# apple/ml-4m

Measured on AMD Instinct MI355X. Metric: multimodal tokens/sec (4M-B train step, whole job), higher is better.
Workload: dtype bf16; 1 GPU; 4M-B mod7 (fm_base_12e_12d_swiglu_nobias, 360.8M params, 8 input / 7 target modalities) masked-modeling train step, 224^2 token grids, 128 input + 128 target tokens/sample, AdamW; model=fm_base_12e_12d_swiglu_nobias, per_gpu_batch=256, global_batch=256, seq_len=256, parallelism=dp1

## Files before the change

include/fourm_hip.h:

```cpp
#ifndef FOURM_HIP_H
#define FOURM_HIP_H
#include <stdint.h>

#ifdef __cplusplus
extern "C" {
#endif

#define FM_ABI_VERSION 11
int fm_abi_version(void);
const char* fm_last_error(void);

enum fm_epilogue {
    FM_EPI_BF16 = 0,
    FM_EPI_GELU = 1,
    FM_EPI_RESIDUAL = 2,
    FM_EPI_SWIGLU = 3,
    FM_EPI_F32 = 4,
    FM_EPI_TANH = 5,
    FM_EPI_SWIGLU_BWD = 6,
    FM_EPI_GELU_BWD = 7,
    FM_EPI_QUICK_GELU = 8,
    FM_EPI_RELU = 9,
    FM_EPI_RELU_BWD = 10
};

typedef struct fm_gemm_group {
    const void* W;
    void* out;
    int32_t N, K, ldw, pad_;
} fm_gemm_group;

typedef struct fm_gemm_nt_args {
    const void* W; const void* W2; const void* X;
    void* out; void* out2; const void* res; const void* bias; const void* bias2;
    int32_t M, N, K, ldw, ldx, ldo, ldo2, ldr, Hp, epilogue;
    const fm_gemm_group* groups; const int32_t* tile_group; int32_t max_N;
    int32_t fixed_tiling;
    const int32_t* m_dev; const int32_t* row0_dev;
    void* splitk_ws; int64_t splitk_ws_bytes;
    int32_t conv_C, conv_H, conv_W, conv_Ho, conv_Wo, conv_stride, conv_up, conv_pad_;
} fm_gemm_nt_args;
int fm_gemm_nt(const fm_gemm_nt_args* args, void* stream);
void fm_set_gemm_nt_config(int cfg);
int fm_get_gemm_nt_config(void);
void fm_set_reserved_cus(int n);
int fm_get_reserved_cus(void);

typedef struct fm_gemm_tn_args {
    const void* A; const void* B; void* out;
    int32_t R, N, K, lda, ldb, ldo, a_cols, b_cols, splits, force_tr;
    const fm_gemm_group* groups; const int32_t* seg_start; const int32_t* seg_count;
    int32_t n_groups, max_N, max_R, pad_;
} fm_gemm_tn_args;
int fm_gemm_tn(const fm_gemm_tn_args* args, void* stream);
#define FM_TN_MAX_JOBS 16
typedef struct fm_gemm_tn_job {
    const void* A; const void* B; void* out;
    int32_t R, N, K, lda, ldb, ldo, a_cols, b_cols;
} fm_gemm_tn_job;
int fm_gemm_tn_multi(const fm_gemm_tn_job* jobs, int n_jobs, void* stream);
void fm_set_gemm_tn_config(int cfg);
int fm_get_gemm_tn_config(void);
void fm_set_tn_transpose_read(int on);
int fm_get_tn_transpose_read(void);

int fm_layernorm_fwd(const void* x, int ldx, const void* w, const void* b, void* y, int ldy, int y_is_f32,
                     void* mean, void* rstd, const int32_t* row_map, int R, int D, float eps, void* stream);
int fm_layernorm_fwd_res(const void* x, int ldx, const void* delta, int ldd, void* x_out, int ldxo, const void* w, const void* b,
                         void* y, int ldy, int y_is_f32, void* mean, void* rstd, const int32_t* row_map, int R, int D, float eps,
                         void* stream);
int fm_layernorm_bwd(const void* dy, int lddy, const int32_t* dy_row_map, const void* x, int ldx, const void* w,
                     const void* mean, const void* rstd, const void* dres, void* dx, int lddx, void* dx_bf16,
                     int lddxbf, void* dw, void* db, int R, int D, void* stream);
int fm_layernorm_bwd_h(const void* dy, int lddy, const void* h, int ldh, const void* x, int ldx, const void* w,
                       const void* mean, const void* rstd, const void* dres, void* dx, int lddx, void* dx_bf16,
                       int lddxbf, void* dw, int R, int D, void* stream);

int fm_headnorm_fwd(const void* x, int ldx, const void* w, const void* b, void* y, int ldy, void* stats, int R, int H, float eps,
                    void* stream);
int fm_headnorm_bwd(const void* dy, int lddy, const void* x, int ldx, const void* w, const void* stats, void* dx, int lddx, void* dw,
                    void* db, int R, int H, void* stream);

enum fm_mask_kind {
    FM_MASK_NONE = 0,
    FM_MASK_KEYPAD = 1,
    FM_MASK_DECODER = 2,
    FM_MASK_DENSE = 3
};
typedef struct fm_attn_args {
    const void* Q; const void* K; const void* V; void* O;
    void* stat_m; void* stat_l;
    int32_t ldq, ldk, ldv, ldo;
    int32_t B, H, Nq, Nk, head_dim, mask_kind;
    float scale; int32_t causal;
    const void* kpad; const int32_t* cs; const int16_t* modq; const int16_t* modk; const void* dense;
    const void* dO; void* dQ; void* dK; void* dV;
    int32_t lddo, lddq, lddk, lddv;
    int32_t force_tr;
    int32_t kv_batch_rows;
    int32_t zero_attn;
} fm_attn_args;
int fm_attn_fwd(const fm_attn_args* args, void* stream);
int fm_attn_bwd(const fm_attn_args* args, void* stream);
void fm_set_attn_transpose_read(int on);
int fm_get_attn_transpose_read(void);

#define FM_ATTN_DECODE_MAX_NK 8192
typedef struct fm_attn_decode_args {
    const void* q; void* k; const void* v; void* o;
    const void* q_w; const void* q_b; const void* k_w; const void* k_b;
    const void* kpad;
    int32_t ldq, ldk, ldv, ldo;
    int32_t B, H, Nk, kv_batch_rows, k_new_row, is_f32, zero_attn, pad_;
    float scale, eps;
} fm_attn_decode_args;
int fm_attn_decode(const fm_attn_decode_args* args, void* stream);

#define FM_MAX_MODS 24
enum fm_mod_kind {
    FM_KIND_TOK = 0,
    FM_KIND_PATCH = 1,
    FM_KIND_SEQ = 2,
    FM_KIND_SEQ_EMB = 3
};
typedef struct fm_mod_desc {
    const void* ids;
    const void* mask;
    const void* dam;
    const void* table;
    const void* pos;
    const void* mod_emb;
    const void* proj_bias;
    int32_t L;
    int32_t kind, ids_are_i64, mod_id;
    int32_t max_len;
    int32_t shifted;
    int32_t mask_stride, id_stride;
    int32_t patch, channels, grid_w, orig_dim;
    int32_t head_index;
    int32_t pad_;
} fm_mod_desc;

typedef struct fm_select_desc {
    fm_mod_desc mods[FM_MAX_MODS];
    int32_t n_mods, batch, dim, n_keep, n_reg, total_len, is_decoder;
    int32_t raw;
    const void* reg_tokens;
    const void* mask_token;
    void* tokens;
    void* emb;
    void* x0;
    void* out_mask;
    void* out_mod;
    void* slot_mod;
    void* slot_src;
    void* slot_pos;
    void* target_ids;
    void* out_cs;
    void* out_mod_pre;
    void* out_mod_index;
    void* patch_rows;
    void* seqemb_rows;
    int32_t patch_ld, seqemb_ld;
    int32_t rows_f32;
    int32_t pad2_;
} fm_select_desc;
int fm_select_embed(const fm_select_desc* desc, void* stream);

typedef struct fm_embed_bwd_mod {
    void* d_table;
    void* d_pos;
    void* d_mod_emb;
    void* d_proj_bias;
    int32_t kind, has_padding_idx, padding_idx, pad_;
} fm_embed_bwd_mod;
typedef struct fm_embed_bwd_desc {
    fm_embed_bwd_mod mods[FM_MAX_MODS];
    const void* dx;
    const void* slot_mod; const void* slot_src; const void* slot_pos;
    void* d_mask_token;
    void* d_reg_tokens;
    int32_t n_mods, batch, dim, Nt, lddx, is_decoder;
} fm_embed_bwd_desc;
int fm_embed_bwd(const fm_embed_bwd_desc* desc, void* stream);

int fm_dense_decoder_mask(const int32_t* cs, const int16_t* mod, void* out, int B, int M, int causal, int use_cs,
                          int use_sep, void* stream);

enum fm_loss_type { FM_LOSS_MOD = 0, FM_LOSS_TOKEN = 1 };
#define FM_SEG_ROWS 256
int fm_segment_rows(const int32_t* head_of_row, int R, int n_heads, int32_t* seg_start, int32_t* seg_count,
                    int32_t* perm, int32_t* row_to_padded, int32_t* tile_group, int Rp, void* stream);
int fm_gather_rows(const void* src, int ld_src, const int32_t* perm, void* dst, int ld_dst, int Rp, int D, void* stream);
int fm_cross_entropy(void* logits, int ldl, const int32_t* perm, const int32_t* tile_group, const int64_t* target_ids,
                     const int32_t* vocab, const int32_t* seg_start, const int32_t* seg_count, const void* grad_scale,
                     int loss_type, int n_heads, int Rp, int max_vocab, void* row_loss, void* row_lse, void* head_loss,
                     void* total_loss, int write_grad, void* stream);

int fm_swiglu_bwd(const void* da, int ldda, const void* gu, int ldgu, void* dgu, int lddgu, int R, int H, int Hp, void* stream);
int fm_gelu_bwd(const void* dh, int lddh, const void* pre, int ldp, void* dpre, int lddp, int R, int H, int Hp, void* stream);
typedef struct fm_shadow_desc {
    const void* src; void* dst;
    int32_t ld_src, ld_dst, rows, cols, transpose, tile_start;
    const void* col_scale;
    int32_t dst_f32, reserved;
} fm_shadow_desc;
int fm_shadow_refresh(const fm_shadow_desc* descs, int n_descs, int total_tiles, void* stream);
#define FM_FOLD_MAX_JOBS 48
typedef struct fm_fold_grad_job {
    const void* dWp; const void* W; const void* gamma; void* gW; void* ggamma;
    int32_t rows, cols, ld_dwp, reserved;
} fm_fold_grad_job;
int fm_fold_colscale_grad(const fm_fold_grad_job* jobs, int n_jobs, void* stream);

int fm_cast_pad(const void* src, int ld_src, void* dst, int ld_dst, int rows, int cols, void* stream);
int fm_transpose_cast_pad(const void* src, int ld_src, void* dst, int ld_dst, int dst_cols, int rows, int cols, void* stream);
int fm_colsum(const void* dy, int ldy, void* db, int R, int N, void* stream);
int fm_f32_to_bf16(const void* src, void* dst, int64_t n, void* stream);
int fm_bf16_to_f32_scaled(const void* src, void* dst, int64_t n, float scale, void* stream);
int fm_add_bf16_f32(const void* x, const void* delta, void* out, int64_t n, void* stream);
int fm_scale_rows_bf16(void* x, int ld, const void* scale, int rows_per_sample, int R, int N, void* stream);

int fm_vit_patch_rows(const void* pixels, void* rows, int ld, int B, int C, int H, int W, int P, int rows_f32, void* stream);
int fm_vit_emb_rows(const void* pos, const void* mod_emb, void* x, int ldx, int B, int Np, int D, void* stream);
int fm_vit_colsum(const void* dy, int ldy, void* db, int R, int N, void* ws, int64_t ws_bytes, void* stream);

int fm_clip_embed_ln(const void* patches, int ldp, int patches_f32, const void* cls, const void* pos, const void* w, const void* b,
                     void* out, int ldo, int B, int G, int D, float eps, void* stream);

enum { FM_FEAT_COSINE = 0, FM_FEAT_L1 = 1 };
int fm_feat_distance(const void* pred, int ldp, const void* tgt, int ldt, int B, int T, int D, int mode, void* loss, void* dpred, int lddp,
                     void* stream);
int fm_quick_gelu_bwd(const void* da, int ldda, const void* pre, int ldp, void* dpre, int lddp, int R, int H, int Hp, void* stream);
int fm_quick_gelu_bwd_f32(const void* da, int ldda, const void* pre, int ldp, void* dpre, int lddp, int R, int H, void* stream);
int fm_clip_embed_ln_bwd(const void* dy, int lddy, const void* patches, int ldp, int patches_f32, const void* pos, const void* w,
                         void* d_patches, int lddp, int B, int G, int D, float eps, void* stream);
int fm_tap_add(void* g, int ldg, void* g_bf, int ldgb, const void* dtap, int ldt, const void* row_scale, int rows_per_sample, int R, int D,
               void* stream);

#define FM_LPIPS_CHUNK 64
int fm_lpips_stem(const void* img, const void* mul, const void* add, const void* w, const void* bias, void* out, int ldo, int is_f32, int B, int H,
                  int W, void* stream);
int fm_lpips_stem_bwd(const void* d, int ldd, int is_f32, const void* w, const void* mul, const void* row_scale, void* dimg, int B, int H, int W,
                      void* stream);
int fm_maxpool2x2_nhwc(const void* x, int ldx, void* y, int ldy, int is_f32, int B, int H, int W, int C, void* stream);
int fm_lpips_distance(const void* pred, int ldp, const void* tgt, int ldt, int is_f32, const void* w, int B, int P, int C, void* loss, void* dpred,
                      int lddp, void* scratch, void* stream);
int fm_lpips_tap_bwd(const void* act, int lda, const void* din, int ldi, const void* dtap, int ldt, const void* dpool, int ldp, void* d, int ldd,
                     int is_f32, int B, int H, int W, int C, void* stream);

int fm_lora_apply(const void* x, int ldx, const void* down, int64_t down_sr, int64_t down_sk, const void* up, int64_t up_sn, int64_t up_sr,
                  void* y, int ldy, float scale, void* p_out, int R, int K, int N, int r, int x_f32, int y_f32, void* stream);
int fm_lora_grad(const void* a, int lda, const void* b, void* out, int64_t out_sn, int64_t out_sr, float scale, int accumulate,
                 int R, int n, int r, int a_f32, void* stream);

int fm_adamw(void* p, const void* g, void* m, void* v, int64_t n, float lr, float beta1, float beta2, float eps,
             float weight_decay, int64_t step, const void* grad_mult, const void* hyper, void* sumsq, void* stream);
#define FM_ADAMW_CHUNK 8192
typedef struct fm_adamw_job {
    void* p; const void* g; void* m; void* v; void* dst_plain; void* dst_t;
    int32_t rows, cols, ld_plain, ld_t, tile_start, pad_;
} fm_adamw_job;
int fm_adamw_shadow(const fm_adamw_job* jobs, int n_jobs, int total_tiles, float lr, float beta1, float beta2, float eps,
                    float weight_decay, int64_t step, const void* grad_mult, const void* hyper, void* sumsq, void* stream);
int fm_sumsq(const void* x, int64_t n, void* out, void* stream);
int fm_clip_coef(const void* sumsq, float max_norm, void* norm_out, void* coef_out, void* stream);

int fm_sample_tokens(const void* logits, int ld, int logits_are_f32, int R, int V, float temperature, int top_k, float top_p,
                     const void* uniforms, void* out_ids, void* out_prob, void* stream);
int fm_guidance_combine(const void* uncond, int ldu, int uncond_is_f32, const void* cond, int ldc, int cond_is_f32, float weight,
                        void* out, int ldo, int R, int V, int accumulate, void* stream);
int fm_maskgit_commit(const void* prob, const void* samples, const int32_t* mod_pos, int B, int N, int num_select, void* tensor,
                      int tensor_is_i64, int L, void* input_mask, void* target_mask, int32_t* top_idx, void* stream);

typedef struct fm_gemm_f32_args {
    const void* X; const void* W; const void* W2; void* out; void* out2; const void* res; const void* bias; const void* bias2;
    int64_t sxm, sxk, swn, swk;
    int32_t M, N, K, ldo, ldo2, ldr, Hp, epilogue, accumulate, max_N, seg_rows, n_groups;
    const fm_gemm_group* groups; const int32_t* tile_group; const int32_t* seg_start; const int32_t* seg_count;
} fm_gemm_f32_args;
int fm_gemm_f32(const fm_gemm_f32_args* args, void* stream);
int fm_attn_f32_fwd(const fm_attn_args* args, void* stream);
int fm_attn_f32_bwd(const fm_attn_args* args, void* stream);
int fm_layernorm_bwd_f32(const void* dy, int lddy, const int32_t* dy_row_map, const void* x, int ldx, const void* w, const void* mean,
                         const void* rstd, const void* dres, void* dx, int lddx, void* dx2, int lddx2, void* dw, void* db, int R, int D,
                         void* stream);
int fm_headnorm_f32_fwd(const void* x, int ldx, const void* w, const void* b, void* y, int ldy, void* stats, int R, int H, float eps, void* stream);
int fm_headnorm_f32_bwd(const void* dy, int lddy, const void* x, int ldx, const void* w, const void* stats, void* dx, int lddx, void* dw, void* db,
                        int R, int H, void* stream);
int fm_swiglu_bwd_f32(const void* da, int ldda, const void* gu, int ldgu, void* dgu, int lddgu, int R, int H, int Hp, void* stream);
int fm_gelu_bwd_f32(const void* dh, int lddh, const void* pre, int ldp, void* dpre, int lddp, int R, int H, void* stream);
int fm_colsum_f32(const void* dy, int ldy, void* db, int R, int N, void* stream);
int fm_cross_entropy_f32(void* logits, int ldl, const int32_t* perm, const int32_t* tile_group, const int64_t* target_ids,
                         const int32_t* vocab, const int32_t* seg_start, const int32_t* seg_count, const void* grad_scale, int loss_type,
                         int n_heads, int padded_rows, int max_vocab, void* row_loss, void* row_lse, void* head_loss, void* total_loss,
                         int write_grad, void* stream);

int fm_unet_im2col_f32(const void* src1, int ld1, int C1, const void* src2, int ld2, int C2, int H2, int W2, void* out, int ldo, int kpad,
                       int B, int H, int W, int ksize, int stride, int up1, void* stream);
int fm_groupnorm_nhwc_f32(const void* x, int ldx, const void* add, int ld_add, const void* w, const void* b, void* y, int ldy, int B, int HW, int C,
                          int groups, float eps, int silu, void* stream);
int fm_unet_attention_f32(const void* qkv, int ld, void* out, int ldo, int B, int T, int heads, int ch, void* stream);
int fm_add_f32(const void* a, int lda, const void* b, int ldb, void* out, int ldo, int64_t rows, int C, void* stream);
int fm_silu_f32(const void* x, void* y, int64_t n, void* stream);
int fm_timestep_embedding_f32(const void* t, void* out, int ldo, int B, int dim, float max_period, void* stream);
int fm_unet_col2im_f32(const void* col, int ldc, void* dsrc, int ld, int C, int B, int H, int W, int ksize, int stride, int up1, int accumulate, void* stream);
int fm_groupnorm_nhwc_bwd_f32(const void* dy, int lddy, const void* x, int ldx, const void* add, int ld_add, const void* w, const void* b, void* dx, int lddx,
                              void* dw, void* db, void* dadd, int ld_dadd, void* scratch, int B, int HW, int C, int groups, float eps, int silu, void* stream);
int fm_unet_attention_bwd_f32(const void* qkv, int ld, const void* dout, int lddo, void* dqkv, int lddqkv, void* scratch, int B, int T, int heads, int ch,
                              void* stream);
int fm_silu_bwd_f32(const void* dy, const void* x, void* dx, int64_t n, void* stream);

int fm_vq_patchify(const void* img, void* out, int ld_out, int B, int C, int H, int W, int P, void* stream);
int fm_l2norm_rows(const void* x, int ldx, void* y, int ldy, int R, int D, void* stream);
int fm_vq_assign(const void* z, int ldz, const void* codes_normalized, const void* embed, int K, int D, int R,
                 int tokens_per_image, int normalize_latents, void* ws_val, void* ws_idx, int splits, int64_t* tokens,
                 void* quant, void* stream);
#define FM_VQ_WIDE_TILE 128
int fm_vq_assign_wide(const void* z, int ldz, const void* codes_normalized, const void* embed, int K, int D, int R,
                      int tokens_per_image, void* ws_val, void* ws_idx, int code_tiles, int64_t* tokens, void* quant, void* stream);
int fm_memcodes_assign(const void* z, int ldz, const void* keys, const void* values, int K, int d, int H, int R,
                       int tokens_per_image, void* ws_val, void* ws_idx, int code_tiles, int64_t* tokens, void* quant, void* stream);
int fm_vq_code_stats(const void* z, int ldz, const int64_t* tokens, int R, int D, int K, void* bins, void* sums, void* stream);
int fm_vq_ema_update(const void* bins, const void* sums, void* embed, void* cluster_size, int K, int D, float decay, void* stream);
int fm_vq_code_bias(const void* embed, int K, int D, void* bias, void* stream);
int fm_vq_assign_bias(const void* z, int ldz, const void* codes, const void* code_bias, const void* embed, int K, int D, int R,
                      int tokens_per_image, int normalize_latents, void* ws_val, void* ws_idx, int splits, int64_t* tokens,
                      void* quant, void* stream);
int fm_vq_code_stats_raw(const void* z, int ldz, const int64_t* tokens, int R, int D, int K, void* bins, void* sums, void* stream);
int fm_vq_ema_update_euclid(const void* bins, const void* sums, void* embed, void* embed_avg, void* cluster_size, void* total_scratch,
                            int K, int D, float decay, float eps, void* stream);

int fm_vq_unpatchify(const void* rows, int ld_rows, void* img, int B, int C, int H, int W, int P, void* stream);
#define FM_CONVNEXT_MAX_C 4
int fm_convnext_block(const void* x, void* y, const void* dw_weight, const void* dw_bias, const void* ln_weight, const void* ln_bias,
                      const void* pw1_weight, const void* pw1_bias, const void* pw2_weight, const void* pw2_bias, const void* gamma,
                      int B, int C, int H, int W, float eps, void* stream);
// ... 129 lines not shown
```

ml-4m_amd/csrc/layernorm.hip:

```cpp
#include <algorithm>
#include "common.h"
#include "fourm_hip.h"

namespace {

constexpr int MAXC_LIMIT = 8;

__device__ __forceinline__ float4 ld4(const float* p, bool nt) {
    if (nt) { const f32x4_t t = __builtin_nontemporal_load((const f32x4_t*)p); return make_float4(t[0], t[1], t[2], t[3]); }
    return *(const float4*)p;
}
__device__ __forceinline__ uint2 ld2u(const bf16_t* p, bool nt) {
    typedef __attribute__((ext_vector_type(2))) unsigned int u2_t;
    if (nt) { const u2_t t = __builtin_nontemporal_load((const u2_t*)p); return make_uint2(t[0], t[1]); }
    return *(const uint2*)p;
}
template <typename T> __device__ __forceinline__ void store4(T* p, float a, float b, float c, float d);
template <> __device__ __forceinline__ void store4<float>(float* p, float a, float b, float c, float d) {
    *(float4*)p = make_float4(a, b, c, d);
}
template <> __device__ __forceinline__ void store4<bf16_t>(bf16_t* p, float a, float b, float c, float d) {
    *(uint2*)p = make_uint2(pack2bf(a, b), pack2bf(c, d));
}

template <typename OutT, int MAXC, bool RES = false>
__global__ __launch_bounds__(256) void ln_fwd_kernel(const float* __restrict__ x, int ldx, const float* __restrict__ w,
                                                     const float* __restrict__ b, OutT* __restrict__ y, int ldy,
                                                     float* __restrict__ mean, float* __restrict__ rstd,
                                                     const int* __restrict__ row_map, int R, int D, float eps,
                                                     const bf16_t* __restrict__ delta = nullptr, int ldd = 0, float* __restrict__ xo = nullptr, int ldxo = 0,
                                                     int nt_res = 0) {
    const int lane = threadIdx.x & 63, wave = threadIdx.x >> 6;
    const int nch = D >> 2;
    float4 ww[MAXC], bb[MAXC];
#pragma unroll
    for (int c = 0; c < MAXC; ++c) {
        const int ch = lane + 64 * c;
        ww[c] = ch < nch ? *(const float4*)(w + ch * 4) : make_float4(0.f, 0.f, 0.f, 0.f);
        bb[c] = (b && ch < nch) ? *(const float4*)(b + ch * 4) : make_float4(0.f, 0.f, 0.f, 0.f);
    }
    constexpr int NR = 2;
    for (int r0 = blockIdx.x * 4 + wave; r0 < R; r0 += gridDim.x * 4 * NR) {
        float4 v[NR][MAXC];
#pragma unroll
        for (int q = 0; q < NR; ++q) {
            const int r = r0 + q * gridDim.x * 4;
#pragma unroll
            for (int c = 0; c < MAXC; ++c) {
                const int ch = lane + 64 * c;
                v[q][c] = (ch < nch && r < R) ? ld4(x + (size_t)r * ldx + ch * 4, nt_res & 2) : make_float4(0.f, 0.f, 0.f, 0.f);
            }
        }
        if constexpr (RES) {
            uint2 dl[NR][MAXC];
#pragma unroll
            for (int q = 0; q < NR; ++q) {
                const int r = r0 + q * gridDim.x * 4;
#pragma unroll
                for (int c = 0; c < MAXC; ++c) {
                    const int ch = lane + 64 * c;
                    dl[q][c] = (ch < nch && r < R) ? ld2u(delta + (size_t)r * ldd + ch * 4, nt_res & 2) : make_uint2(0u, 0u);
                }
            }
#pragma unroll
            for (int q = 0; q < NR; ++q) {
                const int r = r0 + q * gridDim.x * 4;
#pragma unroll
                for (int c = 0; c < MAXC; ++c) {
                    const int ch = lane + 64 * c;
                    float d4[4];
                    unpack_bf4(dl[q][c], d4);
                    v[q][c].x += d4[0]; v[q][c].y += d4[1]; v[q][c].z += d4[2]; v[q][c].w += d4[3];
                    if (ch < nch && r < R) {
                        if (nt_res & 1) __builtin_nontemporal_store(f32x4_t{v[q][c].x, v[q][c].y, v[q][c].z, v[q][c].w}, (f32x4_t*)(xo + (size_t)r * ldxo + ch * 4));
                        else *(float4*)(xo + (size_t)r * ldxo + ch * 4) = v[q][c];
                    }
                }
            }
        }
#pragma unroll
        for (int q = 0; q < NR; ++q) {
            const int r = r0 + q * gridDim.x * 4;
            if (r >= R) continue;
            float s = 0.f;
#pragma unroll
            for (int c = 0; c < MAXC; ++c) s += (v[q][c].x + v[q][c].y) + (v[q][c].z + v[q][c].w);
            const float mu = wave_sum(s) / (float)D;
            float sq = 0.f;
#pragma unroll
            for (int c = 0; c < MAXC; ++c) {
                const int ch = lane + 64 * c;
                if (ch < nch) {
                    const float a0 = v[q][c].x - mu, a1 = v[q][c].y - mu, a2 = v[q][c].z - mu, a3 = v[q][c].w - mu;
                    sq += (a0 * a0 + a1 * a1) + (a2 * a2 + a3 * a3);
                }
            }
            const float rs = rsqrtf(wave_sum(sq) / (float)D + eps);
            if (lane == 0) {
                if (mean) mean[r] = mu;
                if (rstd) rstd[r] = rs;
            }
            const int dst = row_map ? row_map[r] : r;
            if (dst < 0) continue;
            OutT* yr = y + (size_t)dst * ldy;
#pragma unroll
            for (int c = 0; c < MAXC; ++c) {
                const int ch = lane + 64 * c;
                if (ch < nch)
                    store4<OutT>(yr + ch * 4, (v[q][c].x - mu) * rs * ww[c].x + bb[c].x, (v[q][c].y - mu) * rs * ww[c].y + bb[c].y,
                                 (v[q][c].z - mu) * rs * ww[c].z + bb[c].z, (v[q][c].w - mu) * rs * ww[c].w + bb[c].w);
            }
        }
    }
}

static int ln_nt_flags() {
    static const int f = [] { const char* e = getenv("FOURM_LN_NT"); return e ? atoi(e) : 24; }();
    return f;
}
static int bwd_rows(int R) {
    static const int env = [] { const char* e = getenv("FOURM_LN_BWD_ROWS"); return e ? atoi(e) : 0; }();
    if (env >= 4) return env;
    return R >= 512 * 64 ? 64 : 32;
}

template <int MAXC, bool FROM_H = false, bool HAS_DB = true>
__global__ __launch_bounds__(256) void ln_bwd_kernel(const bf16_t* __restrict__ dy, int lddy, const int* __restrict__ dy_row_map,
                                                     const bf16_t* __restrict__ h, int ldh,
                                                     const float* __restrict__ x, int ldx, const float* __restrict__ w,
                                                     const float* __restrict__ mean, const float* __restrict__ rstd,
                                                     const float* dres, float* dx, int lddx, bf16_t* __restrict__ dx_bf, int lddxbf,
                                                     float* __restrict__ dw, float* __restrict__ db, int R, int D, int BWD_ROWS, int nt_dx) {
    extern __shared__ __attribute__((aligned(16))) char smem[];
    float* red = (float*)smem;
    const int lane = threadIdx.x & 63, wave = threadIdx.x >> 6;
    const int nch = D >> 2;
    float4 aw[MAXC], ab[MAXC], wv[MAXC], iw[FROM_H ? MAXC : 1];
    bool from_x[FROM_H ? MAXC : 1];
#pragma unroll
    for (int c = 0; c < MAXC; ++c) {
        aw[c] = ab[c] = make_float4(0.f, 0.f, 0.f, 0.f);
        const int ch = lane + 64 * c;
        wv[c] = ch < nch ? *(const float4*)(w + ch * 4) : make_float4(0.f, 0.f, 0.f, 0.f);
        if constexpr (FROM_H) {
            from_x[c] = fminf(fminf(fabsf(wv[c].x), fabsf(wv[c].y)), fminf(fabsf(wv[c].z), fabsf(wv[c].w))) < 1e-20f;
            iw[c] = from_x[c] ? make_float4(0.f, 0.f, 0.f, 0.f) : make_float4(1.f / wv[c].x, 1.f / wv[c].y, 1.f / wv[c].z, 1.f / wv[c].w);
        }
    }
    const int r_end = min(R, (int)(blockIdx.x + 1) * BWD_ROWS);
    constexpr int NR = 2;
    for (int r0 = blockIdx.x * BWD_ROWS + wave; r0 < r_end; r0 += 4 * NR) {
        uint2 dyp[NR][MAXC], hp[NR][FROM_H ? MAXC : 1];
        float4 xv[NR][MAXC], rv[NR][MAXC];
        float mu[NR], rs[NR];
        bool live[NR];
#pragma unroll
        for (int q = 0; q < NR; ++q) {
            const int r = r0 + 4 * q;
            live[q] = r < r_end;
            const int rr = live[q] ? r : r0;
            const int src = dy_row_map ? dy_row_map[rr] : rr;
            mu[q] = mean[rr]; rs[q] = rstd[rr];
#pragma unroll
            for (int c = 0; c < MAXC; ++c) {
                const int ch = lane + 64 * c;
                dyp[q][c] = make_uint2(0u, 0u);
                xv[q][c] = rv[q][c] = make_float4(0.f, 0.f, 0.f, 0.f);
                if (ch < nch && live[q]) {
                    if (src >= 0) dyp[q][c] = ld2u(dy + (size_t)src * lddy + ch * 4, nt_dx & 2);
                    if constexpr (FROM_H) {
                        hp[q][c] = ld2u(h + (size_t)rr * ldh + ch * 4, nt_dx & 4);
                        if (from_x[c]) xv[q][c] = *(const float4*)(x + (size_t)rr * ldx + ch * 4);
                    } else xv[q][c] = *(const float4*)(x + (size_t)rr * ldx + ch * 4);
                    if (dres) rv[q][c] = ld4(dres + (size_t)rr * lddx + ch * 4, nt_dx & 2);
                }
            }
        }
#pragma unroll
        for (int q = 0; q < NR; ++q) {
            if (!live[q]) continue;
            const int r = r0 + 4 * q;
            float4 g[MAXC], xh[MAXC];
            float s1 = 0.f, s2 = 0.f;
#pragma unroll
            for (int c = 0; c < MAXC; ++c) {
                const int ch = lane + 64 * c;
                g[c] = xh[c] = make_float4(0.f, 0.f, 0.f, 0.f);
                if (ch < nch) {
                    const uint2 p = dyp[q][c];
                    const float4 d = make_float4(bf2f((bf16_t)(p.x & 0xffff)), bf2f((bf16_t)(p.x >> 16)), bf2f((bf16_t)(p.y & 0xffff)), bf2f((bf16_t)(p.y >> 16)));
                    const float4 v = xv[q][c];
                    xh[c] = make_float4((v.x - mu[q]) * rs[q], (v.y - mu[q]) * rs[q], (v.z - mu[q]) * rs[q], (v.w - mu[q]) * rs[q]);
                    if constexpr (FROM_H) {
                        const uint2 hh = hp[q][c];
                        if (!from_x[c]) xh[c] = make_float4(bf2f((bf16_t)(hh.x & 0xffff)) * iw[c].x, bf2f((bf16_t)(hh.x >> 16)) * iw[c].y,
                                                            bf2f((bf16_t)(hh.y & 0xffff)) * iw[c].z, bf2f((bf16_t)(hh.y >> 16)) * iw[c].w);
                    }
                    aw[c].x += d.x * xh[c].x; aw[c].y += d.y * xh[c].y; aw[c].z += d.z * xh[c].z; aw[c].w += d.w * xh[c].w;
                    if constexpr (HAS_DB) { ab[c].x += d.x; ab[c].y += d.y; ab[c].z += d.z; ab[c].w += d.w; }
                    g[c] = make_float4(d.x * wv[c].x, d.y * wv[c].y, d.z * wv[c].z, d.w * wv[c].w);
                    s1 += (g[c].x + g[c].y) + (g[c].z + g[c].w);
                    s2 += (g[c].x * xh[c].x + g[c].y * xh[c].y) + (g[c].z * xh[c].z + g[c].w * xh[c].w);
                }
            }
            const float m1 = wave_sum(s1) / (float)D, m2 = wave_sum(s2) / (float)D;
#pragma unroll
            for (int c = 0; c < MAXC; ++c) {
                const int ch = lane + 64 * c;
                if (ch < nch) {
                    const float4 t = rv[q][c];
                    const float4 o = make_float4(rs[q] * (g[c].x - m1 - xh[c].x * m2) + t.x, rs[q] * (g[c].y - m1 - xh[c].y * m2) + t.y,
                                                 rs[q] * (g[c].z - m1 - xh[c].z * m2) + t.z, rs[q] * (g[c].w - m1 - xh[c].w * m2) + t.w);
                    if (nt_dx & 1) __builtin_nontemporal_store(f32x4_t{o.x, o.y, o.z, o.w}, (f32x4_t*)(dx + (size_t)r * lddx + ch * 4));
                    else *(float4*)(dx + (size_t)r * lddx + ch * 4) = o;
                    if (dx_bf) *(uint2*)(dx_bf + (size_t)r * lddxbf + ch * 4) = make_uint2(pack2bf(o.x, o.y), pack2bf(o.z, o.w));
                }
            }
        }
    }
    if (!dw && !db) return;
#pragma unroll
    for (int c = 0; c < MAXC; ++c) {
        const int ch = lane + 64 * c;
        if (ch < nch) {
            *(float4*)(red + (size_t)wave * D + ch * 4) = aw[c];
            if constexpr (HAS_DB) *(float4*)(red + (size_t)(4 + wave) * D + ch * 4) = ab[c];
        }
    }
    __syncthreads();
    for (int i = threadIdx.x; i < D; i += 256) {
        if (dw) unsafeAtomicAdd(dw + i, (red[i] + red[D + i]) + (red[2 * D + i] + red[3 * D + i]));
        if constexpr (HAS_DB) if (db) unsafeAtomicAdd(db + i, (red[4 * D + i] + red[5 * D + i]) + (red[6 * D + i] + red[7 * D + i]));
    }
}


__device__ __forceinline__ float group16_sum(float v) {
    v += __shfl_xor(v, 1, 64); v += __shfl_xor(v, 2, 64); v += __shfl_xor(v, 4, 64); v += __shfl_xor(v, 8, 64);
    return v;
}

__global__ __launch_bounds__(256) void headnorm_fwd_kernel(const bf16_t* __restrict__ x, int ldx, const float* __restrict__ w,
                                                           const float* __restrict__ b, bf16_t* __restrict__ y, int ldy,
                                                           float2* __restrict__ stats, int R, int H, float eps) {
    const int sub = threadIdx.x & 15;
    const float4 wv = *(const float4*)(w + sub * 4);
    const float4 bv = b ? *(const float4*)(b + sub * 4) : make_float4(0.f, 0.f, 0.f, 0.f);
    const size_t total = (size_t)R * H;
    for (size_t v = (size_t)blockIdx.x * 16 + (threadIdx.x >> 4); v < total; v += (size_t)gridDim.x * 16) {
        const int r = v / H, h = v % H;
        const uint2 p = *(const uint2*)(x + (size_t)r * ldx + h * 64 + sub * 4);
        const float e[4] = {bf2f((bf16_t)(p.x & 0xffff)), bf2f((bf16_t)(p.x >> 16)), bf2f((bf16_t)(p.y & 0xffff)), bf2f((bf16_t)(p.y >> 16))};
        const float mean = group16_sum(e[0] + e[1] + e[2] + e[3]) * (1.0f / 64.0f);
        float q = 0.f;
#pragma unroll
        for (int i = 0; i < 4; ++i) q += (e[i] - mean) * (e[i] - mean);
        const float rs = rsqrtf(group16_sum(q) * (1.0f / 64.0f) + eps);
        const float o0 = (e[0] - mean) * rs * wv.x + bv.x, o1 = (e[1] - mean) * rs * wv.y + bv.y;
        const float o2 = (e[2] - mean) * rs * wv.z + bv.z, o3 = (e[3] - mean) * rs * wv.w + bv.w;
        *(uint2*)(y + (size_t)r * ldy + h * 64 + sub * 4) = make_uint2(pack2bf(o0, o1), pack2bf(o2, o3));
        if (sub == 0 && stats) stats[v] = make_float2(mean, rs);
    }
}

__global__ __launch_bounds__(256) void headnorm_bwd_kernel(const bf16_t* __restrict__ dy, int lddy, const bf16_t* __restrict__ x, int ldx,
                                                           const float* __restrict__ w, const float2* __restrict__ stats,
                                                           bf16_t* __restrict__ dx, int lddx, float* __restrict__ dw, float* __restrict__ db,
                                                           int R, int H) {
    __shared__ float red[2][16][64];
    const int sub = threadIdx.x & 15, grp = threadIdx.x >> 4;
    const float4 wv = *(const float4*)(w + sub * 4);
    const float wj[4] = {wv.x, wv.y, wv.z, wv.w};
    float aw[4] = {0.f, 0.f, 0.f, 0.f}, ab[4] = {0.f, 0.f, 0.f, 0.f};
    const size_t total = (size_t)R * H;
    for (size_t v = (size_t)blockIdx.x * 16 + grp; v < total; v += (size_t)gridDim.x * 16) {
        const int r = v / H, h = v % H;
        const uint2 px = *(const uint2*)(x + (size_t)r * ldx + h * 64 + sub * 4);
        const uint2 pd = *(const uint2*)(dy + (size_t)r * lddy + h * 64 + sub * 4);
        const float2 st = stats[v];
        const float e[4] = {bf2f((bf16_t)(px.x & 0xffff)), bf2f((bf16_t)(px.x >> 16)), bf2f((bf16_t)(px.y & 0xffff)), bf2f((bf16_t)(px.y >> 16))};
        const float d[4] = {bf2f((bf16_t)(pd.x & 0xffff)), bf2f((bf16_t)(pd.x >> 16)), bf2f((bf16_t)(pd.y & 0xffff)), bf2f((bf16_t)(pd.y >> 16))};
        float xh[4], g[4], s1 = 0.f, s2 = 0.f;
#pragma unroll
        for (int i = 0; i < 4; ++i) {
            xh[i] = (e[i] - st.x) * st.y;
            g[i] = d[i] * wj[i];
            s1 += g[i]; s2 += g[i] * xh[i];
            aw[i] += d[i] * xh[i]; ab[i] += d[i];
        }
        s1 = group16_sum(s1) * (1.0f / 64.0f); s2 = group16_sum(s2) * (1.0f / 64.0f);
        float o[4];
#pragma unroll
        for (int i = 0; i < 4; ++i) o[i] = st.y * (g[i] - s1 - xh[i] * s2);
        *(uint2*)(dx + (size_t)r * lddx + h * 64 + sub * 4) = make_uint2(pack2bf(o[0], o[1]), pack2bf(o[2], o[3]));
    }
#pragma unroll
    for (int i = 0; i < 4; ++i) { red[0][grp][sub * 4 + i] = aw[i]; red[1][grp][sub * 4 + i] = ab[i]; }
    __syncthreads();
    if (threadIdx.x < 128) {
        const int which = threadIdx.x >> 6, c = threadIdx.x & 63;
        float s = 0.f;
#pragma unroll
        for (int gq = 0; gq < 16; ++gq) s += red[which][gq][c];
        float* dst = which ? db : dw;
        if (dst) unsafeAtomicAdd(dst + c, s);
    }
}

}

static int chunks_for(int D) { const int c = (D / 4 + 63) / 64; return c <= 2 ? 2 : c <= 3 ? 3 : c <= 4 ? 4 : 8; }

extern "C" int fm_layernorm_fwd(const void* x, int ldx, const void* w, const void* b, void* y, int ldy, int y_is_f32,
                                void* mean, void* rstd, const int32_t* row_map, int R, int D, float eps, void* stream) {
    FM_CHECK_ARG(x && w && y, "fm_layernorm_fwd: null pointer");
    FM_CHECK_ARG(R > 0 && D > 0 && D % 4 == 0 && D <= 64 * 4 * MAXC_LIMIT, "fm_layernorm_fwd: D=%d must be a multiple of 4 and <= %d", D, 64 * 4 * MAXC_LIMIT);
    FM_CHECK_ARG(ldx % 4 == 0 && ldy % 4 == 0, "fm_layernorm_fwd: leading dims must be multiples of 4");
    int grid = (R + 3) / 4;
    if (grid > 256 * 16) grid = 256 * 16;
#define LN_FWD(T, C)                                                                                                        \
    hipLaunchKernelGGL((ln_fwd_kernel<T, C>), dim3(grid), dim3(256), 0, (hipStream_t)stream, (const float*)x, ldx, (const float*)w, \
                       (const float*)b, (T*)y, ldy, (float*)mean, (float*)rstd, row_map, R, D, eps)
#define LN_FWD_C(T)                                    \
    switch (chunks_for(D)) {                           \
        case 2: LN_FWD(T, 2); break;                   \
        case 3: LN_FWD(T, 3); break;                   \
        case 4: LN_FWD(T, 4); break;                   \
        default: LN_FWD(T, 8); break;                  \
    }
    if (y_is_f32) { LN_FWD_C(float) } else { LN_FWD_C(bf16_t) }
#undef LN_FWD_C
#undef LN_FWD
    FM_CHECK_LAUNCH("fm_layernorm_fwd");
    return 0;
}

extern "C" int fm_layernorm_fwd_res(const void* x, int ldx, const void* delta, int ldd, void* x_out, int ldxo, const void* w, const void* b,
                                    void* y, int ldy, int y_is_f32, void* mean, void* rstd, const int32_t* row_map, int R, int D, float eps,
                                    void* stream) {
    FM_CHECK_ARG(x && delta && x_out && w && y, "fm_layernorm_fwd_res: null pointer");
    FM_CHECK_ARG(R > 0 && D > 0 && D % 4 == 0 && D <= 64 * 4 * MAXC_LIMIT, "fm_layernorm_fwd_res: D=%d must be a multiple of 4 and <= %d", D, 64 * 4 * MAXC_LIMIT);
    FM_CHECK_ARG(ldx % 4 == 0 && ldy % 4 == 0 && ldd % 4 == 0 && ldxo % 4 == 0, "fm_layernorm_fwd_res: leading dims must be multiples of 4");
    FM_CHECK_ARG((((uintptr_t)delta) & 7) == 0 && (((uintptr_t)x_out | (uintptr_t)x) & 15) == 0, "fm_layernorm_fwd_res: alignment (delta 8 B, x / x_out 16 B)");
    int grid = (R + 3) / 4;
    if (grid > 256 * 16) grid = 256 * 16;
#define LN_FWD(T, C)                                                                                                        \
    hipLaunchKernelGGL((ln_fwd_kernel<T, C, true>), dim3(grid), dim3(256), 0, (hipStream_t)stream, (const float*)x, ldx, (const float*)w, \
                       (const float*)b, (T*)y, ldy, (float*)mean, (float*)rstd, row_map, R, D, eps, (const bf16_t*)delta, ldd, (float*)x_out, ldxo, (ln_nt_flags() & 1) | ((ln_nt_flags() >> 1) & 2))
#define LN_FWD_C(T)                                    \
    switch (chunks_for(D)) {                           \
        case 2: LN_FWD(T, 2); break;                   \
        case 3: LN_FWD(T, 3); break;                   \
        case 4: LN_FWD(T, 4); break;                   \
        default: LN_FWD(T, 8); break;                  \
    }
    if (y_is_f32) { LN_FWD_C(float) } else { LN_FWD_C(bf16_t) }
#undef LN_FWD_C
#undef LN_FWD
    FM_CHECK_LAUNCH("fm_layernorm_fwd_res");
    return 0;
}

static int layernorm_bwd_launch(const void* dy, int lddy, const int32_t* dy_row_map, const void* h, int ldh, const void* x, int ldx, const void* w,
                                const void* mean, const void* rstd, const void* dres, void* dx, int lddx, void* dx_bf16,
                                int lddxbf, void* dw, void* db, int R, int D, void* stream) {
    FM_CHECK_ARG(dy && x && w && mean && rstd && dx, "fm_layernorm_bwd: null pointer");
    FM_CHECK_ARG(!h || ldh % 4 == 0, "fm_layernorm_bwd_h: ldh must be a multiple of 4");
    FM_CHECK_ARG(R > 0 && D > 0 && D % 4 == 0 && D <= 64 * 4 * MAXC_LIMIT, "fm_layernorm_bwd: D=%d unsupported", D);
    FM_CHECK_ARG(ldx % 4 == 0 && lddy % 4 == 0 && lddx % 4 == 0 && lddxbf % 4 == 0, "fm_layernorm_bwd: leading dims must be multiples of 4");
    const int BWD_ROWS = bwd_rows(R);
    const int grid = (R + BWD_ROWS - 1) / BWD_ROWS;
    const size_t lds = (size_t)8 * D * sizeof(float);
#define LN_BWD_(C, FH)                                                                                                      \
    {                                                                                                                       \
        auto k = ln_bwd_kernel<C, FH, !FH>;                                                                                     \
        static bool once = (hipFuncSetAttribute((const void*)k, hipFuncAttributeMaxDynamicSharedMemorySize, 8 * 2048 * 4) == hipSuccess); \
        (void)once;                                                                                                         \
        hipLaunchKernelGGL(k, dim3(grid), dim3(256), lds, (hipStream_t)stream, (const bf16_t*)dy, lddy, dy_row_map, (const bf16_t*)h, ldh, \
                           (const float*)x, ldx, (const float*)w, (const float*)mean, (const float*)rstd, (const float*)dres, (float*)dx, lddx, \
                           (bf16_t*)dx_bf16, lddxbf, (float*)dw, (float*)db, R, D, BWD_ROWS, ((ln_nt_flags() >> 1) & 1) | ((ln_nt_flags() >> 2) & 2) | ((ln_nt_flags() >> 2) & 4));                               \
    }
#define LN_BWD(C) { if (h) LN_BWD_(C, true) else LN_BWD_(C, false) }
    switch (chunks_for(D)) {
        case 2: LN_BWD(2) break;
        case 3: LN_BWD(3) break;
        case 4: LN_BWD(4) break;
        default: LN_BWD(8) break;
    }
#undef LN_BWD
#undef LN_BWD_
    FM_CHECK_LAUNCH("fm_layernorm_bwd");
    return 0;
}

extern "C" int fm_layernorm_bwd(const void* dy, int lddy, const int32_t* dy_row_map, const void* x, int ldx, const void* w,
                                const void* mean, const void* rstd, const void* dres, void* dx, int lddx, void* dx_bf16,
                                int lddxbf, void* dw, void* db, int R, int D, void* stream) {
    return layernorm_bwd_launch(dy, lddy, dy_row_map, nullptr, 0, x, ldx, w, mean, rstd, dres, dx, lddx, dx_bf16, lddxbf, dw, db, R, D, stream);
}

extern "C" int fm_layernorm_bwd_h(const void* dy, int lddy, const void* h, int ldh, const void* x, int ldx, const void* w,
                                  const void* mean, const void* rstd, const void* dres, void* dx, int lddx, void* dx_bf16,
                                  int lddxbf, void* dw, int R, int D, void* stream) {
    FM_CHECK_ARG(h, "fm_layernorm_bwd_h: null pointer");
    return layernorm_bwd_launch(dy, lddy, nullptr, h, ldh, x, ldx, w, mean, rstd, dres, dx, lddx, dx_bf16, lddxbf, dw, nullptr, R, D, stream);
}

extern "C" int fm_headnorm_fwd(const void* x, int ldx, const void* w, const void* b, void* y, int ldy, void* stats, int R, int H, float eps,
                               void* stream) {
    FM_CHECK_ARG(x && w && y && R > 0 && H > 0, "fm_headnorm_fwd: bad argument");
    FM_CHECK_ARG(ldx % 4 == 0 && ldy % 4 == 0 && ((((uintptr_t)x | (uintptr_t)y) & 7) == 0) && ((((uintptr_t)w | (uintptr_t)b) & 15) == 0),
                 "fm_headnorm_fwd: alignment (x/y 8 B, w/b 16 B, leading dims %% 4)");
    const size_t total = (size_t)R * H;
    const int grid = (int)std::min<size_t>((total + 15) / 16, 256 * 32);
    hipLaunchKernelGGL(headnorm_fwd_kernel, dim3(grid), dim3(256), 0, (hipStream_t)stream, (const bf16_t*)x, ldx, (const float*)w, (const float*)b,
                       (bf16_t*)y, ldy, (float2*)stats, R, H, eps);
    FM_CHECK_LAUNCH("fm_headnorm_fwd");
    return 0;
}

extern "C" int fm_headnorm_bwd(const void* dy, int lddy, const void* x, int ldx, const void* w, const void* stats, void* dx, int lddx, void* dw,
                               void* db, int R, int H, void* stream) {
    FM_CHECK_ARG(dy && x && w && stats && dx && R > 0 && H > 0, "fm_headnorm_bwd: bad argument");
    FM_CHECK_ARG(ldx % 4 == 0 && lddy % 4 == 0 && lddx % 4 == 0 && ((((uintptr_t)x | (uintptr_t)dy | (uintptr_t)dx) & 7) == 0) &&
                     ((((uintptr_t)w) & 15) == 0), "fm_headnorm_bwd: alignment (x/dy/dx 8 B, w 16 B, leading dims %% 4)");
    const size_t total = (size_t)R * H;
    const int grid = (int)std::min<size_t>((total + 15) / 16, 256 * 8);
    hipLaunchKernelGGL(headnorm_bwd_kernel, dim3(grid), dim3(256), 0, (hipStream_t)stream, (const bf16_t*)dy, lddy, (const bf16_t*)x, ldx,
                       (const float*)w, (const float2*)stats, (bf16_t*)dx, lddx, (float*)dw, (float*)db, R, H);
    FM_CHECK_LAUNCH("fm_headnorm_bwd");
    return 0;
}
```

ml-4m_amd/csrc/select_embed.hip:

```cpp
#include "common.h"
#include "fourm_hip.h"

namespace {

constexpr int MAXPOS = 8192;
constexpr int MAXKEEP = 1024;

struct SelArgs {
    fm_select_desc d;
};

__device__ __forceinline__ long long load_id(const void* ids, int is64, size_t i) {
    return is64 ? ((const long long*)ids)[i] : (long long)((const int*)ids)[i];
}

__device__ __forceinline__ int block_scan_excl(int v, int* wave_tot , int* total) {
    const int lane = threadIdx.x & 63, wave = threadIdx.x >> 6;
    const int inc = wave_scan_incl(v);
    if (lane == 63) wave_tot[wave] = inc;
    __syncthreads();
    int base = 0, tot = 0;
#pragma unroll
    for (int w = 0; w < 4; ++w) {
        const int t = wave_tot[w];
        if (w < wave) base += t;
        tot += t;
    }
    __syncthreads();
    *total = tot;
    return base + inc - v;
}

__global__ __launch_bounds__(256) void select_embed_kernel(SelArgs A) {
    const fm_select_desc& d = A.d;
    extern __shared__ __attribute__((aligned(16))) char smem[];
    const int P = d.total_len;
    int* rank_sel = (int*)smem;
    int* rank_pos = rank_sel + P;
    int* slot_p = rank_pos + P;
    uint8_t* flag = (uint8_t*)(slot_p + d.n_keep);
    __shared__ int wave_tot[4];
    __shared__ int mod_off[FM_MAX_MODS + 1];
    __shared__ int cs_scan[MAXKEEP];

    const int b = blockIdx.x;
    const int tid = threadIdx.x, lane = tid & 63, wave = tid >> 6;
    if (tid == 0) {
        int o = 0;
        for (int m = 0; m < d.n_mods; ++m) { mod_off[m] = o; o += d.mods[m].L; }
        mod_off[d.n_mods] = o;
    }
    __syncthreads();

    auto mod_of = [&](int p) {
        int m = 0;
        while (m + 1 < d.n_mods && p >= mod_off[m + 1]) ++m;
        return m;
    };

    int run_sel = 0, run_pos = 0;
    for (int base = 0; base < P; base += 256) {
        const int p = base + tid;
        int sel = 0, um = 0;
        if (p < P) {
            const int m = mod_of(p);
            const fm_mod_desc& md = d.mods[m];
            const int j = p - mod_off[m];
            const uint8_t* mk = (const uint8_t*)md.mask + (size_t)b * md.mask_stride;
            if (d.is_decoder && md.shifted) {
                um = mk[j] == 0;
                sel = (mk[j] == 0) && (mk[j + 1] == 0);
            } else {
                um = sel = mk[j] == 0;
            }
            flag[p] = (uint8_t)(sel | (um << 1));
        }
        int ts, tp;
        const int es = block_scan_excl(sel, wave_tot, &ts);
        const int ep = block_scan_excl(um, wave_tot, &tp);
        if (p < P) { rank_sel[p] = run_sel + es; rank_pos[p] = run_pos + ep; }
        run_sel += ts; run_pos += tp;
    }
    const int n_valid = run_sel;
    __syncthreads();
    for (int p = tid; p < P; p += 256) {
        const int s = d.raw ? p : (flag[p] & 1) ? rank_sel[p] : n_valid + (p - rank_sel[p]);
        if (s < d.n_keep) slot_p[s] = p;
    }
    __syncthreads();

    if (d.is_decoder && !d.raw) {
        if (wave == 0) {
            int run = 0;
            for (int base = 0; base < d.n_keep; base += 64) {
                const int s = base + lane;
                int v = 0;
                if (s < d.n_keep) {
                    const int p = slot_p[s];
                    const int m = mod_of(p);
                    const fm_mod_desc& md = d.mods[m];
                    v = ((const int*)md.dam)[(size_t)b * md.mask_stride + (p - mod_off[m])];
                }
                const int inc = wave_scan_incl(v);
                if (s < d.n_keep) cs_scan[s] = run + inc;
                run += __shfl(inc, 63, 64);
            }
        }
        __syncthreads();
    }

    const int D = d.dim, nch = D >> 2;
    const int Nt = d.n_reg + d.n_keep;
    for (int s = wave + 4 * blockIdx.y; s < Nt; s += 4 * gridDim.y) {
        const size_t orow = (size_t)b * Nt + s;
        float* tok_o = (float*)d.tokens + orow * D;
        float* emb_o = (float*)d.emb + orow * D;
        float* x0_o = d.x0 ? (float*)d.x0 + orow * D : nullptr;
        if (s < d.n_reg) {
            for (int c = lane; c < nch; c += 64) {
                const float4 t = *(const float4*)((const float*)d.reg_tokens + (size_t)s * D + c * 4);
                *(float4*)(tok_o + c * 4) = t;
                *(float4*)(emb_o + c * 4) = make_float4(0.f, 0.f, 0.f, 0.f);
                if (x0_o) *(float4*)(x0_o + c * 4) = t;
            }
            if (lane == 0) {
                ((uint8_t*)d.out_mask)[orow] = 0;
                ((int16_t*)d.out_mod)[orow] = -1;
                ((int32_t*)d.slot_mod)[orow] = -2;
                ((int32_t*)d.slot_src)[orow] = s;
                ((int32_t*)d.slot_pos)[orow] = 0;
            }
            const int esz = d.rows_f32 ? 2 : 1;
            if (d.patch_rows) {
                uint2* pr = (uint2*)((char*)d.patch_rows + orow * d.patch_ld * (size_t)(2 * esz));
                for (int f = lane; f < d.patch_ld / 4 * esz; f += 64) pr[f] = make_uint2(0u, 0u);
            }
            if (d.seqemb_rows) {
                uint2* sr = (uint2*)((char*)d.seqemb_rows + orow * d.seqemb_ld * (size_t)(2 * esz));
                for (int f = lane; f < d.seqemb_ld / 4 * esz; f += 64) sr[f] = make_uint2(0u, 0u);
            }
            continue;
        }
        const int sk = s - d.n_reg;
        const int p = slot_p[sk];
        const int m = mod_of(p);
        const fm_mod_desc& md = d.mods[m];
        const int j = p - mod_off[m];
        const bool masked = (flag[p] & 1) == 0;
        const bool own_unmasked = (flag[p] & 2) != 0;
        const bool raw = d.raw != 0;
        long long id = 0;
        int posrow = 0;
// ... 25 lines not shown
            else if (md.kind == FM_KIND_SEQ_EMB) trow = (const float*)md.proj_bias;
        }
        const float* prow = (const float*)md.pos + (size_t)posrow * D;
        const float* mrow = (const float*)md.mod_emb;
        const bool seq_kind = md.kind == FM_KIND_SEQ || md.kind == FM_KIND_SEQ_EMB;
        const bool with_emb = raw ? true : !masked;
        const bool with_pos = raw ? (!seq_kind || own_unmasked) : true;
        for (int c = lane; c < nch; c += 64) {
            float4 t = make_float4(0.f, 0.f, 0.f, 0.f), e = make_float4(0.f, 0.f, 0.f, 0.f);
            if (trow) t = *(const float4*)(trow + c * 4);
            if (with_emb) {
                const float4 mm = *(const float4*)(mrow + c * 4);
                float4 pp = make_float4(0.f, 0.f, 0.f, 0.f);
                if (with_pos) pp = *(const float4*)(prow + c * 4);
                e = make_float4(pp.x + mm.x, pp.y + mm.y, pp.z + mm.z, pp.w + mm.w);
            }
            *(float4*)(tok_o + c * 4) = t;
            *(float4*)(emb_o + c * 4) = e;
            if (x0_o) *(float4*)(x0_o + c * 4) = make_float4(t.x + e.x, t.y + e.y, t.z + e.z, t.w + e.w);
        }
        if (d.patch_rows && d.rows_f32) {
            float* pr = (float*)d.patch_rows + orow * d.patch_ld;
            const bool here = (!masked || raw) && md.kind == FM_KIND_PATCH;
            const int ps = md.patch, C = md.channels, gw = md.grid_w;
            const float* img = (const float*)md.ids + (size_t)b * md.id_stride;
            for (int f = lane; f < d.patch_ld; f += 64) {
                float v = 0.f;
                if (here && f < ps * ps * C) {
                    const int gy = j / gw, gx = j % gw, Wd = gw * ps, Hd = (md.L / gw) * ps;
                    const int c = f % C, px = (f / C) % ps, py = f / (C * ps);
                    v = img[((size_t)c * Hd + gy * ps + py) * Wd + gx * ps + px];
                }
                pr[f] = v;
            }
        } else if (d.patch_rows) {
            bf16_t* pr = (bf16_t*)d.patch_rows + orow * d.patch_ld;
            if ((!masked || raw) && md.kind == FM_KIND_PATCH) {
                const int ps = md.patch, C = md.channels, gw = md.grid_w;
                const int gy = j / gw, gx = j % gw;
                const float* img = (const float*)md.ids + (size_t)b * md.id_stride;
                const int Wd = gw * ps, Hd = (md.L / gw) * ps;
                for (int f = lane; f < d.patch_ld; f += 64) {
                    float v = 0.f;
                    if (f < ps * ps * C) {
                        const int c = f % C, px = (f / C) % ps, py = f / (C * ps);
                        v = img[((size_t)c * Hd + gy * ps + py) * Wd + gx * ps + px];
                    }
                    pr[f] = f2bf(v);
                }
            } else {
                for (int f = lane; f < d.patch_ld / 4; f += 64) *(uint2*)(pr + f * 4) = make_uint2(0u, 0u);
            }
        }
        if (d.seqemb_rows && d.rows_f32) {
            float* sr = (float*)d.seqemb_rows + orow * d.seqemb_ld;
            const bool here = (!masked || raw) && md.kind == FM_KIND_SEQ_EMB;
            const float* src = (const float*)md.ids + (size_t)b * md.id_stride + (size_t)j * md.orig_dim;
            for (int f = lane; f < d.seqemb_ld; f += 64) sr[f] = (here && f < md.orig_dim) ? src[f] : 0.f;
        } else if (d.seqemb_rows) {
            bf16_t* sr = (bf16_t*)d.seqemb_rows + orow * d.seqemb_ld;
            if ((!masked || raw) && md.kind == FM_KIND_SEQ_EMB) {
                const float* src = (const float*)md.ids + (size_t)b * md.id_stride + (size_t)j * md.orig_dim;
                for (int f = lane; f < d.seqemb_ld; f += 64) sr[f] = f2bf(f < md.orig_dim ? src[f] : 0.f);
            } else {
                for (int f = lane; f < d.seqemb_ld / 4; f += 64) *(uint2*)(sr + f * 4) = make_uint2(0u, 0u);
            }
        }
    }
}

__global__ __launch_bounds__(256) void embed_bwd_kernel(fm_embed_bwd_desc d) {
    extern __shared__ __attribute__((aligned(16))) char smem[];
    float* acc = (float*)smem;
    const int D = d.dim, nch = D >> 2;
    const int b = blockIdx.x, lane = threadIdx.x & 63, wave = threadIdx.x >> 6;
    const int rows = d.n_mods + 1;
    for (int i = threadIdx.x; i < rows * D; i += 256) acc[i] = 0.f;
    __shared__ int used[FM_MAX_MODS + 1];
    if (threadIdx.x <= FM_MAX_MODS) used[threadIdx.x] = 0;
    __syncthreads();
    constexpr int MAXQ = 8;
    const int parts = 4 * gridDim.y, part = wave + 4 * blockIdx.y;
    const int per = (d.Nt + parts - 1) / parts, s_lo = part * per, s_hi = min(d.Nt, s_lo + per);
    float4 racc[MAXQ];
    int cur = -1;
    bool cur_mask = false;
    auto flush = [&]() {
        if (cur < 0) return;
#pragma unroll
        for (int q = 0; q < MAXQ; ++q) {
            const int c = lane + 64 * q;
            if (c >= nch) break;
            float* a0 = acc + (size_t)cur * D + c * 4;
            atomicAdd(a0, racc[q].x); atomicAdd(a0 + 1, racc[q].y); atomicAdd(a0 + 2, racc[q].z); atomicAdd(a0 + 3, racc[q].w);
            if (cur_mask) {
                float* a1 = acc + (size_t)d.n_mods * D + c * 4;
                atomicAdd(a1, racc[q].x); atomicAdd(a1 + 1, racc[q].y); atomicAdd(a1 + 2, racc[q].z); atomicAdd(a1 + 3, racc[q].w);
            }
        }
    };
    for (int s = s_lo; s < s_hi; ++s) {
        const size_t row = (size_t)b * d.Nt + s;
        const int m = ((const int32_t*)d.slot_mod)[row];
        if (m == -1) continue;
        const float* g = (const float*)d.dx + row * d.lddx;
        if (m == -2) {
            if (d.d_reg_tokens)
                for (int c = lane; c < D; c += 64) unsafeAtomicAdd((float*)d.d_reg_tokens + (size_t)s * D + c, g[c]);
            continue;
        }
        const fm_embed_bwd_mod& md = d.mods[m];
        const int src = ((const int32_t*)d.slot_src)[row];
        const int posrow = ((const int32_t*)d.slot_pos)[row];
        const bool to_mask_token = d.is_decoder && md.kind == FM_KIND_TOK;
        if (m != cur) {
            flush();
            cur = m; cur_mask = to_mask_token;
#pragma unroll
            for (int q = 0; q < MAXQ; ++q) racc[q] = make_float4(0.f, 0.f, 0.f, 0.f);
            if (lane == 0) { used[m] = 1; if (to_mask_token) used[d.n_mods] = 1; }
        }
        float* trow = nullptr;
        if (to_mask_token) {}
        else if ((md.kind == FM_KIND_TOK || md.kind == FM_KIND_SEQ) && md.d_table && !(md.has_padding_idx && src == md.padding_idx))
            trow = (float*)md.d_table + (size_t)src * D;
        else if (md.kind == FM_KIND_SEQ_EMB && md.d_proj_bias) trow = (float*)md.d_proj_bias;
        float* prow = md.d_pos ? (float*)md.d_pos + (size_t)posrow * D : nullptr;
#pragma unroll
        for (int q = 0; q < MAXQ; ++q) {
            const int c = lane + 64 * q;
            if (c >= nch) break;
            const float4 v = *(const float4*)(g + c * 4);
            racc[q].x += v.x; racc[q].y += v.y; racc[q].z += v.z; racc[q].w += v.w;
            if (trow) {
                unsafeAtomicAdd(trow + c * 4, v.x); unsafeAtomicAdd(trow + c * 4 + 1, v.y);
                unsafeAtomicAdd(trow + c * 4 + 2, v.z); unsafeAtomicAdd(trow + c * 4 + 3, v.w);
            }
            if (prow) {
                unsafeAtomicAdd(prow + c * 4, v.x); unsafeAtomicAdd(prow + c * 4 + 1, v.y);
                unsafeAtomicAdd(prow + c * 4 + 2, v.z); unsafeAtomicAdd(prow + c * 4 + 3, v.w);
            }
        }
    }
    flush();
    __syncthreads();
    for (int m = 0; m < d.n_mods; ++m) {
        if (!used[m] || !d.mods[m].d_mod_emb) continue;
        for (int c = threadIdx.x; c < D; c += 256) unsafeAtomicAdd((float*)d.mods[m].d_mod_emb + c, acc[(size_t)m * D + c]);
    }
    if (used[d.n_mods] && d.d_mask_token)
        for (int c = threadIdx.x; c < D; c += 256) unsafeAtomicAdd((float*)d.d_mask_token + c, acc[(size_t)d.n_mods * D + c]);
}

__global__ void dense_decoder_mask_kernel(const int32_t* cs, const int16_t* mod, uint8_t* out, int B, int M, int causal, int use_cs, int use_sep) {
    const size_t i = (size_t)blockIdx.x * 256 + threadIdx.x;
    if (i >= (size_t)B * M * M) return;
    const int k = i % M, q = (i / M) % M, b = i / ((size_t)M * M);
    bool blk = false;
    if (causal) blk = k > q;
    else if (use_cs) blk = k >= cs[(size_t)b * M + q];
    if (use_sep) blk = blk || (mod[(size_t)b * M + q] != mod[(size_t)b * M + k]);
    out[i] = blk ? 1 : 0;
}

}

extern "C" int fm_select_embed(const fm_select_desc* d, void* stream) {
    FM_CHECK_ARG(d && d->tokens && d->emb && d->out_mask && d->out_mod && d->slot_mod && d->slot_src && d->slot_pos, "fm_select_embed: null output");
    FM_CHECK_ARG(d->n_mods > 0 && d->n_mods <= FM_MAX_MODS, "fm_select_embed: n_mods=%d out of range (max %d)", d->n_mods, FM_MAX_MODS);
    FM_CHECK_ARG(d->dim > 0 && d->dim % 4 == 0, "fm_select_embed: dim must be a multiple of 4");
    FM_CHECK_ARG(d->batch > 0 && d->n_keep > 0 && d->n_keep <= (d->raw ? MAXPOS : MAXKEEP), "fm_select_embed: n_keep=%d out of range (max %d)", d->n_keep,
                 d->raw ? MAXPOS : MAXKEEP);
    int total = 0;
    for (int m = 0; m < d->n_mods; ++m) {
        const fm_mod_desc& md = d->mods[m];
        FM_CHECK_ARG(md.L > 0 && md.mask && md.pos && md.mod_emb, "fm_select_embed: modality %d incomplete", m);
        FM_CHECK_ARG(md.kind != FM_KIND_PATCH || (d->patch_rows && md.ids), "fm_select_embed: pixel modality needs patch_rows and pixels");
        FM_CHECK_ARG(md.kind != FM_KIND_SEQ_EMB || (d->seqemb_rows && md.ids), "fm_select_embed: seq_emb modality needs seqemb_rows");
        FM_CHECK_ARG(!((md.kind == FM_KIND_TOK || md.kind == FM_KIND_SEQ) && !(d->is_decoder && md.kind == FM_KIND_TOK)) || md.table, "fm_select_embed: modality %d needs a table", m);
        FM_CHECK_ARG(!d->is_decoder || md.dam || d->raw, "fm_select_embed: decoder modality %d needs decoder_attention_mask", m);
        FM_CHECK_ARG(!(d->raw == 2 && md.kind == FM_KIND_TOK) || md.table, "fm_select_embed: modality %d needs a table", m);
        total += md.L;
    }
    FM_CHECK_ARG(total == d->total_len, "fm_select_embed: total_len=%d but the modalities sum to %d", d->total_len, total);
    FM_CHECK_ARG(total <= MAXPOS, "fm_select_embed: %d concatenated positions exceed %d", total, MAXPOS);
    FM_CHECK_ARG(d->n_keep <= total, "fm_select_embed: n_keep=%d exceeds the %d available positions", d->n_keep, total);
    FM_CHECK_ARG(d->raw >= 0 && d->raw <= 2 && (!d->raw || (d->n_keep == total && d->n_reg == 0)),
                 "fm_select_embed: raw views cover every position (n_keep == total_len) and carry no register tokens");
    FM_CHECK_ARG(!d->is_decoder || (d->target_ids && d->out_cs && d->out_mod_pre && d->out_mod_index && d->mask_token), "fm_select_embed: decoder outputs missing");
    FM_CHECK_ARG(d->n_reg == 0 || d->reg_tokens, "fm_select_embed: register tokens missing");
    FM_CHECK_ARG(d->patch_ld % 4 == 0 && d->seqemb_ld % 4 == 0, "fm_select_embed: side buffers need ld %% 4 == 0");
    const size_t lds = (size_t)total * 9 + (size_t)d->n_keep * 4 + 16;
    static bool once = (hipFuncSetAttribute((const void*)select_embed_kernel, hipFuncAttributeMaxDynamicSharedMemorySize, MAXPOS * 9 + MAXPOS * 4 + 16) == hipSuccess);
    (void)once;
    SelArgs A; A.d = *d;
    const int slices = d->batch >= 2048 ? 1 : d->batch >= 1024 ? 2 : 4;
    hipLaunchKernelGGL(select_embed_kernel, dim3(d->batch, slices), dim3(256), lds, (hipStream_t)stream, A);
    FM_CHECK_LAUNCH("fm_select_embed");
    return 0;
}

extern "C" int fm_embed_bwd(const fm_embed_bwd_desc* d, void* stream) {
    FM_CHECK_ARG(d && d->dx && d->slot_mod && d->slot_src && d->slot_pos, "fm_embed_bwd: null pointer");
    FM_CHECK_ARG(d->n_mods > 0 && d->n_mods <= FM_MAX_MODS && d->dim % 4 == 0 && d->dim <= 2048 && d->lddx % 4 == 0, "fm_embed_bwd: bad shape (dim <= 2048)");
    const size_t lds = (size_t)(d->n_mods + 1) * d->dim * sizeof(float);
    FM_CHECK_ARG(lds <= 150 * 1024, "fm_embed_bwd: %zu bytes of LDS needed", lds);
    static bool once = (hipFuncSetAttribute((const void*)embed_bwd_kernel, hipFuncAttributeMaxDynamicSharedMemorySize, 150 * 1024) == hipSuccess);
    (void)once;
    const int slices = d->batch >= 2048 ? 1 : d->batch >= 1024 ? 2 : 4;
    hipLaunchKernelGGL(embed_bwd_kernel, dim3(d->batch, slices), dim3(256), lds, (hipStream_t)stream, *d);
    FM_CHECK_LAUNCH("fm_embed_bwd");
    return 0;
}

extern "C" int fm_dense_decoder_mask(const int32_t* cs, const int16_t* mod, void* out, int B, int M, int causal, int use_cs, int use_sep, void* stream) {
    FM_CHECK_ARG(out && (causal || !use_cs || cs) && (!use_sep || mod), "fm_dense_decoder_mask: null pointer");
    const size_t n = (size_t)B * M * M;
    hipLaunchKernelGGL(dense_decoder_mask_kernel, dim3((n + 255) / 256), dim3(256), 0, (hipStream_t)stream, cs, mod, (uint8_t*)out, B, M, causal, use_cs, use_sep);
    FM_CHECK_LAUNCH("fm_dense_decoder_mask");
    return 0;
}
```

ml-4m_amd/fourm/hip/_lib.py:

```python
import ctypes as C
import os

FM_MAX_MODS = 24
_LIB_PATH = os.environ.get("FOURM_HIP_LIB") or os.path.join(os.path.dirname(os.path.dirname(os.path.abspath(__file__))), "_lib", "libfourm_hip.so")


class FourmHipUnavailable(ImportError):
    pass


def _load():
    if not os.path.exists(_LIB_PATH):
        raise FourmHipUnavailable(
            f"{_LIB_PATH} is missing - build the gfx950 kernels first: python ml-4m_amd/build_ext.py "
            "(the 4M hot path has no fallback implementation)")
    return C.CDLL(_LIB_PATH)


lib = _load()
lib.fm_last_error.restype = C.c_char_p
lib.fm_abi_version.restype = C.c_int
ABI_VERSION = 11
if lib.fm_abi_version() != ABI_VERSION:
    raise FourmHipUnavailable(f"libfourm_hip.so ABI {lib.fm_abi_version()} != expected {ABI_VERSION}; rebuild")

vp, i32, i64, f32 = C.c_void_p, C.c_int32, C.c_int64, C.c_float

EPI_BF16, EPI_GELU, EPI_RESIDUAL, EPI_SWIGLU, EPI_F32, EPI_TANH, EPI_SWIGLU_BWD, EPI_GELU_BWD, EPI_QUICK_GELU = 0, 1, 2, 3, 4, 5, 6, 7, 8
EPI_RELU, EPI_RELU_BWD = 9, 10
MASK_NONE, MASK_KEYPAD, MASK_DECODER, MASK_DENSE = 0, 1, 2, 3
KIND_TOK, KIND_PATCH, KIND_SEQ, KIND_SEQ_EMB = 0, 1, 2, 3
LOSS_MOD, LOSS_TOKEN = 0, 1


class GemmGroup(C.Structure):
    _fields_ = [("W", vp), ("out", vp), ("N", i32), ("K", i32), ("ldw", i32), ("pad_", i32)]


class GemmNTArgs(C.Structure):
    _fields_ = [("W", vp), ("W2", vp), ("X", vp), ("out", vp), ("out2", vp), ("res", vp), ("bias", vp), ("bias2", vp),
                ("M", i32), ("N", i32), ("K", i32), ("ldw", i32), ("ldx", i32), ("ldo", i32), ("ldo2", i32), ("ldr", i32),
                ("Hp", i32), ("epilogue", i32), ("groups", vp), ("tile_group", vp), ("max_N", i32), ("fixed_tiling", i32),
                ("m_dev", vp), ("row0_dev", vp), ("splitk_ws", vp), ("splitk_ws_bytes", i64),
                ("conv_C", i32), ("conv_H", i32), ("conv_W", i32), ("conv_Ho", i32), ("conv_Wo", i32), ("conv_stride", i32), ("conv_up", i32), ("conv_pad_", i32)]


class GemmTNArgs(C.Structure):
    _fields_ = [("A", vp), ("B", vp), ("out", vp), ("R", i32), ("N", i32), ("K", i32), ("lda", i32), ("ldb", i32),
                ("ldo", i32), ("a_cols", i32), ("b_cols", i32), ("splits", i32), ("force_tr", i32), ("groups", vp),
                ("seg_start", vp), ("seg_count", vp), ("n_groups", i32), ("max_N", i32), ("max_R", i32), ("pad_", i32)]


class GemmTNJob(C.Structure):
    _fields_ = [("A", vp), ("B", vp), ("out", vp), ("R", i32), ("N", i32), ("K", i32), ("lda", i32), ("ldb", i32),
                ("ldo", i32), ("a_cols", i32), ("b_cols", i32)]


TN_MAX_JOBS = 16


class AttnArgs(C.Structure):
    _fields_ = [("Q", vp), ("K", vp), ("V", vp), ("O", vp), ("stat_m", vp), ("stat_l", vp),
                ("ldq", i32), ("ldk", i32), ("ldv", i32), ("ldo", i32),
                ("B", i32), ("H", i32), ("Nq", i32), ("Nk", i32), ("head_dim", i32), ("mask_kind", i32),
                ("scale", f32), ("causal", i32),
                ("kpad", vp), ("cs", vp), ("modq", vp), ("modk", vp), ("dense", vp),
                ("dO", vp), ("dQ", vp), ("dK", vp), ("dV", vp),
                ("lddo", i32), ("lddq", i32), ("lddk", i32), ("lddv", i32), ("force_tr", i32), ("kv_batch_rows", i32), ("zero_attn", i32)]


class AttnDecodeArgs(C.Structure):
    _fields_ = [("q", vp), ("k", vp), ("v", vp), ("o", vp), ("q_w", vp), ("q_b", vp), ("k_w", vp), ("k_b", vp), ("kpad", vp),
                ("ldq", i32), ("ldk", i32), ("ldv", i32), ("ldo", i32),
                ("B", i32), ("H", i32), ("Nk", i32), ("kv_batch_rows", i32), ("k_new_row", i32), ("is_f32", i32), ("zero_attn", i32), ("pad_", i32),
                ("scale", f32), ("eps", f32)]


class ModDesc(C.Structure):
    _fields_ = [("ids", vp), ("mask", vp), ("dam", vp), ("table", vp), ("pos", vp), ("mod_emb", vp), ("proj_bias", vp),
                ("L", i32), ("kind", i32), ("ids_are_i64", i32), ("mod_id", i32), ("max_len", i32), ("shifted", i32),
                ("mask_stride", i32), ("id_stride", i32), ("patch", i32), ("channels", i32), ("grid_w", i32),
                ("orig_dim", i32), ("head_index", i32), ("pad_", i32)]


class ShadowDesc(C.Structure):
    _fields_ = [("src", vp), ("dst", vp), ("ld_src", i32), ("ld_dst", i32), ("rows", i32), ("cols", i32),
                ("transpose", i32), ("tile_start", i32), ("col_scale", vp), ("dst_f32", i32), ("reserved", i32)]


FOLD_MAX_JOBS = 48


class FoldGradJob(C.Structure):
    _fields_ = [("dWp", vp), ("W", vp), ("gamma", vp), ("gW", vp), ("ggamma", vp), ("rows", i32), ("cols", i32), ("ld_dwp", i32), ("reserved", i32)]


class GemmF32Args(C.Structure):
    _fields_ = [("X", vp), ("W", vp), ("W2", vp), ("out", vp), ("out2", vp), ("res", vp), ("bias", vp), ("bias2", vp),
                ("sxm", i64), ("sxk", i64), ("swn", i64), ("swk", i64),
                ("M", i32), ("N", i32), ("K", i32), ("ldo", i32), ("ldo2", i32), ("ldr", i32), ("Hp", i32), ("epilogue", i32),
                ("accumulate", i32), ("max_N", i32), ("seg_rows", i32), ("n_groups", i32),
                ("groups", vp), ("tile_group", vp), ("seg_start", vp), ("seg_count", vp)]


class SpanMaskArgs(C.Structure):
    _fields_ = [("ids", vp), ("len", vp), ("unit", vp), ("noise", vp), ("keep_prob", vp), ("r_choice", vp), ("input_budget", vp), ("target_budget", vp),
                ("sentinel_ids", vp), ("emb", vp), ("emb_out", vp), ("src", vp), ("tensor", vp), ("input_mask", vp), ("target_mask", vp),
                ("decoder_attention_mask", vp), ("tries", vp),
                ("B", i32), ("ld_ids", i32), ("T", i32), ("ld_noise", i32), ("n_sentinels", i32), ("max_tokens", i32), ("vocab_offset", i32), ("pad_id", i32),
                ("emb_rows", i32), ("emb_dim", i32)]


class AdamWJob(C.Structure):
    _fields_ = [("p", vp), ("g", vp), ("m", vp), ("v", vp), ("dst_plain", vp), ("dst_t", vp),
                ("rows", i32), ("cols", i32), ("ld_plain", i32), ("ld_t", i32), ("tile_start", i32), ("pad_", i32)]


class SelectDesc(C.Structure):
    _fields_ = [("mods", ModDesc * FM_MAX_MODS),
                ("n_mods", i32), ("batch", i32), ("dim", i32), ("n_keep", i32), ("n_reg", i32), ("total_len", i32),
                ("is_decoder", i32), ("raw", i32),
                ("reg_tokens", vp), ("mask_token", vp),
                ("tokens", vp), ("emb", vp), ("x0", vp), ("out_mask", vp), ("out_mod", vp), ("slot_mod", vp),
                ("slot_src", vp), ("slot_pos", vp), ("target_ids", vp), ("out_cs", vp), ("out_mod_pre", vp),
                ("out_mod_index", vp), ("patch_rows", vp), ("seqemb_rows", vp), ("patch_ld", i32), ("seqemb_ld", i32),
                ("rows_f32", i32), ("pad2_", i32)]


class EmbedBwdMod(C.Structure):
    _fields_ = [("d_table", vp), ("d_pos", vp), ("d_mod_emb", vp), ("d_proj_bias", vp),
                ("kind", i32), ("has_padding_idx", i32), ("padding_idx", i32), ("pad_", i32)]


class EmbedBwdDesc(C.Structure):
    _fields_ = [("mods", EmbedBwdMod * FM_MAX_MODS), ("dx", vp), ("slot_mod", vp), ("slot_src", vp), ("slot_pos", vp),
                ("d_mask_token", vp), ("d_reg_tokens", vp),
                ("n_mods", i32), ("batch", i32), ("dim", i32), ("Nt", i32), ("lddx", i32), ("is_decoder", i32)]


class EmaJob(C.Structure):
    _fields_ = [("ema", vp), ("model", vp), ("n", i64), ("first_chunk", i64)]


class PilCropJob(C.Structure):
    _fields_ = [("src_off", i64), ("mid_off", i64), ("out_slot", i64), ("blk_rows", i64), ("blk_cols", i64), ("H", i32), ("W", i32), ("top", i32), ("left", i32),
                ("h", i32), ("w", i32), ("flip", i32), ("tab_w", i32), ("tab_h", i32), ("taps_w", i32), ("taps_h", i32), ("pad_", i32)]


def _sig(name, *argtypes):
    fn = getattr(lib, name)
    fn.argtypes = list(argtypes)
    fn.restype = C.c_int
    return fn


P = C.POINTER
gemm_nt = _sig("fm_gemm_nt", P(GemmNTArgs), vp)
gemm_tn = _sig("fm_gemm_tn", P(GemmTNArgs), vp)
gemm_tn_multi = _sig("fm_gemm_tn_multi", P(GemmTNJob), C.c_int, vp)
layernorm_fwd = _sig("fm_layernorm_fwd", vp, i32, vp, vp, vp, i32, i32, vp, vp, vp, i32, i32, f32, vp)
layernorm_fwd_res = _sig("fm_layernorm_fwd_res", vp, i32, vp, i32, vp, i32, vp, vp, vp, i32, i32, vp, vp, vp, i32, i32, f32, vp)
layernorm_bwd = _sig("fm_layernorm_bwd", vp, i32, vp, vp, i32, vp, vp, vp, vp, vp, i32, vp, i32, vp, vp, i32, i32, vp)
layernorm_bwd_h = _sig("fm_layernorm_bwd_h", vp, i32, vp, i32, vp, i32, vp, vp, vp, vp, vp, i32, vp, i32, vp, i32, i32, vp)
attn_fwd = _sig("fm_attn_fwd", P(AttnArgs), vp)
attn_bwd = _sig("fm_attn_bwd", P(AttnArgs), vp)
attn_decode = _sig("fm_attn_decode", P(AttnDecodeArgs), vp)
ATTN_DECODE_MAX_NK = 8192
select_embed = _sig("fm_select_embed", P(SelectDesc), vp)
embed_bwd = _sig("fm_embed_bwd", P(EmbedBwdDesc), vp)
dense_decoder_mask = _sig("fm_dense_decoder_mask", vp, vp, vp, i32, i32, i32, i32, i32, vp)
segment_rows = _sig("fm_segment_rows", vp, i32, i32, vp, vp, vp, vp, vp, i32, vp)
gather_rows = _sig("fm_gather_rows", vp, i32, vp, vp, i32, i32, i32, vp)
cross_entropy = _sig("fm_cross_entropy", vp, i32, vp, vp, vp, vp, vp, vp, vp, i32, i32, i32, i32, vp, vp, vp, vp, i32, vp)
swiglu_bwd = _sig("fm_swiglu_bwd", vp, i32, vp, i32, vp, i32, i32, i32, i32, vp)
gelu_bwd = _sig("fm_gelu_bwd", vp, i32, vp, i32, vp, i32, i32, i32, i32, vp)
cast_pad = _sig("fm_cast_pad", vp, i32, vp, i32, i32, i32, vp)
transpose_cast_pad = _sig("fm_transpose_cast_pad", vp, i32, vp, i32, i32, i32, i32, vp)
colsum = _sig("fm_colsum", vp, i32, vp, i32, i32, vp)
shadow_refresh = _sig("fm_shadow_refresh", vp, i32, i32, vp)
fold_colscale_grad = _sig("fm_fold_colscale_grad", vp, i32, vp)
headnorm_fwd = _sig("fm_headnorm_fwd", vp, i32, vp, vp, vp, i32, vp, i32, i32, C.c_float, vp)
headnorm_bwd = _sig("fm_headnorm_bwd", vp, i32, vp, i32, vp, vp, vp, i32, vp, vp, i32, i32, vp)
f32_to_bf16 = _sig("fm_f32_to_bf16", vp, vp, i64, vp)
bf16_to_f32_scaled = _sig("fm_bf16_to_f32_scaled", vp, vp, i64, f32, vp)
add_bf16_f32 = _sig("fm_add_bf16_f32", vp, vp, vp, i64, vp)
lib.fm_set_reserved_cus.argtypes = [C.c_int]
lib.fm_get_reserved_cus.restype = C.c_int
lib.fm_get_reserved_cus.argtypes = []
adamw = _sig("fm_adamw", vp, vp, vp, vp, i64, f32, f32, f32, f32, f32, i64, vp, vp, vp, vp)
adamw_shadow = _sig("fm_adamw_shadow", vp, i32, i32, f32, f32, f32, f32, f32, i64, vp, vp, vp, vp)
sumsq = _sig("fm_sumsq", vp, i64, vp, vp)
clip_coef = _sig("fm_clip_coef", vp, f32, vp, vp, vp)
sample_tokens = _sig("fm_sample_tokens", vp, i32, i32, i32, i32, f32, i32, f32, vp, vp, vp, vp)
maskgit_commit = _sig("fm_maskgit_commit", vp, vp, vp, i32, i32, i32, vp, i32, i32, vp, vp, vp, vp)
gemm_f32 = _sig("fm_gemm_f32", P(GemmF32Args), vp)
attn_f32_fwd = _sig("fm_attn_f32_fwd", P(AttnArgs), vp)
attn_f32_bwd = _sig("fm_attn_f32_bwd", P(AttnArgs), vp)
layernorm_bwd_f32 = _sig("fm_layernorm_bwd_f32", vp, i32, vp, vp, i32, vp, vp, vp, vp, vp, i32, vp, i32, vp, vp, i32, i32, vp)
headnorm_f32_fwd = _sig("fm_headnorm_f32_fwd", vp, i32, vp, vp, vp, i32, vp, i32, i32, C.c_float, vp)
headnorm_f32_bwd = _sig("fm_headnorm_f32_bwd", vp, i32, vp, i32, vp, vp, vp, i32, vp, vp, i32, i32, vp)
swiglu_bwd_f32 = _sig("fm_swiglu_bwd_f32", vp, i32, vp, i32, vp, i32, i32, i32, i32, vp)
gelu_bwd_f32 = _sig("fm_gelu_bwd_f32", vp, i32, vp, i32, vp, i32, i32, i32, vp)
colsum_f32 = _sig("fm_colsum_f32", vp, i32, vp, i32, i32, vp)
cross_entropy_f32 = _sig("fm_cross_entropy_f32", vp, i32, vp, vp, vp, vp, vp, vp, vp, i32, i32, i32, i32, vp, vp, vp, vp, i32, vp)
vq_patchify = _sig("fm_vq_patchify", vp, vp, i32, i32, i32, i32, i32, i32, vp)
l2norm_rows = _sig("fm_l2norm_rows", vp, i32, vp, i32, i32, i32, vp)
vq_assign = _sig("fm_vq_assign", vp, i32, vp, vp, i32, i32, i32, i32, i32, vp, vp, i32, vp, vp, vp)
lib.fm_set_tn_transpose_read.argtypes = [C.c_int]
lib.fm_set_gemm_tn_config.argtypes = [C.c_int]
lib.fm_set_attn_transpose_read.argtypes = [C.c_int]

lib.fm_set_gemm_nt_config.argtypes = [C.c_int]
lib.fm_lab_set.argtypes = [C.c_int, C.c_int]
lib.fm_lab_set.restype = None
vq_code_stats = _sig("fm_vq_code_stats", vp, i32, vp, i32, i32, i32, vp, vp, vp)
vq_ema_update = _sig("fm_vq_ema_update", vp, vp, vp, vp, i32, i32, f32, vp)
vq_code_bias = _sig("fm_vq_code_bias", vp, i32, i32, vp, vp)
vq_assign_bias = _sig("fm_vq_assign_bias", vp, i32, vp, vp, vp, i32, i32, i32, i32, i32, vp, vp, i32, vp, vp, vp)
vq_code_stats_raw = _sig("fm_vq_code_stats_raw", vp, i32, vp, i32, i32, i32, vp, vp, vp)
vq_ema_update_euclid = _sig("fm_vq_ema_update_euclid", vp, vp, vp, vp, vp, vp, i32, i32, f32, f32, vp)
vq_unpatchify = _sig("fm_vq_unpatchify", vp, i32, vp, i32, i32, i32, i32, i32, vp)
VQ_WIDE_TILE, CONVNEXT_MAX_C = 128, 4
vq_assign_wide = _sig("fm_vq_assign_wide", vp, i32, vp, vp, i32, i32, i32, i32, vp, vp, i32, vp, vp, vp)
memcodes_assign = _sig("fm_memcodes_assign", vp, i32, vp, vp, i32, i32, i32, i32, i32, vp, vp, i32, vp, vp, vp)
convnext_block = _sig("fm_convnext_block", vp, vp, vp, vp, vp, vp, vp, vp, vp, vp, vp, i32, i32, i32, i32, f32, vp)
vq_latent_grad = _sig("fm_vq_latent_grad", vp, i32, vp, vp, vp, i32, vp, f32, vp, i32, vp, i32, i32, vp)
tanh_bwd_f32 = _sig("fm_tanh_bwd_f32", vp, vp, vp, i32, i32, i32, vp)
embed_rows_f32 = _sig("fm_embed_rows_f32", vp, vp, vp, i32, i32, i32, vp)
vq_patchify_ex = _sig("fm_vq_patchify_ex", vp, vp, vp, vp, vp, vp, i32, i32, i32, i32, i32, i32, vp)
vq_cls_emb_bwd = _sig("fm_vq_cls_emb_bwd", vp, i32, vp, vp, i32, i32, i32, i32, i32, vp)
vq_latent_grad_normalized = _sig("fm_vq_latent_grad_normalized", vp, i32, vp, vp, vp, i32, vp, f32, vp, i32, vp, i32, i32, vp)
scale_rows_bf16 = _sig("fm_scale_rows_bf16", vp, i32, vp, i32, i32, i32, vp)
image_mask = _sig("fm_image_mask", vp, vp, vp, i32, i32, vp, vp, vp, vp)
token_budgets = _sig("fm_token_budgets", vp, vp, vp, vp, vp, vp, vp, i32, i32, i32, i32, vp, vp, vp)
span_mask = _sig("fm_span_mask", P(SpanMaskArgs), vp)
guidance_combine = _sig("fm_guidance_combine", vp, i32, i32, vp, i32, i32, f32, vp, i32, i32, i32, i32, vp)
unpack_image_u8 = _sig("fm_unpack_image_u8", vp, vp, i32, i32, i32, i32, P(C.c_float), P(C.c_float), vp)
unpack_ids_u16 = _sig("fm_unpack_ids_u16", vp, vp, i64, vp)
unpack_mask_bits = _sig("fm_unpack_mask_bits", vp, vp, i32, i32, vp)
decoder_attention_from_target = _sig("fm_decoder_attention_from_target", vp, vp, i32, i32, vp)
split3_bf16 = _sig("fm_split3_bf16", vp, i32, vp, i32, i32, i32, i32, i32, vp)
unet_im2col = _sig("fm_unet_im2col", vp, i32, i32, vp, i32, i32, i32, i32, vp, i32, i32, i32, i32, i32, i32, i32, i32, vp)
groupnorm_nhwc = _sig("fm_groupnorm_nhwc", vp, i32, vp, i32, vp, vp, vp, i32, vp, i32, i32, i32, i32, f32, i32, vp)
add_bf16 = _sig("fm_add_bf16", vp, i32, vp, i32, vp, i32, i64, i32, vp)
silu_f32_to_bf16 = _sig("fm_silu_f32_to_bf16", vp, vp, i64, vp)
timestep_embedding = _sig("fm_timestep_embedding", vp, vp, i32, i32, i32, f32, vp)
unet_attention = _sig("fm_unet_attention", vp, i32, vp, i32, i32, i32, i32, i32, vp)
unet_im2col_f32 = _sig("fm_unet_im2col_f32", vp, i32, i32, vp, i32, i32, i32, i32, vp, i32, i32, i32, i32, i32, i32, i32, i32, vp)
groupnorm_nhwc_f32 = _sig("fm_groupnorm_nhwc_f32", vp, i32, vp, i32, vp, vp, vp, i32, i32, i32, i32, i32, f32, i32, vp)
unet_attention_f32 = _sig("fm_unet_attention_f32", vp, i32, vp, i32, i32, i32, i32, i32, vp)
add_f32 = _sig("fm_add_f32", vp, i32, vp, i32, vp, i32, i64, i32, vp)
silu_f32 = _sig("fm_silu_f32", vp, vp, i64, vp)
timestep_embedding_f32 = _sig("fm_timestep_embedding_f32", vp, vp, i32, i32, i32, f32, vp)
unet_col2im_f32 = _sig("fm_unet_col2im_f32", vp, i32, vp, i32, i32, i32, i32, i32, i32, i32, i32, i32, vp)
groupnorm_nhwc_bwd_f32 = _sig("fm_groupnorm_nhwc_bwd_f32", vp, i32, vp, i32, vp, i32, vp, vp, vp, i32, vp, vp, vp, i32, vp, i32, i32, i32, i32, f32, i32, vp)
unet_attention_bwd_f32 = _sig("fm_unet_attention_bwd_f32", vp, i32, vp, i32, vp, i32, vp, i32, i32, i32, i32, vp)
silu_bwd_f32 = _sig("fm_silu_bwd_f32", vp, vp, vp, i64, vp)
diffusion_x0 = _sig("fm_diffusion_x0", vp, vp, f32, f32, vp, i64, vp)
quantile_abs = _sig("fm_quantile_abs", vp, i32, i64, f32, vp, vp)
diffusion_step = _sig("fm_diffusion_step", vp, vp, f32, f32, vp, vp, vp, f32, f32, f32, f32, vp, vp, i32, i64, vp)
lora_apply = _sig("fm_lora_apply", vp, i32, vp, i64, i64, vp, i64, i64, vp, i32, f32, vp, i32, i32, i32, i32, i32, i32, vp)
lora_grad = _sig("fm_lora_grad", vp, i32, vp, vp, i64, i64, f32, i32, i32, i32, i32, i32, vp)
vit_patch_rows = _sig("fm_vit_patch_rows", vp, vp, i32, i32, i32, i32, i32, i32, i32, vp)
vit_emb_rows = _sig("fm_vit_emb_rows", vp, vp, vp, i32, i32, i32, i32, vp)
vit_colsum = _sig("fm_vit_colsum", vp, i32, vp, i32, i32, vp, i64, vp)
clip_embed_ln = _sig("fm_clip_embed_ln", vp, i32, i32, vp, vp, vp, vp, vp, i32, i32, i32, i32, f32, vp)
FEAT_COSINE, FEAT_L1 = 0, 1
feat_distance = _sig("fm_feat_distance", vp, i32, vp, i32, i32, i32, i32, i32, vp, vp, i32, vp)
quick_gelu_bwd = _sig("fm_quick_gelu_bwd", vp, i32, vp, i32, vp, i32, i32, i32, i32, vp)
quick_gelu_bwd_f32 = _sig("fm_quick_gelu_bwd_f32", vp, i32, vp, i32, vp, i32, i32, i32, vp)
clip_embed_ln_bwd = _sig("fm_clip_embed_ln_bwd", vp, i32, vp, i32, i32, vp, vp, vp, i32, i32, i32, i32, f32, vp)
tap_add = _sig("fm_tap_add", vp, i32, vp, i32, vp, i32, vp, i32, i32, i32, vp)
LPIPS_CHUNK = 64
lpips_stem = _sig("fm_lpips_stem", vp, vp, vp, vp, vp, vp, i32, i32, i32, i32, i32, vp)
lpips_stem_bwd = _sig("fm_lpips_stem_bwd", vp, i32, i32, vp, vp, vp, vp, i32, i32, i32, vp)
maxpool2x2_nhwc = _sig("fm_maxpool2x2_nhwc", vp, i32, vp, i32, i32, i32, i32, i32, i32, vp)
lpips_distance = _sig("fm_lpips_distance", vp, i32, vp, i32, i32, vp, i32, i32, i32, vp, vp, i32, vp, vp)
lpips_tap_bwd = _sig("fm_lpips_tap_bwd", vp, i32, vp, i32, vp, i32, vp, i32, vp, i32, i32, i32, i32, i32, i32, vp)
LOSS_MSE, LOSS_L1, LOSS_SMOOTH_L1, LOSS_CE_INDEX, LOSS_BCE, LOSS_COSINE, LOSS_COSINE_1D = 0, 1, 2, 3, 4, 5, 6
RECONST_CHUNK, EMA_CHUNK, TOKEN_USAGE_MAX_K = 4096, 4096, 1 << 20
reconst_loss_scratch = _sig("fm_reconst_loss_scratch", i32, i32, i32, i64)
reconst_loss = _sig("fm_reconst_loss", vp, vp, i32, i32, i32, i64, vp, vp, vp, vp)
scale_f32 = _sig("fm_scale_f32", vp, vp, i64, vp)
mask_out_samples = _sig("fm_mask_out_samples", vp, vp, f32, vp, i32, i32, i64, vp)
ema_update = _sig("fm_ema_update", vp, i32, i64, f32, f32, vp)
diffusion_pair = _sig("fm_diffusion_pair", vp, vp, vp, vp, vp, i32, vp, vp, i32, i64, vp)
token_usage = _sig("fm_token_usage", vp, i32, i64, i64, i32, vp, vp, vp)
METRIC_RAW, METRIC_DENORM, METRIC_SIGMOID_PRED = 0, 1, 2
METRIC_CHUNK, SSIM_TILE, SSIM_MAX_KERNEL = 4096, 32, 11
metric_sums_scratch = _sig("fm_metric_sums_scratch", i32, i32, i64)
metric_sums = _sig("fm_metric_sums", vp, vp, i32, i32, i32, i32, i64, i32, i32, f32, vp, vp, vp, vp)
ssim_scale_scratch = _sig("fm_ssim_scale_scratch", i32, i32, i32, i32, i32)
ssim_scale = _sig("fm_ssim_scale", vp, vp, i32, i32, i32, i32, i32, i32, i32, vp, i32, f32, f32, vp, vp, vp, vp)
avgpool2x2_pair = _sig("fm_avgpool2x2_pair", vp, vp, i32, i32, i32, i32, i32, i32, i32, vp, vp, vp)
token_histogram = _sig("fm_token_histogram", vp, i32, i64, i32, vp, vp, vp)
RESIZE_BILINEAR, RESIZE_BILINEAR_AA, RESIZE_NEAREST = 0, 1, 2
RESIZE_MAX_TAPS = 64
resize_axis_table = _sig("fm_resize_axis_table", i32, i32, i32, P(i32), P(i32), P(f32), P(C.c_double), P(i32), P(i32))
resize_bilinear_fwd = _sig("fm_resize_bilinear_fwd", vp, vp, i32, i32, i32, i32, i32, vp, vp, vp, i32, vp, vp, vp, i32, vp, vp, i32, vp)
resize_bilinear_bwd = _sig("fm_resize_bilinear_bwd", vp, vp, i32, i32, i32, i32, i32, vp, vp, vp, i32, vp, vp, vp, vp, vp, i32, vp, vp, vp, i32, vp)
resize_nearest = _sig("fm_resize_nearest", vp, vp, i32, i32, i32, i32, i32, i32, vp, vp, vp)
PIL_NEAREST, PIL_BILINEAR, PIL_BICUBIC = 0, 1, 2
PIL_MAX_TAPS = 1024
pil_axis_table = _sig("fm_pil_axis_table", i32, i32, i32, P(i32), P(i32), P(i32))
pil_crop_resize = _sig("fm_pil_crop_resize", P(PilCropJob), vp, i32, vp, i64, vp, i64, vp, i64, i32, i32, i32, vp, vp, vp, vp, i64, vp)
pil_axis_table_f64 = _sig("fm_pil_axis_table_f64", i32, i32, i32, P(i32), P(i32), P(C.c_double))
pil_crop_resize16 = _sig("fm_pil_crop_resize16", P(PilCropJob), vp, i32, vp, i64, vp, i64, vp, i64, i32, vp, vp, i64, vp)
depth_standardize = _sig("fm_depth_standardize", vp, i32, i64, i64, i64, vp, vp, vp)
EXPORTS = ["fm_pil_axis_table_f64", "fm_pil_crop_resize16", "fm_depth_standardize", "fm_pil_axis_table", "fm_pil_crop_resize", "fm_resize_axis_table", "fm_resize_bilinear_fwd", "fm_resize_bilinear_bwd", "fm_resize_nearest","fm_metric_sums_scratch", "fm_metric_sums", "fm_ssim_scale_scratch", "fm_ssim_scale", "fm_avgpool2x2_pair", "fm_token_histogram",
           "fm_reconst_loss_scratch", "fm_reconst_loss", "fm_scale_f32", "fm_mask_out_samples", "fm_ema_update", "fm_diffusion_pair", "fm_token_usage", "fm_lpips_stem", "fm_lpips_stem_bwd", "fm_maxpool2x2_nhwc", "fm_lpips_distance", "fm_lpips_tap_bwd", "fm_feat_distance", "fm_quick_gelu_bwd", "fm_quick_gelu_bwd_f32", "fm_clip_embed_ln_bwd", "fm_tap_add", "fm_clip_embed_ln", "fm_attn_decode", "fm_vit_patch_rows", "fm_vit_emb_rows", "fm_vit_colsum", "fm_lora_apply", "fm_lora_grad", "fm_vq_assign_wide", "fm_memcodes_assign", "fm_convnext_block", "fm_split3_bf16", "fm_unet_im2col", "fm_groupnorm_nhwc", "fm_add_bf16", "fm_silu_f32_to_bf16", "fm_timestep_embedding", "fm_unet_attention", "fm_diffusion_x0", "fm_quantile_abs",
           "fm_diffusion_step", "fm_unpack_image_u8", "fm_unpack_ids_u16", "fm_unpack_mask_bits", "fm_decoder_attention_from_target", "fm_guidance_combine", "fm_image_mask", "fm_token_budgets", "fm_span_mask", "fm_vq_code_stats", "fm_vq_ema_update", "fm_vq_code_bias", "fm_vq_assign_bias", "fm_vq_code_stats_raw", "fm_vq_ema_update_euclid", "fm_vq_unpatchify", "fm_vq_latent_grad", "fm_tanh_bwd_f32", "fm_embed_rows_f32", "fm_vq_patchify_ex", "fm_vq_cls_emb_bwd", "fm_vq_latent_grad_normalized", "fm_abi_version", "fm_last_error", "fm_gemm_nt", "fm_set_gemm_nt_config", "fm_get_gemm_nt_config", "fm_set_reserved_cus", "fm_get_reserved_cus", "fm_bf16_to_f32_scaled", "fm_add_bf16_f32", "fm_scale_rows_bf16", "fm_gemm_tn", "fm_gemm_tn_multi", "fm_set_gemm_tn_config", "fm_get_gemm_tn_config", "fm_set_tn_transpose_read",
           "fm_get_tn_transpose_read", "fm_layernorm_fwd", "fm_layernorm_fwd_res", "fm_layernorm_bwd", "fm_layernorm_bwd_h", "fm_headnorm_fwd", "fm_headnorm_bwd", "fm_attn_fwd", "fm_attn_bwd",
           "fm_set_attn_transpose_read", "fm_get_attn_transpose_read", "fm_select_embed", "fm_embed_bwd",
           "fm_dense_decoder_mask", "fm_segment_rows", "fm_gather_rows", "fm_cross_entropy", "fm_swiglu_bwd",
           "fm_gelu_bwd", "fm_cast_pad", "fm_transpose_cast_pad", "fm_shadow_refresh", "fm_fold_colscale_grad", "fm_colsum", "fm_f32_to_bf16", "fm_adamw", "fm_adamw_shadow",
           "fm_sumsq", "fm_clip_coef", "fm_vq_patchify", "fm_l2norm_rows", "fm_vq_assign",
           "fm_sample_tokens", "fm_maskgit_commit", "fm_gemm_f32", "fm_attn_f32_fwd", "fm_attn_f32_bwd", "fm_layernorm_bwd_f32", "fm_headnorm_f32_fwd", "fm_headnorm_f32_bwd",
           "fm_swiglu_bwd_f32", "fm_gelu_bwd_f32", "fm_colsum_f32", "fm_cross_entropy_f32", "fm_lab_set",
           "fm_unet_im2col_f32", "fm_groupnorm_nhwc_f32", "fm_unet_attention_f32", "fm_add_f32", "fm_silu_f32", "fm_timestep_embedding_f32",
           "fm_unet_col2im_f32", "fm_groupnorm_nhwc_bwd_f32", "fm_unet_attention_bwd_f32", "fm_silu_bwd_f32"]


def check(rc: int):
    if rc != 0:
        raise RuntimeError(f"libfourm_hip: {lib.fm_last_error().decode()} (rc={rc})")
```

ml-4m_amd/fourm/hip/engine.py:

```python
import math
import os
import random
import weakref
from typing import Dict, List, Optional

import torch
import torch.nn as nn

from . import _lib as L
from . import ops

_WEIGHT_EPOCH = 0
FUSE_ACT_BWD = os.environ.get("FOURM_FUSE_ACT_BWD", "0") == "1"
HEADS_DENSE = os.environ.get("FOURM_HEADS_DENSE", "1") == "1"
HEADS_DENSE_MAX = int(os.environ.get("FOURM_HEADS_DENSE_MAX", "8"))
DEFER_RESIDUAL = os.environ.get("FOURM_DEFER_RESIDUAL", "1") == "1"
HOIST_CTX = os.environ.get("FOURM_HOIST_CTX", "1") == "1"
LN_BWD_FROM_H = os.environ.get("FOURM_LN_BWD_FROM_H", "1") == "1"
DP_RESERVE_ALWAYS = os.environ.get("FOURM_DP_RESERVE_ALWAYS", "0") == "1"


def bump_weight_epoch():
    global _WEIGHT_EPOCH
    _WEIGHT_EPOCH += 1


def ru(x, m):
    return (x + m - 1) // m * m


def is_lora(lin) -> bool:
    return hasattr(lin, "lora_down")


def check_lora_targets(model):
    from fourm.models.lora_utils import MAX_LORA_WIDTH, LoRAWrapper
    ok = set()
    for blk in model.encoder:
        ok |= {id(blk.attn.qkv), id(blk.attn.proj)}
    for blk in getattr(model, "decoder", ()):
        ok |= {id(blk.self_attn.qkv), id(blk.self_attn.proj), id(blk.cross_attn.q), id(blk.cross_attn.kv), id(blk.cross_attn.proj)}
    for name, mod in model.named_modules():
        if not isinstance(mod, LoRAWrapper):
            continue
        if id(mod) not in ok:
            raise NotImplementedError(f"LoRA wrapper at '{name}': the HIP engine adapts the attention Linears of the encoder / decoder blocks only "
                                      "(the MLP's fc1 / fc3 run as one launch whose SwiGLU epilogue consumes the pre-activation; embeddings and "
                                      "heads have no low-rank path)")
        width = mod.lora_down.weight.shape[0]
        if width > MAX_LORA_WIDTH:
            raise NotImplementedError(f"LoRA wrapper at '{name}': rank x packed Linears = {width} exceeds {MAX_LORA_WIDTH}")


class Shadow:
    __slots__ = ("buf", "params", "jobs", "stamp")

    def __init__(self, buf, params, jobs):
        self.buf, self.params, self.jobs, self.stamp = buf, params, jobs, None


class Workspace:

    def __init__(self, device, per_stream: bool = False):
        self.device = device
        self.per_stream = per_stream
        self.bufs: Dict[tuple, torch.Tensor] = {}

    def get(self, name, shape, dtype):
        key = (name, tuple(shape), dtype, torch.cuda.current_stream(self.device).cuda_stream) if self.per_stream else (name, tuple(shape), dtype)
        t = self.bufs.get(key)
        if t is None:
            t = self.bufs[key] = torch.zeros(shape, dtype=dtype, device=self.device)
        return t

    def nbytes(self):
        return sum(t.numel() * t.element_size() for t in self.bufs.values())


def fill_mod_desc(md, d, emb, is_dec: bool, mod_id: int, head_index: int = 0, raw: int = 0, name: str = "modality"):
    kind = emb.kind
    t = d["tensor"]
    B = t.shape[0]
    mask = d["target_mask" if is_dec else "input_mask"]
    mask = mask.reshape(B, -1)
    if mask.dtype != torch.bool:
        mask = mask.bool()
    mask = mask.contiguous()
    keep = [mask]
    md.mask, md.mask_stride = mask.data_ptr(), mask.shape[1]
    md.kind, md.mod_id, md.head_index = kind, mod_id, head_index
    md.pos = emb.pos_emb.data_ptr()
    md.mod_emb = emb.mod_emb.data_ptr()
    md.shifted = 1 if (is_dec and kind == L.KIND_SEQ and raw != 2) else 0
    md.max_len = getattr(emb, "max_length", 0) or 0
    if kind in (L.KIND_TOK, L.KIND_SEQ):
        ids = t.reshape(B, -1)
        if ids.dtype not in (torch.int32, torch.int64):
            ids = ids.long()
        ids = ids.contiguous()
        keep.append(ids)
        md.ids, md.ids_are_i64, md.id_stride = ids.data_ptr(), 1 if ids.dtype == torch.int64 else 0, ids.shape[1]
        md.table = emb.token_emb.weight.data_ptr()
        md.L = ids.shape[1] - (1 if md.shifted else 0)
        if ids.shape[1] != mask.shape[1]:
            raise ValueError(f"{name}: tensor has {ids.shape[1]} positions but the mask has {mask.shape[1]}")
    elif kind == L.KIND_PATCH:
        px = t.float().contiguous()
        keep.append(px)
        _, C, Hh, Ww = px.shape
        ps = emb.patch_size[0]
        md.ids, md.id_stride = px.data_ptr(), C * Hh * Ww
        md.patch, md.channels, md.grid_w = ps, C, Ww // ps
        md.L = (Hh // ps) * (Ww // ps)
    else:
        e = t.float().contiguous()
        keep.append(e)
        md.ids, md.id_stride, md.orig_dim = e.data_ptr(), e.shape[1] * e.shape[2], e.shape[2]
        md.proj_bias = emb.emb_proj.bias.data_ptr()
        md.L = e.shape[1]
    if is_dec and (raw != 2 or "decoder_attention_mask" in d):
        dam = d["decoder_attention_mask"].reshape(B, -1)
        if dam.dtype != torch.int32:
            dam = dam.int()
        dam = dam.contiguous()
        keep.append(dam)
        md.dam = dam.data_ptr()
    return keep


class FourMEngine:
    _pending = None
    _drop_now = None
    drop_uniforms = None

    def __init__(self, model):
        from fourm.models.fm_utils import GatedMlp, NormAttention, act_name
        self.model = model
        check_lora_targets(model)
        self.D = model.dim
        blk = model.encoder[0] if len(model.encoder) else model.decoder[0]
        attn0 = blk.attn if hasattr(blk, "attn") else blk.self_attn
        self.H = attn0.num_heads
        if self.D // self.H != 64:
            raise NotImplementedError(f"head_dim {self.D // self.H}: the HIP attention kernels are built for head_dim 64")
        self.qk_norm = isinstance(attn0, NormAttention)
        self.gated = isinstance(blk.mlp, GatedMlp)
        self.act = act_name(blk.mlp.act)
        if self.gated and self.act != "silu":
            raise NotImplementedError("gated MLP is implemented for SiLU (SwiGLU) only")
        if not self.gated and self.act != "gelu":
            raise NotImplementedError("plain MLP is implemented for exact GELU only")
        self.Hd = blk.mlp.hidden_features
        self.Hp = ru(self.Hd, 64)
        self.scale = 64 ** -0.5
        self.eps = blk.norm1.eps
        prec = getattr(model, "compute_precision", None) or os.environ.get("FOURM_PRECISION", "bf16")
        if prec not in ("bf16", "fp32"):
            raise ValueError(f"compute_precision {prec!r}: 'bf16' or 'fp32'")
        self.fp32 = prec == "fp32"
        self.adt = torch.float32 if self.fp32 else torch.bfloat16
        self.ws: Optional[Workspace] = None
        self.shadows: Dict[tuple, Shadow] = {}
        self._shadow_table = None
        self.flat_params = self.flat_grads = None
        self._slices = {}
        self._ctx = None
        self._dw_jobs = None
        self._pending = None
        self.reducer = None

    @property
    def checkpointing(self):
        return bool(getattr(self.model, "use_act_checkpoint", False))

    @property
    def device(self):
        t = getattr(self.model, "mask_token", None)
        return (t if t is not None else next(self.model.parameters())).device

    def _unique_params(self):
        seen, out = set(), []
        for n, p in getattr(self.model, "engine_parameters", self.model.named_parameters)():
            if id(p) not in seen:
                seen.add(id(p))
                out.append((n, p))
        return out

    def flatten(self):
        named = self._unique_params()
        dev = self.device

        def nodecay(n):
            return "norm." in n or ".norm" in n or n.endswith(".bias")
        late = {id(b.cross_attn.kv.weight) for b in self.model.decoder} if self.hoist_ctx else set()
        named.sort(key=lambda np_: (nodecay(np_[0]), id(np_[1]) in late))
        off, slices = 0, {}
        for n, p in named:
            slices[id(p)] = (off, p.numel())
            off += ru(p.numel(), 16)
        flat = torch.zeros(off, dtype=torch.float32, device=dev)
        for n, p in named:
            o, k = slices[id(p)]
            flat[o:o + k].copy_(p.data.reshape(-1))
            p.data = flat[o:o + k].view(p.shape)
        self.flat_params, self._slices = flat, slices
        self.flat_grads = torch.zeros_like(flat)
        self._named = named
        bump_weight_epoch()

    def _ensure_flat(self):
        if self.flat_params is None or self.flat_params.device != self.device:
            self.flatten()
            return
        for n, p in self._named[:4] + self._named[-4:]:
            o, k = self._slices[id(p)]
            if p.data_ptr() != self.flat_params.data_ptr() + 4 * o:
                self.flatten()
                return

    def grad_stages(self):
        m = self.model
        owner = {}

        def claim(stage, module_or_params):
            ps = module_or_params.parameters() if isinstance(module_or_params, nn.Module) else module_or_params
            for p in ps:
                owner[id(p)] = stage
        for i, blk in enumerate(m.decoder):
            claim(f"dec{i}", blk)
        if self.hoist_ctx:
            claim("dec_emb", [b.cross_attn.kv.weight for b in m.decoder] + [b.context_norm.weight for b in m.decoder])
        claim("heads", [m.decoder_norm.weight] + ([m.decoder_norm.bias] if isinstance(m.decoder_norm.bias, nn.Parameter) else []))
        claim("dec_emb", m.decoder_embeddings)
        claim("dec_emb", [m.mask_token])
        claim("ctx", m.decoder_proj_context)
        claim("ctx", m.encoder_norm)
        for i, blk in enumerate(m.encoder):
            claim(f"enc{i}", blk)
        claim("enc_emb", m.encoder_embeddings)
        if m.register_tokens is not None:
            claim("enc_emb", [m.register_tokens])
        stages = {}
        for n, p in self._named:
            o, k = self._slices[id(p)]
            stage = owner.get(id(p), "enc_emb") if k >= 65536 else "tail"
            stages.setdefault(stage, []).append((o, ru(k, 16)))
        return stages

    def _stage(self, name):
        if self.reducer is not None:
            self.reducer.stage_done(name)

    def grad_view(self, p):
        o, k = self._slices[id(p)]
        return self.flat_grads[o:o + k].view(p.shape)

    def grads_were_cleared(self) -> bool:
        live = getattr(self, "_attached", None)
        if not live:
            return True
        for p in live[:4] + live[-4:]:
            if p.grad is None or p.grad.data_ptr() != self.grad_view(p).data_ptr():
                return True
        return False

    def untouched_params(self):
        c = self._ctx
        if c is None or self.reducer is not None:
            return []
        m, touched, cand = self.model, set(), []
        for names, embs in ((c["enc"]["names"], m.encoder_embeddings), (c["dec"]["names"], m.decoder_embeddings)):
            for n, e in embs.items():
                if n in names:
                    touched.update(id(p) for p in e.parameters())
                else:
                    cand.extend(e.parameters())
        return [p for p in cand if id(p) not in touched]

    def attach_grads(self, zero: bool, untouched=()):
        if zero:
            with ops._prof("fills"):
                self.flat_grads.zero_()
            self._window_touched = set()
        skip = {id(p) for p in untouched} - getattr(self, "_window_touched", set())
        self._attached = []
        for n, p in self._named:
            if not p.requires_grad:
                continue
            if id(p) in skip:
                p.grad = None
                continue
            self._window_touched.add(id(p))
            p.grad = self.grad_view(p)
            self._attached.append(p)

    def _stamp(self, params):
        return tuple((p._version, _WEIGHT_EPOCH, p.data_ptr()) for p in params)

    def _get_shadow(self, key, make) -> torch.Tensor:
        s = self.shadows.get(key)
        if s is None:
            s = self.shadows[key] = make()
            for p in s.params:
                regs = getattr(p, "_fourm_shadows", None)
                if regs is None:
                    regs = p._fourm_shadows = []
                regs.append((weakref.ref(self), key))
        if s.stamp != self._stamp(s.params):
            self._refresh_shadows()
        return s.buf

    def _refresh_shadows(self):
        stale = [s for s in self.shadows.values() if s.stamp != self._stamp(s.params)]
        jobs = []
        for s in stale:
            jobs += [(j[0].detach().reshape(j[0].shape[0], -1), j[1], j[2], j[3].detach() if len(j) > 3 and j[3] is not None else None) for j in s.jobs]
        sig = tuple((a.data_ptr(), b.data_ptr(), tr, sc.data_ptr() if sc is not None else 0) for (a, b, tr, sc) in jobs)
        if self._shadow_table is None or self._shadow_table[0] != sig:
            table, tiles = ops.shadow_jobs_table(jobs, self.device)
            self._shadow_table = (sig, table, len(jobs), tiles)
        _, table, n, tiles = self._shadow_table
        ops.shadow_refresh(table, n, tiles)
        for s in stale:
            s.stamp = self._stamp(s.params)

    def mark_shadows_fresh(self, keys, written):
        for key in keys:
            s = self.shadows.get(key)
            if s is not None and all(len(j) == 3 and (id(j[0]), j[1].data_ptr()) in written for j in s.jobs):
                s.stamp = self._stamp(s.params)

    def w(self, p, pad_rows=False):
        if self.fp32:
            return p.detach().reshape(p.shape[0], -1)
        def make():
            out_f, in_f = p.shape[0], p[0].numel()
            buf = torch.zeros(ru(out_f, 64) if pad_rows else out_f, ru(in_f, 64), dtype=torch.bfloat16, device=p.device)
            return Shadow(buf, (p,), [(p, buf, False)])
        s = self._get_shadow(("w", id(p)), make)
        assert not pad_rows or s.shape[0] >= ru(p.shape[0], 64), "w(): the cached image was created without pad_rows"
        return s

    def wt(self, p, pad_rows=False):
        if self.fp32:
            return p.detach().reshape(p.shape[0], -1).t()
        def make():
            out_f, in_f = p.shape[0], p[0].numel()
            buf = torch.zeros(ru(in_f, 64) if pad_rows else in_f, ru(out_f, 64), dtype=torch.bfloat16, device=p.device)
            return Shadow(buf, (p,), [(p, buf, True)])
        s = self._get_shadow(("wt", id(p)), make)
        assert not pad_rows or s.shape[0] >= ru(p[0].numel(), 64), "wt(): the cached image was created without pad_rows"
        return s

    def w_fold(self, lin, norm):
        p, g = lin.weight, norm.weight
        def make():
            out_f, in_f = p.shape
            buf = torch.zeros(out_f, in_f if self.fp32 else ru(in_f, 64), dtype=self.adt, device=p.device)
            return Shadow(buf, (p, g), [(p, buf, False, g)])
        return self._get_shadow(("wfold", id(p)), make)

    def wt_fold_stack(self):
        m, D = self.model, self.D
        def make():
            Ld = len(m.decoder)
            buf = torch.zeros(D, Ld * 2 * D, dtype=self.adt, device=self.device)
            ps, jobs = [], []
            for i, blk in enumerate(m.decoder):
                p, g = blk.cross_attn.kv.weight, blk.context_norm.weight
                ps += [p, g]
                jobs.append((p, buf[:, i * 2 * D:(i + 1) * 2 * D], True, g))
            return Shadow(buf, tuple(ps), jobs)
        return self._get_shadow(("wtfold", 0), make)

    @property
    def hoist_ctx(self):
        h = getattr(self, "_hoist_ctx", None)
        if h is None:
            dec = getattr(self.model, "decoder", ())
            h = HOIST_CTX and len(dec) > 0 and all(
                not isinstance(b.context_norm.bias, nn.Parameter) and b.cross_attn.kv.bias is None and not is_lora(b.cross_attn.kv)
                for b in dec)
            self._hoist_ctx = h
        return h

    def w13t(self, mlp):
        def make():
            buf = torch.zeros(self.D, 2 * self.Hp, dtype=torch.bfloat16, device=self.device)
            p1, p3 = mlp.fc1.weight, mlp.fc3.weight
            return Shadow(buf, (p1, p3), [(p1, buf[:, :self.Hp], True), (p3, buf[:, self.Hp:], True)])
        return self._get_shadow(("w13t", id(mlp)), make)

    def _mod_desc(self, md: L.ModDesc, name, d, emb, is_dec, head_index=0, raw=0):
        return fill_mod_desc(md, d, emb, is_dec, int(self.model.modality_info[name]["id"]), head_index, raw, name)

    def select(self, mod_dict, n_keep: int, is_dec: bool, order: List[str], prefix: str, want_x0=True, heads=None, raw=0):
        m = self.model
        embs = m.decoder_embeddings if is_dec else m.encoder_embeddings
        names = [n for n in order if n in embs]
        if not names:
            raise ValueError("no modality of mod_dict is known to the model")
        if len(names) > L.FM_MAX_MODS:
# ... 267 lines not shown
    def decoder_mask(self, cs, mod_pre):
        m = self.model
        return dict(mask_kind=L.MASK_DECODER, cs=None if m.decoder_causal_mask else cs, causal=m.decoder_causal_mask,
                    modq=mod_pre if m.decoder_sep_mask else None, modk=mod_pre if m.decoder_sep_mask else None)

    def encode_context(self, enc, st=None):
        m = self.model
        save = st is not None
        B, N = enc["B"], enc["Nt"]
        emask = self.keypad(enc["mask"])
        x = enc["x0"]
        ckpt = save and self.checkpointing
        for i, blk in enumerate(m.encoder):
            if ckpt:
                st["enc_layers"].append(dict(ckpt_in=x))
                x = self.encoder_block_fwd(blk, x, B, N, emask, None, f"enc{i % 2}", defer_out=True, out_name=f"enc{i}.x_out")
                st["enc_layers"][-1]["dp"] = self._last_dp
                continue
            sv = {} if save else None
            x = self.encoder_block_fwd(blk, x, B, N, emask, sv, f"enc{i}" if save else f"enc{i % 2}", defer_out=True)
            if save:
                st["enc_layers"].append(sv)
        R, Rp, D = B * N, x.shape[0], self.D
        sv_top = {} if save else None
        xn = self._ln(m.encoder_norm, x, self._buf(sv_top, "top", "xn", (Rp, D), self.adt), R, sv_top, "en", "top")
        ctx = self._buf(sv_top, "top", "ctx", (Rp, D), torch.float32)
        pc = m.decoder_proj_context
        ops.gemm_nt(xn, self.w(pc.weight), ctx, epilogue=L.EPI_RESIDUAL, res=enc["emb"], bias=pc.bias, M=R, N=D, K=D)
        return x, ctx, emask, sv_top

    def trunk_forward(self, enc, dec, save: bool):
        m = self.model
        B, N, Mt = enc["B"], enc["Nt"], dec["Nt"]
        st = dict(enc_layers=[], dec_layers=[]) if save else None
        x, ctx, emask, sv_top = self.encode_context(enc, st)
        y = dec["x0"]
        smask = self.decoder_mask(dec["cs"], dec["mod_pre"]) if "cs" in dec else dec["sa_mask"]
        ctx_hat, sv_hat = None, None
        if self.hoist_ctx:
            sv_hat = {} if save else None
            ctx_hat = self._ln(self._unit_norm(), ctx, self._buf(sv_hat, "top", "ctx_hat", (ctx.shape[0], self.D), self.adt), B * N, sv_hat, "ch", "top")
        for i, blk in enumerate(m.decoder):
            if save and self.checkpointing:
                st["dec_layers"].append(dict(ckpt_in=y))
                y = self.decoder_block_fwd(blk, y, ctx, B, Mt, N, smask, emask, None, f"dec{i % 2}", defer_out=i + 1 < len(m.decoder),
                                           out_name=f"dec{i}.y_out", ctx_hat=ctx_hat)
                st["dec_layers"][-1]["dp"] = self._last_dp
                continue
            sv = {} if save else None
            y = self.decoder_block_fwd(blk, y, ctx, B, Mt, N, smask, emask, sv, f"dec{i}" if save else f"dec{i % 2}",
                                       defer_out=i + 1 < len(m.decoder), ctx_hat=ctx_hat)
            if save:
                st["dec_layers"].append(sv)
        if save:
            st.update(top=sv_top, x_final=x, y_final=y, ctx=ctx, emask=emask, smask=smask, ctx_hat=ctx_hat, sv_hat=sv_hat)
        return y, st

    def heads_setup(self, dec, y_final, save):
        m = self.model
        heads = dec["heads"]
        nH = len(heads)
        B, Mt, D = dec["B"], dec["Nt"], self.D
        R = B * Mt
        Rp = ops.padded_rows(R, nH)
        ws, dev, i32 = self.ws, self.device, torch.int32
        hs = dict(n=nH, Rp=Rp, heads=heads)
        hs["seg_start"], hs["seg_count"] = ws.get("heads.seg_start", (nH,), i32), ws.get("heads.seg_count", (nH,), i32)
        hs["perm"], hs["r2p"] = ws.get("heads.perm", (Rp,), i32), ws.get("heads.r2p", (R,), i32)
        hs["tile_group"] = ws.get("heads.tile_group", (Rp // ops.SEG,), i32)
        ops.segment_rows(dec["head_of_row"].view(-1), nH, hs["seg_start"], hs["seg_count"], hs["perm"], hs["r2p"], hs["tile_group"])
        sv = {} if save else None
        yp = ws.get("heads.yp", (Rp, D), self.adt)
        with ops._prof("fills"):
            yp.zero_()
        self._ln(m.decoder_norm, y_final, yp, R, sv, "dn", "heads", row_map=hs["r2p"])
        vocabs = [m.decoder_embeddings[h].vocab_size for h in heads]
        hs["vocabs"], hs["maxV"] = vocabs, max(vocabs)
        ldl = ru(hs["maxV"], 64)
        w_fwd = [self.w(m.decoder_embeddings[h].to_logits.weight) for h in heads]
        w_bwd = [self.wt(m.decoder_embeddings[h].to_logits.weight) for h in heads] if save else None
        key = tuple(t.data_ptr() for t in w_fwd) + (tuple(t.data_ptr() for t in w_bwd) if save else ())
        cache = getattr(self, "_head_groups", None)
        if cache is None or cache[0] != key:
            fwd = ops.make_groups([dict(W=t, N=v, K=D, ldw=D) for t, v in zip(w_fwd, vocabs)], dev)
            if self.fp32:
                bwd = ops.make_groups([dict(W=m.decoder_embeddings[h].to_logits.weight, N=D, K=v, ldw=D, transposed=1)
                                       for h, v in zip(heads, vocabs)], dev) if save else None
            else:
                bwd = ops.make_groups([dict(W=t, N=D, K=ru(v, 64), ldw=ru(v, 64)) for t, v in zip(w_bwd, vocabs)], dev) if save else None
            vt = torch.tensor(vocabs, dtype=i32, device=dev)
            self._head_groups = cache = (key, fwd, bwd, vt)
        hs["g_fwd"], hs["g_bwd"], hs["vocab_t"] = cache[1], cache[2], cache[3]
        logits = ws.get("heads.logits", (Rp, ldl), self.adt)
        if HEADS_DENSE and not self.fp32 and nH <= HEADS_DENSE_MAX and ops.heads_dense_ok(w_fwd, vocabs, logits):
            ops.gemm_nt_heads(yp, w_fwd, vocabs, hs["seg_start"], hs["seg_count"], logits, D)
        else:
            ops.gemm_nt_grouped(yp, hs["g_fwd"], hs["tile_group"], logits, hs["maxV"], max_K=D)
        hs.update(yp=yp, logits=logits, sv=sv)
        hs["row_loss"] = ws.get("heads.row_loss", (Rp,), torch.float32)
        hs["row_lse"] = ws.get("heads.row_lse", (Rp,), torch.float32)
        hs["head_loss"] = ws.get("heads.head_loss", (nH,), torch.float32)
        hs["total"] = ws.get("heads.total", (1,), torch.float32)
        return hs

    def loss_forward(self, dec, hs, loss_type):
        lt = L.LOSS_MOD if loss_type in ("mod", "modality") else L.LOSS_TOKEN
        hs["loss_type"] = lt
        ops.cross_entropy(hs["logits"], hs["perm"], hs["tile_group"], dec["target_ids"].view(-1), hs["vocab_t"], hs["seg_start"],
                          hs["seg_count"], hs["n"], hs["maxV"], hs["row_loss"], hs["row_lse"], hs["head_loss"], hs["total"], loss_type=lt)
        return hs["total"], hs["head_loss"]

    def dec_order(self, mod_dict):
        names = [n for n in mod_dict if n in self.model.decoder_embeddings]
        return random.sample(names, len(names))

    def train_forward(self, mod_dict, n_enc, n_dec, loss_type, save=True):
        if loss_type not in ("mod", "modality", "token"):
            raise ValueError("Invalid loss type")
        self.prepare()
        if save:
            self._ensure_flat()
        enc_names = [n for n in mod_dict if n in self.model.encoder_embeddings]
        enc = self.select(mod_dict, n_enc, False, enc_names, "enc.")
        dec = self.select(mod_dict, n_dec, True, self.dec_order(mod_dict), "dec.")
        y, st = self.trunk_forward(enc, dec, save)
        hs = self.heads_setup(dec, y, save)
        total, head_loss = self.loss_forward(dec, hs, loss_type)
        if save:
            self._ctx = dict(enc=enc, dec=dec, st=st, hs=hs)
        return total, head_loss, hs["heads"], hs["seg_count"]

    def _g(self, p):
        return self.grad_view(p) if p.requires_grad else None

    def _dW(self, dy, x, lin, R64, n_cols=None, dy_cols=None):
        g = self._g(lin.weight)
        N = lin.weight.shape[0] if n_cols is None else n_cols
        if g is not None:
            if self._dw_jobs is not None:
                self._dw_jobs.append((dy, x, g.view(g.shape[0], -1), N, lin.weight[0].numel(), R64))
            else:
                ops.gemm_tn(dy, x, g.view(g.shape[0], -1), N=N, K=lin.weight[0].numel(), R=R64)
        if lin.bias is not None and lin.bias.requires_grad:
            ops.colsum(dy, self.grad_view(lin.bias), N, R=R64)

    def _flush_dW(self):
        jobs, self._dw_jobs = self._dw_jobs, None
        if jobs:
            ops.gemm_tn_multi(jobs)

    def _ln_bwd(self, norm, dy, x, sv, key, g, g_bf, R, dres, dy_row_map=None):
        dw = self._g(norm.weight)
        db = self._g(norm.bias) if isinstance(norm.bias, nn.Parameter) else None
        ops.layernorm_bwd(dy, x, norm.weight, sv[key + ".mu"], sv[key + ".rs"], g, dres=dres, dx_bf16=g_bf, dw=dw, db=db,
                          dy_row_map=dy_row_map, R=R, h=sv.get(key + ".h"))

    def _mlp_bwd(self, mlp, sv, g_bf, R, Rp):
        bf, D, Hp, Hd = self.adt, self.D, self.Hp, self.Hd
        R64 = R
        ws = self.ws
        self._dW(g_bf, sv["act"], mlp.fc2, R64)
        dh = ws.get("bwd.dh", (Rp, D), bf)
        fuse = FUSE_ACT_BWD and self.act != "quick_gelu"
        if not fuse:
            da = ws.get("bwd.da", (Rp, Hp), bf)
            padN = not self.fp32 and Hp != Hd
            ops.gemm_nt(g_bf, self.wt(mlp.fc2.weight, padN), da, M=R, N=Hp if padN else Hd, K=D)
        if self.gated:
            dgu = ws.get("bwd.dgu", (Rp, 2 * Hp), bf)
            if fuse:
                ops.gemm_nt(g_bf, self.wt(mlp.fc2.weight), dgu, M=R, N=Hd, K=D, epilogue=L.EPI_SWIGLU_BWD, res=sv["gu"], Hp=Hp)
            else:
                ops.swiglu_bwd(da, sv["gu"], dgu, Hd, Hp, R=R)
            self._dW(dgu[:, :Hp], sv["h2"], mlp.fc1, R64, n_cols=Hd)
            self._dW(dgu[:, Hp:], sv["h2"], mlp.fc3, R64, n_cols=Hd)
            if self.fp32:
                ops.gemm_nt(dgu[:, :Hp], self.wt(mlp.fc1.weight), dh, M=R, N=D, K=Hd)
                ops.gemm_nt(dgu[:, Hp:], self.wt(mlp.fc3.weight), dh, M=R, N=D, K=Hd, epilogue=L.EPI_F32, res=dh)
            else:
                ops.gemm_nt(dgu, self.w13t(mlp), dh, M=R, N=D, K=2 * Hp)
        else:
            dpre = ws.get("bwd.dpre", (Rp, Hp), bf)
            if fuse:
                ops.gemm_nt(g_bf, self.wt(mlp.fc2.weight), dpre, M=R, N=Hd, K=D, epilogue=L.EPI_GELU_BWD, res=sv["pre"])
            elif self.act == "quick_gelu":
                ops.quick_gelu_bwd(da, sv["pre"], dpre, Hd, Hp, R=R)
            else:
                ops.gelu_bwd(da, sv["pre"], dpre, Hd, Hp, R=R)
            self._dW(dpre, sv["h2"], mlp.fc1, R64, n_cols=Hd)
            ops.gemm_nt(dpre, self.wt(mlp.fc1.weight), dh, M=R, N=D, K=Hp)
        return dh

    def _self_attn_bwd(self, attn, sv, g_bf, B, N, R, Rp, mask):
        bf, D = self.adt, self.D
        R64, ws = R, self.ws
        self._dW(g_bf, sv["o"], attn.proj, R64)
        do = ws.get("bwd.do", (Rp, D), bf)
        ops.gemm_nt(g_bf, self.wt(attn.proj.weight), do, M=R, N=D, K=D)
        self._lora_bwd(attn.proj, g_bf, sv["o"], do, sv.get("lora.proj"), R)
        dqkv = ws.get("bwd.dqkv", (Rp, 3 * D), bf)
        qkv = sv["qkv"]
        if self.qk_norm:
            dqkn = ws.get("bwd.dqkn", (Rp, 2 * D), bf)
            ops.attn_bwd(sv["qkn.q"], sv["qkn.k"], qkv[:, 2 * D:], sv["o"], do, dqkn[:, :D], dqkn[:, D:], dqkv[:, 2 * D:],
                         B, self.H, N, N, self.scale, sv["sm"], sv["sl"], zero_attn=getattr(attn, "allow_zero_attn", False), **mask)
            self._qk_norm_bwd(attn, sv, "qkn", dqkn[:, :D], dqkn[:, D:], qkv[:, :D], qkv[:, D:2 * D], dqkv[:, :D], dqkv[:, D:2 * D], R, R)
        else:
            ops.attn_bwd(qkv[:, :D], qkv[:, D:2 * D], qkv[:, 2 * D:], sv["o"], do, dqkv[:, :D], dqkv[:, D:2 * D], dqkv[:, 2 * D:],
                         B, self.H, N, N, self.scale, sv["sm"], sv["sl"], zero_attn=getattr(attn, "allow_zero_attn", False), **mask)
        self._dW(dqkv, sv["h1"], attn.qkv, R64)
        dh = ws.get("bwd.dh", (Rp, D), bf)
        ops.gemm_nt(dqkv, self.wt(attn.qkv.weight), dh, M=R, N=D, K=3 * D)
        self._lora_bwd(attn.qkv, dqkv, sv["h1"], dh, sv.get("lora.qkv"), R)
        return dh

    def encoder_block_bwd(self, blk, sv, g, g_bf, B, N, mask):
        R, Rp = B * N, g.shape[0]
        self._dw_jobs = []
        dp = sv.get("dp")
        if dp:
            ops.scale_rows_bf16(g_bf, dp[1], N, R)
        dh = self._mlp_bwd(blk.mlp, sv, g_bf, R, Rp)
        g1 = self.ws.get("bwd.enc.gbf1", tuple(g_bf.shape), g_bf.dtype)
        self._ln_bwd(blk.norm2, dh, sv["x_mid"], sv, "n2", g, g1, R, dres=g)
        if dp:
            ops.scale_rows_bf16(g1, dp[0], N, R)
        dh = self._self_attn_bwd(blk.attn, sv, g1, B, N, R, Rp, mask)
        self._flush_dW()
        self._ln_bwd(blk.norm1, dh, sv["x_in"], sv, "n1", g, g_bf, R, dres=g)

    def decoder_block_bwd(self, blk, sv, g, g_bf, dctx, dctx_bf, ctx, B, M, N, sa_mask, xa_mask, hoist=None):
        bf, D = self.adt, self.D
        Rq, Rqp, Rc, Rcp = B * M, g.shape[0], B * N, ctx.shape[0]
        ws = self.ws
        self._dw_jobs = []
        g_in = g_bf
        dp = sv.get("dp")
        if dp:
            ops.scale_rows_bf16(g_in, dp[2], M, Rq)
        dh = self._mlp_bwd(blk.mlp, sv, g_in, Rq, Rqp)
        g_bf = ws.get("bwd.dec.gbf1", tuple(g_in.shape), g_in.dtype)
        self._ln_bwd(blk.norm2, dh, sv["y2"], sv, "n2", g, g_bf, Rq, dres=g)
        if dp:
            ops.scale_rows_bf16(g_bf, dp[1], M, Rq)
        xa = blk.cross_attn
        self._dW(g_bf, sv["o2"], xa.proj, Rq)
        do = ws.get("bwd.do", (Rqp, D), bf)
        ops.gemm_nt(g_bf, self.wt(xa.proj.weight), do, M=Rq, N=D, K=D)
        self._lora_bwd(xa.proj, g_bf, sv["o2"], do, sv.get("lora.proj2"), Rq)
        dq = ws.get("bwd.dq", (Rqp, D), bf)
        dkv = ws.get("bwd.dkv", (Rcp, 2 * D), bf) if hoist is None else hoist[0]
        kv = sv["kv"]
        if self.qk_norm:
            dqn = ws.get("bwd.dqn", (Rqp, D), bf)
            dkn = ws.get("bwd.dkn", (Rcp, D), bf)
            ops.attn_bwd(sv["xqkn.q"], sv["xqkn.k"], kv[:, D:], sv["o2"], do, dqn, dkn, dkv[:, D:], B, self.H, M, N, self.scale,
                         sv["sm2"], sv["sl2"], zero_attn=getattr(xa, "allow_zero_attn", False), **xa_mask)
            self._qk_norm_bwd(xa, sv, "xqkn", dqn, dkn, sv["q"], kv[:, :D], dq, dkv[:, :D], Rq, Rc)
        else:
            ops.attn_bwd(sv["q"], kv[:, :D], kv[:, D:], sv["o2"], do, dq, dkv[:, :D], dkv[:, D:], B, self.H, M, N, self.scale,
                         sv["sm2"], sv["sl2"], zero_attn=getattr(xa, "allow_zero_attn", False), **xa_mask)
        self._dW(dq, sv["hq"], xa.q, Rq)
        dhq = ws.get("bwd.dh", (Rqp, D), bf)
        ops.gemm_nt(dq, self.wt(xa.q.weight), dhq, M=Rq, N=D, K=D)
        self._lora_bwd(xa.q, dq, sv["hq"], dhq, sv.get("lora.q"), Rq)
        g_bf = ws.get("bwd.dec.gbf2", tuple(g_in.shape), g_in.dtype)
        self._ln_bwd(blk.query_norm, dhq, sv["y1"], sv, "nq", g, g_bf, Rq, dres=g)
        if dp:
            ops.scale_rows_bf16(g_bf, dp[0], M, Rq)
        if hoist is None:
            self._dW(dkv, sv["hc"], xa.kv, Rc)
            dhc = ws.get("bwd.dhc", (Rcp, D), bf)
            ops.gemm_nt(dkv, self.wt(xa.kv.weight), dhc, M=Rc, N=D, K=2 * D)
            self._lora_bwd(xa.kv, dkv, sv["hc"], dhc, sv.get("lora.kv"), Rc)
            self._ln_bwd(blk.context_norm, dhc, ctx, sv, "nc", dctx, dctx_bf, Rc, dres=dctx)
        elif xa.kv.weight.requires_grad or blk.context_norm.weight.requires_grad:
            self._dw_jobs.append((dkv, hoist[1], hoist[2], 2 * D, D, Rc))
        dh = self._self_attn_bwd(blk.self_attn, sv, g_bf, B, M, Rq, Rqp, sa_mask)
        self._flush_dW()
        self._ln_bwd(blk.norm1, dh, sv["y_in"], sv, "n1", g, g_in, Rq, dres=g)

    def _embed_bwd(self, sel, dx, dx_extra, is_dec):
        m = self.model
        embs = m.decoder_embeddings if is_dec else m.encoder_embeddings
        d = L.EmbedBwdDesc()
        for i, n in enumerate(sel["names"]):
            e, md = embs[n], d.mods[i]
            md.kind = e.kind
            if e.kind in (L.KIND_TOK, L.KIND_SEQ) and not (is_dec and e.kind == L.KIND_TOK):
                w = e.token_emb.weight
                md.d_table = self.grad_view(w).data_ptr() if w.requires_grad else None
                pad = e.token_emb.padding_idx
                md.has_padding_idx, md.padding_idx = (1, pad) if pad is not None else (0, 0)
            if isinstance(e.pos_emb, nn.Parameter) and e.pos_emb.requires_grad:
                md.d_pos = self.grad_view(e.pos_emb).data_ptr()
            if e.mod_emb.requires_grad:
                md.d_mod_emb = self.grad_view(e.mod_emb).data_ptr()
            if e.kind == L.KIND_SEQ_EMB and e.emb_proj.bias.requires_grad:
                md.d_proj_bias = self.grad_view(e.emb_proj.bias).data_ptr()
        d.dx, d.lddx = dx.data_ptr(), dx.stride(0)
        d.slot_mod, d.slot_src, d.slot_pos = sel["slot_mod"].data_ptr(), sel["slot_src"].data_ptr(), sel["slot_pos"].data_ptr()
        if is_dec and m.mask_token.requires_grad:
            d.d_mask_token = self.grad_view(m.mask_token).data_ptr()
        if not is_dec and m.num_register_tokens and m.register_tokens.requires_grad:
            d.d_reg_tokens = self.grad_view(m.register_tokens).data_ptr()
        d.n_mods, d.batch, d.dim, d.Nt, d.is_decoder = len(sel["names"]), sel["B"], self.D, sel["Nt"], 1 if is_dec else 0
        with ops._prof("embed_bwd"):
            L.check(L.embed_bwd(ops.C.byref(d), ops._stream()))
        if dx_extra is not None:
            d2 = L.EmbedBwdDesc()
            ops.C.memmove(ops.C.byref(d2), ops.C.byref(d), ops.C.sizeof(d))
            for i in range(d.n_mods):
                d2.mods[i].d_table = None
                d2.mods[i].d_proj_bias = None
            d2.d_reg_tokens = None
            d2.dx, d2.lddx = dx_extra.data_ptr(), dx_extra.stride(0)
            with ops._prof("embed_bwd"):
                L.check(L.embed_bwd(ops.C.byref(d2), ops._stream()))

    def train_backward(self, grad_scale: torch.Tensor):
        c = self._ctx
        if c is None:
            raise RuntimeError("train_backward without a preceding training forward")
        self._ctx, self._dw_jobs = None, None
        if self.reducer is not None:
            self.reducer.begin()
            if getattr(self.reducer, "reserved_cus", 0):
                L.lib.fm_set_reserved_cus(int(self.reducer.reserved_cus))
        m, ws = self.model, self.ws
        enc, dec, st, hs = c["enc"], c["dec"], c["st"], c["hs"]
        B, N, Mt, D = enc["B"], enc["Nt"], dec["Nt"], self.D
        bf, f32 = self.adt, torch.float32
        Rq, Rc = B * Mt, B * N
        Rqp, Rcp = st["y_final"].shape[0], st["x_final"].shape[0]
        ops.cross_entropy(hs["logits"], hs["perm"], hs["tile_group"], dec["target_ids"].view(-1), hs["vocab_t"], hs["seg_start"],
                          hs["seg_count"], hs["n"], hs["maxV"], hs["row_loss"], hs["row_lse"], hs["head_loss"], hs["total"],
                          loss_type=hs["loss_type"], grad_scale=grad_scale, write_grad=True)
        dyp = ws.get("bwd.dyp", (hs["Rp"], D), bf)
        ops.gemm_nt_grouped(hs["logits"], hs["g_bwd"], hs["tile_group"], dyp, D, max_K=ru(hs["maxV"], 64))
        heads = [m.decoder_embeddings[h] for h in hs["heads"]]
        if any(h.to_logits.weight.requires_grad for h in heads):
            outs = [self.grad_view(h.to_logits.weight) if h.to_logits.weight.requires_grad else None for h in heads]
            key = tuple(o.data_ptr() if o is not None else 0 for o in outs)
            cache = getattr(self, "_head_tn_groups", None)
            if cache is None or cache[0] != key:
                cache = self._head_tn_groups = (key, ops.make_groups(
                    [dict(out=o, N=(v if o is not None else 0)) for o, v in zip(outs, hs["vocabs"])], self.device))
            tn = cache[1]
            ops.gemm_tn_grouped(hs["logits"], hs["yp"], tn, hs["seg_start"], hs["seg_count"], hs["n"], hs["maxV"], hs["Rp"], D)
        g = ws.get("bwd.g_dec", (Rqp, D), f32)
        g_bf = ws.get("bwd.g_dec_bf", (Rqp, D), bf)
        self._ln_bwd(m.decoder_norm, dyp, st["y_final"], hs["sv"], "dn", g, g_bf, Rq, dres=None, dy_row_map=hs["r2p"])
        self._stage("heads")
        dctx = ws.get("bwd.dctx", (Rcp, D), f32)
        dctx_bf = ws.get("bwd.dctx_bf", (Rcp, D), bf)
        Ld = len(m.decoder)
        ctx_hat = st.get("ctx_hat")
        if ctx_hat is None:
            with ops._prof("fills"):
                dctx.zero_()
        else:
            dkv_all = ws.get("bwd.dkv_all", (Rcp, Ld * 2 * D), bf)
            dwp = ws.get("bwd.dwp", (Ld, 2 * D, D), f32)
            with ops._prof("fills"):
                dwp.zero_()
        for i in reversed(range(Ld)):
            sv = st["dec_layers"][i]
            if "ckpt_in" in sv:
                y_in, dp, sv = sv["ckpt_in"], sv["dp"], {}
                self.decoder_block_fwd(m.decoder[i], y_in, st["ctx"], B, Mt, N, st["smask"], st["emask"], sv, "ckpt", out_name="ckpt.out", dp=dp,
                                       ctx_hat=ctx_hat)
            hoist = None if ctx_hat is None else (dkv_all[:, i * 2 * D:(i + 1) * 2 * D], ctx_hat, dwp[i])
            self.decoder_block_bwd(m.decoder[i], sv, g, g_bf, dctx, dctx_bf, st["ctx"], B, Mt, N, st["smask"], st["emask"], hoist=hoist)
            self._stage(f"dec{i}")
        if ctx_hat is not None and Ld:
            dxh = ws.get("bwd.dhc", (Rcp, D), bf)
            ops.gemm_nt(dkv_all, self.wt_fold_stack(), dxh, M=Rc, N=D, K=Ld * 2 * D)
            self._ln_bwd(self._unit_norm(), dxh, st["ctx"], st["sv_hat"], "ch", dctx, dctx_bf, Rc, dres=None)
            jobs = [(dwp[i], b.cross_attn.kv.weight.detach(), b.context_norm.weight.detach(), self._g(b.cross_attn.kv.weight), self._g(b.context_norm.weight))
                    for i, b in enumerate(m.decoder) if b.cross_attn.kv.weight.requires_grad or b.context_norm.weight.requires_grad]
            if jobs:
                ops.fold_colscale_grad(jobs)
        self._embed_bwd(dec, g, None, True)
        self._stage("dec_emb")
        top = st["top"]
        if len(m.decoder) == 0:
            ops.f32_to_bf16(dctx, dctx_bf)
        self._dW(dctx_bf, top["xn"], m.decoder_proj_context, Rc)
        dxn = ws.get("bwd.dh", (Rcp, D), bf)
        ops.gemm_nt(dctx_bf, self.wt(m.decoder_proj_context.weight), dxn, M=Rc, N=D, K=D)
        ge = ws.get("bwd.g_enc", (Rcp, D), f32)
        ge_bf = ws.get("bwd.g_enc_bf", (Rcp, D), bf)
        self._ln_bwd(m.encoder_norm, dxn, st["x_final"], top, "en", ge, ge_bf, Rc, dres=None)
        self._stage("ctx")
        for i in reversed(range(len(m.encoder))):
            sv = st["enc_layers"][i]
            if "ckpt_in" in sv:
                x_in, dp, sv = sv["ckpt_in"], sv["dp"], {}
                self.encoder_block_fwd(m.encoder[i], x_in, B, N, st["emask"], sv, "ckpt", out_name="ckpt.out", dp=dp)
            self.encoder_block_bwd(m.encoder[i], sv, ge, ge_bf, B, N, st["emask"])
            self._stage(f"enc{i}")
        for n in enc["names"]:
            e = m.encoder_embeddings[n]
            if e.kind == L.KIND_PATCH and e.proj.weight.requires_grad:
                ops.gemm_tn(ge_bf, enc["patch_rows"], self.grad_view(e.proj.weight), N=D, K=e.proj.weight.shape[1], R=Rc)
            elif e.kind == L.KIND_SEQ_EMB and e.emb_proj.weight.requires_grad:
                ops.gemm_tn(ge_bf, enc["seqemb_rows"], self.grad_view(e.emb_proj.weight), N=D, K=e.emb_proj.weight.shape[1], R=Rc)
        self._embed_bwd(enc, ge, dctx, False)
        if self.reducer is not None:
            self.reducer.finish()
            if getattr(self.reducer, "reserved_cus", 0) and not DP_RESERVE_ALWAYS:
                L.lib.fm_set_reserved_cus(0)
```

ml-4m_amd/fourm/hip/ops.py:

```python
import contextlib
import ctypes as C
import threading
from typing import Optional

import torch

from . import _lib as L

_PROFILER = None


def set_profiler(p):
    global _PROFILER
    _PROFILER = p


class _Null:
    def __enter__(self):
        return self

    def __exit__(self, *a):
        return False


# ... 101 lines not shown


def _gemm_f32(x, w, out, *, epilogue=L.EPI_BF16, bias=None, res=None, w2=None, bias2=None, out2=None, Hp=0, N=None, K=None, M=None,
              accumulate=False):
    assert w.dtype == torch.float32 and out.dtype == torch.float32 and x.stride(1) == 1 and out.stride(1) == 1
    a = L.GemmF32Args()
    a.X, a.W, a.W2, a.out, a.out2, a.res, a.bias, a.bias2 = _p(x), _p(w), _p(w2), _p(out), _p(out2), _p(res), _p(bias), _p(bias2)
    a.M = x.shape[0] if M is None else M
    a.N = w.shape[0] if N is None else N
    a.K = min(w.shape[1] if K is None else K, w.shape[1])
    a.sxm, a.sxk, a.swn, a.swk = x.stride(0), 1, w.stride(0), w.stride(1)
    if w2 is not None:
        assert w2.stride() == w.stride()
    a.ldo, a.ldo2, a.ldr = out.stride(0), out2.stride(0) if out2 is not None else 0, res.stride(0) if res is not None else 0
    a.Hp, a.epilogue, a.accumulate = Hp, epilogue, 1 if accumulate else 0
    with _prof("gemm_f32", 2.0 * a.M * a.N * a.K * (2 if epilogue == L.EPI_SWIGLU else 1), 4.0 * (a.K * (a.M + a.N) + a.M * a.N), tag=f"M{a.M} N{a.N} K{a.K}"):
        L.check(L.gemm_f32(C.byref(a), _stream()))
    return out


@_timed("heads_gemm_nt (logits, dY)")
def gemm_nt_grouped(x, groups, tile_group, out, max_N, M=None, max_K=0):
    if x.dtype == torch.float32:
        a = L.GemmF32Args()
        a.X, a.out, a.groups, a.tile_group = _p(x), _p(out), _p(groups), _p(tile_group)
        a.M, a.N, a.max_N, a.seg_rows = (x.shape[0] if M is None else M), max_N, max_N, SEG
        a.sxm, a.sxk, a.ldo, a.epilogue = x.stride(0), 1, out.stride(0), L.EPI_BF16
        L.check(L.gemm_f32(C.byref(a), _stream()))
        return out
    a = L.GemmNTArgs()
    a.X, a.out = _p(x), _p(out)
    a.M = x.shape[0] if M is None else M
    a.K = max_K
    a.ldx, a.ldo = _ld(x), _ld(out)
    a.epilogue = L.EPI_BF16
    a.groups, a.tile_group, a.max_N = _p(groups), _p(tile_group), max_N
    L.check(L.gemm_nt(C.byref(a), _stream()))
    return out


def heads_dense_ok(ws, vocabs, out):
    return (out.dtype == torch.bfloat16 and all(v % 8 == 0 for v in vocabs) and all(w.dtype == torch.bfloat16 and w.shape[1] % 64 == 0 for w in ws)
            and _ld(out) % 64 == 0 and out.data_ptr() % 128 == 0)


@_timed("heads_gemm_nt (logits, dY)")
def gemm_nt_heads(x, ws, vocabs, seg_start, seg_count, out, K):
    for h, (w, v) in enumerate(zip(ws, vocabs)):
        a = L.GemmNTArgs()
        a.W, a.X, a.out = _p(w), _p(x), _p(out)
        a.M, a.N, a.K = x.shape[0], v, K
        a.ldw, a.ldx, a.ldo = _ld(w), _ld(x), _ld(out)
        a.epilogue = L.EPI_BF16
        a.m_dev, a.row0_dev = seg_count.data_ptr() + 4 * h, seg_start.data_ptr() + 4 * h
        L.check(L.gemm_nt(C.byref(a), _stream()))
    return out


def gemm_tn(a_mat, b_mat, out, *, N=None, K=None, R=None, splits=0, force_tr=-1, a_cols=0, b_cols=0):
    if a_mat.dtype == torch.float32:
        g = L.GemmF32Args()
        g.X, g.W, g.out = _p(a_mat), _p(b_mat), _p(out)
        g.M = a_mat.shape[1] if N is None else N
        g.N = b_mat.shape[1] if K is None else K
        g.K = a_mat.shape[0] if R is None else R
        g.sxm, g.sxk, g.swn, g.swk = 1, a_mat.stride(0), 1, b_mat.stride(0)
        g.ldo, g.epilogue, g.accumulate = _ld(out), L.EPI_BF16, 1
        L.check(L.gemm_f32(C.byref(g), _stream()))
        return out
    a = L.GemmTNArgs()
    a.A, a.B, a.out = _p(a_mat), _p(b_mat), _p(out)
    a.R = a_mat.shape[0] if R is None else R
    a.N = a_mat.shape[1] if N is None else N
    a.K = b_mat.shape[1] if K is None else K
    a.lda, a.ldb, a.ldo = _ld(a_mat), _ld(b_mat), _ld(out)
    a.a_cols = a_cols or a_mat.shape[1]
    a.b_cols = b_cols or b_mat.shape[1]
    a.splits, a.force_tr = splits, force_tr
    with _prof("gemm_tn", 2.0 * a.R * a.N * a.K, 2.0 * a.R * (a.N + a.K) + 4.0 * a.N * a.K, tag=f"R{a.R} N{a.N} K{a.K}"):
        L.check(L.gemm_tn(C.byref(a), _stream()))
    return out


def gemm_tn_multi(jobs):
    if not jobs:
        return
    if jobs[0][0].dtype == torch.float32:
        for a_mat, b_mat, out, N, K, R in jobs:
            gemm_tn(a_mat, b_mat, out, N=N, K=K, R=R)
        return
    for lo in range(0, len(jobs), L.TN_MAX_JOBS):
        part = jobs[lo:lo + L.TN_MAX_JOBS]
        arr = (L.GemmTNJob * len(part))()
        flops = 0.0
        for j, (a_mat, b_mat, out, N, K, R) in zip(arr, part):
            j.A, j.B, j.out = _p(a_mat), _p(b_mat), _p(out)
            j.R, j.N, j.K = R, N, K
            j.lda, j.ldb, j.ldo = _ld(a_mat), _ld(b_mat), _ld(out)
            j.a_cols, j.b_cols = a_mat.shape[1], b_mat.shape[1]
            flops += 2.0 * R * N * K
        with _prof("gemm_tn_multi", flops, 0.0, tag=f"jobs{len(part)} R{part[0][5]}"):
            L.check(L.gemm_tn_multi(arr, len(part), _stream()))


@_timed("heads_gemm_tn (dW)")
def gemm_tn_grouped(a_mat, b_mat, groups, seg_start, seg_count, n_groups, max_N, max_R, K, *, splits=0, force_tr=-1):
    if a_mat.dtype == torch.float32:
        g = L.GemmF32Args()
        g.X, g.W, g.groups, g.seg_start, g.seg_count = _p(a_mat), _p(b_mat), _p(groups), _p(seg_start), _p(seg_count)
        g.N, g.max_N, g.n_groups = K, max_N, n_groups
        g.sxm, g.sxk, g.swn, g.swk = 1, a_mat.stride(0), 1, b_mat.stride(0)
        g.ldo, g.epilogue, g.accumulate = K, L.EPI_BF16, 1
        L.check(L.gemm_f32(C.byref(g), _stream()))
        return
    a = L.GemmTNArgs()
    a.A, a.B = _p(a_mat), _p(b_mat)
    a.K = K
    a.lda, a.ldb, a.ldo = _ld(a_mat), _ld(b_mat), K
    a.a_cols, a.b_cols = a_mat.shape[1], b_mat.shape[1]
    a.splits, a.force_tr = splits, force_tr
    a.groups, a.seg_start, a.seg_count = _p(groups), _p(seg_start), _p(seg_count)
    a.n_groups, a.max_N, a.max_R = n_groups, max_N, max_R
    L.check(L.gemm_tn(C.byref(a), _stream()))


def make_groups(entries, device):
    arr = (L.GemmGroup * len(entries))()
    for i, e in enumerate(entries):
        arr[i].W = e["W"].data_ptr() if e.get("W") is not None else None
        arr[i].out = e["out"].data_ptr() if e.get("out") is not None else None
        arr[i].N, arr[i].K, arr[i].ldw = e["N"], e.get("K", 0), e.get("ldw", 0)
        arr[i].pad_ = e.get("transposed", 0)
    host = torch.frombuffer(bytearray(bytes(arr)), dtype=torch.uint8)
    return host.to(device)


def layernorm_fwd(x, w, b, y, mean=None, rstd=None, row_map=None, eps=1e-6, R=None, delta=None, x_out=None):
    R = x.shape[0] if R is None else R
    if delta is not None:
        with _prof("layernorm_fwd", 0.0, R * w.numel() * (10 + y.element_size())):
            L.check(L.layernorm_fwd_res(_p(x), _ld(x), _p(delta), _ld(delta), _p(x_out), _ld(x_out), _p(w), _p(b), _p(y), _ld(y),
                                        1 if y.dtype == torch.float32 else 0, _p(mean), _p(rstd), _p(row_map), R, w.numel(), eps, _stream()))
        return y
    with _prof("layernorm_fwd", 0.0, R * w.numel() * (4 + y.element_size())):
        return _ln_fwd(x, w, b, y, mean, rstd, row_map, eps, R)


def _ln_fwd(x, w, b, y, mean, rstd, row_map, eps, R):
    L.check(L.layernorm_fwd(_p(x), _ld(x), _p(w), _p(b), _p(y), _ld(y), 1 if y.dtype == torch.float32 else 0,
                            _p(mean), _p(rstd), _p(row_map), R, w.numel(), eps, _stream()))
    return y


def layernorm_bwd(dy, x, w, mean, rstd, dx, *, dres=None, dx_bf16=None, dw=None, db=None, dy_row_map=None, R=None, h=None):
    R = x.shape[0] if R is None else R
    if h is not None and dy.dtype != torch.float32 and db is None and dy_row_map is None:
        with _prof("layernorm_bwd", 0.0, R * w.numel() * (2 + 2 + 4 + 4 + (2 if dx_bf16 is not None else 0))):
            L.check(L.layernorm_bwd_h(_p(dy), _ld(dy), _p(h), _ld(h), _p(x), _ld(x), _p(w), _p(mean), _p(rstd), _p(dres), _p(dx), _ld(dx),
                                      _p(dx_bf16), _ld(dx_bf16) if dx_bf16 is not None else 0, _p(dw), R, w.numel(), _stream()))
        return dx
    with _prof("layernorm_bwd", 0.0, R * w.numel() * (2 + 4 + 4 + 4 + (2 if dx_bf16 is not None else 0))):
        return _ln_bwd(dy, x, w, mean, rstd, dx, dres, dx_bf16, dw, db, dy_row_map, R)


def _ln_bwd(dy, x, w, mean, rstd, dx, dres, dx_bf16, dw, db, dy_row_map, R):
    if dy.dtype == torch.float32:
        L.check(L.layernorm_bwd_f32(_p(dy), _ld(dy), _p(dy_row_map), _p(x), _ld(x), _p(w), _p(mean), _p(rstd), _p(dres), _p(dx), _ld(dx),
                                    _p(dx_bf16), _ld(dx_bf16) if dx_bf16 is not None else 0, _p(dw), _p(db), R, w.numel(), _stream()))
        return dx
    L.check(L.layernorm_bwd(_p(dy), _ld(dy), _p(dy_row_map), _p(x), _ld(x), _p(w), _p(mean), _p(rstd), _p(dres), _p(dx), _ld(dx),
                            _p(dx_bf16), _ld(dx_bf16) if dx_bf16 is not None else 0, _p(dw), _p(db), R, w.numel(), _stream()))
    return dx


@_timed("headnorm")
def headnorm_fwd(x, w, b, y, stats, R, H, eps):
    if x.dtype == torch.float32:
        return L.check(L.headnorm_f32_fwd(_p(x), _ld(x), _p(w), _p(b), _p(y), _ld(y), _p(stats), R, H, eps, _stream()))
    L.check(L.headnorm_fwd(_p(x), _ld(x), _p(w), _p(b), _p(y), _ld(y), _p(stats), R, H, eps, _stream()))


@_timed("headnorm")
def headnorm_bwd(dy, x, w, stats, dx, dw, db, R, H):
    if x.dtype == torch.float32:
        return L.check(L.headnorm_f32_bwd(_p(dy), _ld(dy), _p(x), _ld(x), _p(w), _p(stats), _p(dx), _ld(dx), _p(dw), _p(db), R, H, _stream()))
    L.check(L.headnorm_bwd(_p(dy), _ld(dy), _p(x), _ld(x), _p(w), _p(stats), _p(dx), _ld(dx), _p(dw), _p(db), R, H, _stream()))


def _attn_args(q, k, v, o, B, H, Nq, Nk, scale, mask_kind, kpad, cs, modq, modk, dense, causal, stat_m, stat_l, force_tr, zero_attn=False):
    a = L.AttnArgs()
    a.Q, a.K, a.V, a.O = _p(q), _p(k), _p(v), _p(o)
    a.ldq, a.ldk, a.ldv, a.ldo = q.stride(0), k.stride(0), v.stride(0), o.stride(0)
    a.B, a.H, a.Nq, a.Nk, a.head_dim, a.mask_kind = B, H, Nq, Nk, 64, mask_kind
    a.scale, a.causal = scale, 1 if causal else 0
    a.kpad, a.cs, a.modq, a.modk, a.dense = _p(kpad), _p(cs), _p(modq), _p(modk), _p(dense)
    a.stat_m, a.stat_l = _p(stat_m), _p(stat_l)
    a.force_tr, a.zero_attn = force_tr, 1 if zero_attn else 0
    return a


def attn_fwd(q, k, v, o, B, H, Nq, Nk, scale, *, mask_kind=L.MASK_NONE, kpad=None, cs=None, modq=None, modk=None, dense=None,
             causal=False, stat_m=None, stat_l=None, force_tr=-1, kv_batch_rows=0, zero_attn=False):
    a = _attn_args(q, k, v, o, B, H, Nq, Nk, scale, mask_kind, kpad, cs, modq, modk, dense, causal, stat_m, stat_l, force_tr, zero_attn)
    a.kv_batch_rows = kv_batch_rows
    if q.dtype == torch.float32:
        L.check(L.attn_f32_fwd(C.byref(a), _stream()))
        return o
    with _prof("attn_fwd", 4.0 * B * H * Nq * Nk * 64):
        L.check(L.attn_fwd(C.byref(a), _stream()))
    return o


@_timed("attn_decode")
def attn_decode(q, k, v, o, B, H, Nk, scale, *, kv_batch_rows=0, k_new_row=-1, q_norm=None, k_norm=None, eps=1e-6, kpad=None, zero_attn=False):
    a = L.AttnDecodeArgs()
    a.q, a.k, a.v, a.o = _p(q), _p(k), _p(v), _p(o)
    if not (q.dtype == k.dtype == v.dtype == o.dtype) or q.dtype not in (torch.bfloat16, torch.float32):
        raise TypeError("attn_decode: q, k, v, o must share one of bf16 / fp32")
    for w in (q_norm or ()) + (k_norm or ()):
        if w is not None and (w.dtype != torch.float32 or w.numel() != 64 or not w.is_contiguous()):
            raise TypeError("attn_decode: norm vectors are contiguous fp32 (64)")
    a.q_w, a.q_b = (_p(q_norm[0]), _p(q_norm[1])) if q_norm is not None else (None, None)
    a.k_w, a.k_b = (_p(k_norm[0]), _p(k_norm[1])) if k_norm is not None else (None, None)
    if kpad is not None and (kpad.dtype not in (torch.bool, torch.uint8) or kpad.shape != (B, Nk) or not kpad.is_contiguous()):
        raise TypeError("attn_decode: kpad is a contiguous (B, Nk) bool / uint8 tensor")
    a.kpad = _p(kpad)
    a.ldq, a.ldk, a.ldv, a.ldo = _ld(q), _ld(k), _ld(v), _ld(o)
    a.B, a.H, a.Nk, a.kv_batch_rows, a.k_new_row = B, H, Nk, kv_batch_rows, k_new_row
    a.is_f32, a.zero_attn, a.scale, a.eps = int(q.dtype == torch.float32), 1 if zero_attn else 0, scale, eps
    L.check(L.attn_decode(C.byref(a), _stream()))
    return o


def attn_bwd(q, k, v, o, do, dq, dk, dv, B, H, Nq, Nk, scale, stat_m, stat_l, *, mask_kind=L.MASK_NONE, kpad=None, cs=None,
             modq=None, modk=None, dense=None, causal=False, force_tr=-1, zero_attn=False):
    a = _attn_args(q, k, v, o, B, H, Nq, Nk, scale, mask_kind, kpad, cs, modq, modk, dense, causal, stat_m, stat_l, force_tr, zero_attn)
    a.dO, a.dQ, a.dK, a.dV = _p(do), _p(dq), _p(dk), _p(dv)
    a.lddo, a.lddq, a.lddk, a.lddv = do.stride(0), dq.stride(0), dk.stride(0), dv.stride(0)
    if q.dtype == torch.float32:
        dk.zero_(); dv.zero_()
        L.check(L.attn_f32_bwd(C.byref(a), _stream()))
        return
    with _prof("attn_bwd", 10.0 * B * H * Nq * Nk * 64):
        L.check(L.attn_bwd(C.byref(a), _stream()))


def padded_rows(R: int, n_heads: int) -> int:
    return ru(R, SEG) + SEG * (n_heads - 1)


@_timed("heads_misc")
def segment_rows(head_of_row, n_heads, seg_start, seg_count, perm, row_to_padded, tile_group):
    L.check(L.segment_rows(_p(head_of_row), head_of_row.numel(), n_heads, _p(seg_start), _p(seg_count), _p(perm),
                           _p(row_to_padded), _p(tile_group), perm.numel(), _stream()))


@_timed("heads_misc")
def gather_rows(src, perm, dst, D):
    L.check(L.gather_rows(_p(src), _ld(src), _p(perm), _p(dst), _ld(dst), perm.numel(), D, _stream()))


@_timed("cross_entropy")
def cross_entropy(logits, perm, tile_group, target_ids, vocab, seg_start, seg_count, n_heads, max_vocab, row_loss, row_lse, head_loss,
                  total_loss, *, loss_type=L.LOSS_MOD, grad_scale=None, write_grad=False):
    fn = L.cross_entropy_f32 if logits.dtype == torch.float32 else L.cross_entropy
    L.check(fn(_p(logits), _ld(logits), _p(perm), _p(tile_group), _p(target_ids), _p(vocab), _p(seg_start),
                            _p(seg_count), _p(grad_scale), loss_type, n_heads, perm.numel(), max_vocab, _p(row_loss), _p(row_lse),
                            _p(head_loss), _p(total_loss), 1 if write_grad else 0, _stream()))


@_timed("swiglu_bwd")
def swiglu_bwd(da, gu, dgu, H, Hp, R=None):
    if da.dtype == torch.float32:
        return L.check(L.swiglu_bwd_f32(_p(da), _ld(da), _p(gu), _ld(gu), _p(dgu), _ld(dgu), da.shape[0] if R is None else R, H, Hp, _stream()))
    L.check(L.swiglu_bwd(_p(da), _ld(da), _p(gu), _ld(gu), _p(dgu), _ld(dgu), da.shape[0] if R is None else R, H, Hp, _stream()))


@_timed("gelu_bwd")
def gelu_bwd(dh, pre, dpre, H, Hp, R=None):
    if dh.dtype == torch.float32:
        return L.check(L.gelu_bwd_f32(_p(dh), _ld(dh), _p(pre), _ld(pre), _p(dpre), _ld(dpre), dh.shape[0] if R is None else R, H, _stream()))
    L.check(L.gelu_bwd(_p(dh), _ld(dh), _p(pre), _ld(pre), _p(dpre), _ld(dpre), dh.shape[0] if R is None else R, H, Hp, _stream()))


@_timed("gelu_bwd")
def quick_gelu_bwd(da, pre, dpre, H, Hp, R=None):
    R = da.shape[0] if R is None else R
    if da.dtype == torch.float32:
        return L.check(L.quick_gelu_bwd_f32(_p(da), _ld(da), _p(pre), _ld(pre), _p(dpre), _ld(dpre), R, H, _stream()))
    L.check(L.quick_gelu_bwd(_p(da), _ld(da), _p(pre), _ld(pre), _p(dpre), _ld(dpre), R, H, Hp, _stream()))


def tap_add(g, dtap, g_bf=None, row_scale=None, rows_per_sample=0, R=None):
    R = g.shape[0] if R is None else R
    L.check(L.tap_add(_p(g), _ld(g), _p(g_bf), _ld(g_bf) if g_bf is not None else 0, _p(dtap), _ld(dtap), _p(row_scale), rows_per_sample, R, g.shape[1],
                      _stream()))
    return g


def feat_distance(pred, tgt, B, T, mode, loss, dpred):
    L.check(L.feat_distance(_p(pred), _ld(pred), _p(tgt), _ld(tgt), B, T, pred.shape[1], mode, _p(loss), _p(dpred), _ld(dpred), _stream()))
    return loss


def _is_f32(t):
    if t.dtype not in (torch.float32, torch.bfloat16):
        raise TypeError(f"feature rows are bf16 or f32, got {t.dtype}")
    return 1 if t.dtype == torch.float32 else 0


def lpips_stem(img, mul, add, w, bias, out, B, H, W):
    esz = out.element_size()
    with _prof("lpips_stem", 2.0 * B * H * W * 64 * 27, B * H * W * (12.0 + 64 * esz), tag=f"B{B} {H}x{W}"):
        L.check(L.lpips_stem(_p(img), _p(mul), _p(add), _p(w), _p(bias), _p(out), _ld(out), _is_f32(out), B, H, W, _stream()))
    return out


def lpips_stem_bwd(d, w, mul, row_scale, dimg, B, H, W):
    with _prof("lpips_stem_bwd", 2.0 * B * H * W * 64 * 27, B * H * W * (12.0 + 64 * d.element_size()), tag=f"B{B} {H}x{W}"):
        L.check(L.lpips_stem_bwd(_p(d), _ld(d), _is_f32(d), _p(w), _p(mul), _p(row_scale), _p(dimg), B, H, W, _stream()))
    return dimg


def maxpool2x2_nhwc(x, y, B, H, W, C):
    with _prof("maxpool2x2_nhwc", 0.0, 1.25 * B * H * W * C * x.element_size(), tag=f"B{B} {H}x{W} C{C}"):
# ... 391 lines not shown
```

Before: 1.156 million tokens/s.

## Replace atomic LayerNorm/embedding grad accumulation with per-workgroup partials and batched folds

Result: no change. 1.166 million tokens/s, median of 6 (+0.9%).

```diff
diff --git a/include/fourm_hip.h b/include/fourm_hip.h
--- a/include/fourm_hip.h
+++ b/include/fourm_hip.h
@@ -75,6 +75,19 @@
 int fm_layernorm_bwd_h(const void* dy, int lddy, const void* h, int ldh, const void* x, int ldx, const void* w,
                        const void* mean, const void* rstd, const void* dres, void* dx, int lddx, void* dx_bf16,
                        int lddxbf, void* dw, int R, int D, void* stream);
+int fm_layernorm_bwd_workgroups(int R);
+int fm_layernorm_bwd_parts(const void* dy, int lddy, const int32_t* dy_row_map, const void* x, int ldx, const void* w,
+                           const void* mean, const void* rstd, const void* dres, void* dx, int lddx, void* dx_bf16,
+                           int lddxbf, void* part_dw, void* part_db, int R, int D, void* stream);
+int fm_layernorm_bwd_h_parts(const void* dy, int lddy, const void* h, int ldh, const void* x, int ldx, const void* w,
+                             const void* mean, const void* rstd, const void* dres, void* dx, int lddx, void* dx_bf16,
+                             int lddxbf, void* part_dw, int R, int D, void* stream);
+#define FM_FOLD_PARTS_MAX_JOBS 16
+typedef struct fm_fold_parts_job {
+    const void* part; void* dst;
+    int32_t n_parts, D, ld, reserved;
+} fm_fold_parts_job;
+int fm_fold_partials(const fm_fold_parts_job* jobs, int n_jobs, void* stream);
 
 int fm_headnorm_fwd(const void* x, int ldx, const void* w, const void* b, void* y, int ldy, void* stats, int R, int H, float eps,
                     void* stream);
@@ -183,6 +196,8 @@
     int32_t n_mods, batch, dim, Nt, lddx, is_decoder;
 } fm_embed_bwd_desc;
 int fm_embed_bwd(const fm_embed_bwd_desc* desc, void* stream);
+int fm_embed_bwd_ws_scratch(const fm_embed_bwd_desc* desc);
+int fm_embed_bwd_ws(const fm_embed_bwd_desc* desc, const void* dx_extra, int lddx_extra, void* scratch, int64_t scratch_bytes, void* stream);
 
 int fm_dense_decoder_mask(const int32_t* cs, const int16_t* mod, void* out, int B, int M, int causal, int use_cs,
                           int use_sep, void* stream);
diff --git a/ml-4m_amd/csrc/layernorm.hip b/ml-4m_amd/csrc/layernorm.hip
--- a/ml-4m_amd/csrc/layernorm.hip
+++ b/ml-4m_amd/csrc/layernorm.hip
@@ -130,7 +130,8 @@
                                                      const float* __restrict__ x, int ldx, const float* __restrict__ w,
                                                      const float* __restrict__ mean, const float* __restrict__ rstd,
                                                      const float* dres, float* dx, int lddx, bf16_t* __restrict__ dx_bf, int lddxbf,
-                                                     float* __restrict__ dw, float* __restrict__ db, int R, int D, int BWD_ROWS, int nt_dx) {
+                                                     float* __restrict__ dw, float* __restrict__ db, int R, int D, int BWD_ROWS, int nt_dx,
+                                                     float* __restrict__ part_dw, float* __restrict__ part_db) {
     extern __shared__ __attribute__((aligned(16))) char smem[];
     float* red = (float*)smem;
     const int lane = threadIdx.x & 63, wave = threadIdx.x >> 6;
@@ -218,7 +219,7 @@
             }
         }
     }
-    if (!dw && !db) return;
+    if (!dw && !db && !part_dw && !part_db) return;
 #pragma unroll
     for (int c = 0; c < MAXC; ++c) {
         const int ch = lane + 64 * c;
@@ -229,8 +230,47 @@
     }
     __syncthreads();
     for (int i = threadIdx.x; i < D; i += 256) {
-        if (dw) unsafeAtomicAdd(dw + i, (red[i] + red[D + i]) + (red[2 * D + i] + red[3 * D + i]));
-        if constexpr (HAS_DB) if (db) unsafeAtomicAdd(db + i, (red[4 * D + i] + red[5 * D + i]) + (red[6 * D + i] + red[7 * D + i]));
+        const float sw = (red[i] + red[D + i]) + (red[2 * D + i] + red[3 * D + i]);
+        if (part_dw) part_dw[(size_t)blockIdx.x * D + i] = sw;
+        else if (dw) unsafeAtomicAdd(dw + i, sw);
+        if constexpr (HAS_DB) {
+            const float sb = (red[4 * D + i] + red[5 * D + i]) + (red[6 * D + i] + red[7 * D + i]);
+            if (part_db) part_db[(size_t)blockIdx.x * D + i] = sb;
+            else if (db) unsafeAtomicAdd(db + i, sb);
+        }
+    }
+}
+
+constexpr int FOLD_WAVES = 16;
+struct FoldPartsArgs { fm_fold_parts_job job[FM_FOLD_PARTS_MAX_JOBS]; };
+__global__ __launch_bounds__(64 * FOLD_WAVES) void fold_partials_kernel(FoldPartsArgs a) {
+    __shared__ float red[FOLD_WAVES][64];
+    const fm_fold_parts_job j = a.job[blockIdx.y];
+    const int lane = threadIdx.x & 63, wave = threadIdx.x >> 6;
+    const int c = blockIdx.x * 64 + lane;
+    if (blockIdx.x * 64 >= j.D) return;
+    const int per = (j.n_parts + FOLD_WAVES - 1) / FOLD_WAVES;
+    const int lo = min(j.n_parts, wave * per), hi = min(j.n_parts, lo + per);
+    float s = 0.f;
+    if (c < j.D) {
+        const float* p = (const float*)j.part + (size_t)lo * j.ld + c;
+        int i = lo;
+        for (; i + 8 <= hi; i += 8, p += (size_t)8 * j.ld) {
+            float v[8];
+#pragma unroll
+            for (int q = 0; q < 8; ++q) v[q] = p[(size_t)q * j.ld];
+#pragma unroll
+            for (int q = 0; q < 8; ++q) s += v[q];
+        }
+        for (; i < hi; ++i, p += j.ld) s += *p;
+    }
+    red[wave][lane] = s;
+    __syncthreads();
+    if (wave == 0 && c < j.D) {
+        float t = red[0][lane];
+#pragma unroll
+        for (int w = 1; w < FOLD_WAVES; ++w) t += red[w][lane];
+        ((float*)j.dst)[c] += t;
     }
 }
 
@@ -363,7 +403,7 @@
 
 static int layernorm_bwd_launch(const void* dy, int lddy, const int32_t* dy_row_map, const void* h, int ldh, const void* x, int ldx, const void* w,
                                 const void* mean, const void* rstd, const void* dres, void* dx, int lddx, void* dx_bf16,
-                                int lddxbf, void* dw, void* db, int R, int D, void* stream) {
+                                int lddxbf, void* dw, void* db, int R, int D, void* stream, void* part_dw = nullptr, void* part_db = nullptr) {
     FM_CHECK_ARG(dy && x && w && mean && rstd && dx, "fm_layernorm_bwd: null pointer");
     FM_CHECK_ARG(!h || ldh % 4 == 0, "fm_layernorm_bwd_h: ldh must be a multiple of 4");
     FM_CHECK_ARG(R > 0 && D > 0 && D % 4 == 0 && D <= 64 * 4 * MAXC_LIMIT, "fm_layernorm_bwd: D=%d unsupported", D);
@@ -378,7 +418,8 @@
         (void)once;                                                                                                         \
         hipLaunchKernelGGL(k, dim3(grid), dim3(256), lds, (hipStream_t)stream, (const bf16_t*)dy, lddy, dy_row_map, (const bf16_t*)h, ldh, \
                            (const float*)x, ldx, (const float*)w, (const float*)mean, (const float*)rstd, (const float*)dres, (float*)dx, lddx, \
-                           (bf16_t*)dx_bf16, lddxbf, (float*)dw, (float*)db, R, D, BWD_ROWS, ((ln_nt_flags() >> 1) & 1) | ((ln_nt_flags() >> 2) & 2) | ((ln_nt_flags() >> 2) & 4));                               \
+                           (bf16_t*)dx_bf16, lddxbf, (float*)dw, (float*)db, R, D, BWD_ROWS, ((ln_nt_flags() >> 1) & 1) | ((ln_nt_flags() >> 2) & 2) | ((ln_nt_flags() >> 2) & 4), \
+                           (float*)part_dw, (float*)part_db);                                                               \
     }
 #define LN_BWD(C) { if (h) LN_BWD_(C, true) else LN_BWD_(C, false) }
     switch (chunks_for(D)) {
@@ -404,6 +445,44 @@
                                   int lddxbf, void* dw, int R, int D, void* stream) {
     FM_CHECK_ARG(h, "fm_layernorm_bwd_h: null pointer");
     return layernorm_bwd_launch(dy, lddy, nullptr, h, ldh, x, ldx, w, mean, rstd, dres, dx, lddx, dx_bf16, lddxbf, dw, nullptr, R, D, stream);
+}
+
+extern "C" int fm_layernorm_bwd_workgroups(int R) {
+    if (R <= 0) return 0;
+    const int rows = bwd_rows(R);
+    return (R + rows - 1) / rows;
+}
+
+extern "C" int fm_layernorm_bwd_parts(const void* dy, int lddy, const int32_t* dy_row_map, const void* x, int ldx, const void* w,
+                                      const void* mean, const void* rstd, const void* dres, void* dx, int lddx, void* dx_bf16,
+                                      int lddxbf, void* part_dw, void* part_db, int R, int D, void* stream) {
+    FM_CHECK_ARG((((uintptr_t)part_dw | (uintptr_t)part_db) & 3) == 0, "fm_layernorm_bwd_parts: partial buffers must be 4-byte aligned");
+    return layernorm_bwd_launch(dy, lddy, dy_row_map, nullptr, 0, x, ldx, w, mean, rstd, dres, dx, lddx, dx_bf16, lddxbf, nullptr, nullptr, R, D, stream,
+                                part_dw, part_db);
+}
+
+extern "C" int fm_layernorm_bwd_h_parts(const void* dy, int lddy, const void* h, int ldh, const void* x, int ldx, const void* w,
+                                        const void* mean, const void* rstd, const void* dres, void* dx, int lddx, void* dx_bf16,
+                                        int lddxbf, void* part_dw, int R, int D, void* stream) {
+    FM_CHECK_ARG(h, "fm_layernorm_bwd_h_parts: null pointer");
+    FM_CHECK_ARG((((uintptr_t)part_dw) & 3) == 0, "fm_layernorm_bwd_h_parts: partial buffer must be 4-byte aligned");
+    return layernorm_bwd_launch(dy, lddy, nullptr, h, ldh, x, ldx, w, mean, rstd, dres, dx, lddx, dx_bf16, lddxbf, nullptr, nullptr, R, D, stream,
+                                part_dw, nullptr);
+}
+
+extern "C" int fm_fold_partials(const fm_fold_parts_job* jobs, int n_jobs, void* stream) {
+    FM_CHECK_ARG(jobs && n_jobs > 0 && n_jobs <= FM_FOLD_PARTS_MAX_JOBS, "fm_fold_partials: 1..FM_FOLD_PARTS_MAX_JOBS jobs");
+    FoldPartsArgs a;
+    int max_d = 0;
+    for (int i = 0; i < n_jobs; ++i) {
+        FM_CHECK_ARG(jobs[i].part && jobs[i].dst && jobs[i].n_parts > 0 && jobs[i].D > 0 && jobs[i].ld >= jobs[i].D, "fm_fold_partials: bad job %d", i);
+        FM_CHECK_ARG((((uintptr_t)jobs[i].part | (uintptr_t)jobs[i].dst) & 3) == 0, "fm_fold_partials: job %d is not 4-byte aligned", i);
+        a.job[i] = jobs[i];
+        max_d = std::max(max_d, jobs[i].D);
+    }
+    hipLaunchKernelGGL(fold_partials_kernel, dim3((max_d + 63) / 64, n_jobs), dim3(64 * FOLD_WAVES), 0, (hipStream_t)stream, a);
+    FM_CHECK_LAUNCH("fm_fold_partials");
+    return 0;
 }
 
 extern "C" int fm_headnorm_fwd(const void* x, int ldx, const void* w, const void* b, void* y, int ldy, void* stats, int R, int H, float eps,
diff --git a/ml-4m_amd/csrc/select_embed.hip b/ml-4m_amd/csrc/select_embed.hip
--- a/ml-4m_amd/csrc/select_embed.hip
+++ b/ml-4m_amd/csrc/select_embed.hip
@@ -1,3 +1,4 @@
+#include <algorithm>
 #include "common.h"
 #include "fourm_hip.h"
 
@@ -329,6 +330,108 @@
         for (int c = threadIdx.x; c < D; c += 256) unsafeAtomicAdd((float*)d.d_mask_token + c, acc[(size_t)d.n_mods * D + c]);
 }
 
+constexpr int EMB_WS_MAX_WG = 1024;
+template <int NK>
+__global__ __launch_bounds__(64) void embed_bwd_ws_kernel(fm_embed_bwd_desc d, const float* __restrict__ dx_extra, int lddx_extra,
+                                                          float* __restrict__ scratch, int per) {
+    extern __shared__ __attribute__((aligned(16))) char smem[];
+    float* acc = (float*)smem;
+    const int D = d.dim, lane = threadIdx.x;
+    const int rows = d.n_mods + 1;
+    for (int i = lane; i < rows * D; i += 64) acc[i] = 0.f;
+    __syncthreads();
+    float racc[NK];
+    int cur = -1;
+    bool cur_mask = false;
+    auto flush = [&]() {
+        if (cur < 0) return;
+#pragma unroll
+        for (int k = 0; k < NK; ++k) {
+            const int c = lane + 64 * k;
+            if (c >= D) break;
+            acc[(size_t)cur * D + c] += racc[k];
+            if (cur_mask) acc[(size_t)d.n_mods * D + c] += racc[k];
+        }
+    };
+    float nv[NK], ne[NK];
+#pragma unroll
+    for (int k = 0; k < NK; ++k) nv[k] = ne[k] = 0.f;
+    auto fetch = [&](long long row) {
+        const float* g = (const float*)d.dx + (size_t)row * d.lddx;
+        const float* gx = dx_extra ? dx_extra + (size_t)row * lddx_extra : nullptr;
+#pragma unroll
+        for (int k = 0; k < NK; ++k) {
+            const int c = lane + 64 * k;
+            if (c >= D) break;
+            nv[k] = g[c];
+            ne[k] = gx ? gx[c] : 0.f;
+        }
+    };
+    const long long total = (long long)d.batch * d.Nt;
+    const long long lo = (long long)blockIdx.x * per, hi = lo + per < total ? lo + per : total;
+    for (long long base = lo; base < hi; base += 64) {
+        const int n = (int)(hi - base < 64 ? hi - base : 64);
+        int my_m = -1, my_src = 0, my_pos = 0;
+        if (lane < n) {
+            my_m = ((const int32_t*)d.slot_mod)[base + lane];
+            my_src = ((const int32_t*)d.slot_src)[base + lane];
+            my_pos = ((const int32_t*)d.slot_pos)[base + lane];
+        }
+        unsigned long long live = __ballot(my_m != -1);
+        if (live) fetch(base + __builtin_ctzll(live));
+        while (live) {
+            const int i = __builtin_ctzll(live);
+            live &= live - 1;
+            float v[NK], e[NK];
+#pragma unroll
+            for (int k = 0; k < NK; ++k) { v[k] = nv[k]; e[k] = ne[k]; }
+            if (live) fetch(base + __builtin_ctzll(live));
+            const long long row = base + i;
+            const int m = __builtin_amdgcn_readfirstlane(__shfl(my_m, i, 64)), src = __builtin_amdgcn_readfirstlane(__shfl(my_src, i, 64)),
+                      posrow = __builtin_amdgcn_readfirstlane(__shfl(my_pos, i, 64));
+            if (m == -2) {
+                if (d.d_reg_tokens) {
+                    float* rrow = (float*)d.d_reg_tokens + (size_t)(row % d.Nt) * D;
+#pragma unroll
+                    for (int k = 0; k < NK; ++k) {
+                        const int c = lane + 64 * k;
+                        if (c >= D) break;
+                        unsafeAtomicAdd(rrow + c, v[k]);
+                    }
+                }
+                continue;
+            }
+            const fm_embed_bwd_mod& md = d.mods[m];
+            const bool to_mask_token = d.is_decoder && md.kind == FM_KIND_TOK;
+            if (m != cur) {
+                flush();
+                cur = m; cur_mask = to_mask_token;
+#pragma unroll
+                for (int k = 0; k < NK; ++k) racc[k] = 0.f;
+            }
+            float* trow = nullptr;
+            if (to_mask_token) {}
+            else if ((md.kind == FM_KIND_TOK || md.kind == FM_KIND_SEQ) && md.d_table && !(md.has_padding_idx && src == md.padding_idx))
+                trow = (float*)md.d_table + (size_t)src * D;
+            else if (md.kind == FM_KIND_SEQ_EMB && md.d_proj_bias) trow = (float*)md.d_proj_bias;
+            float* prow = md.d_pos ? (float*)md.d_pos + (size_t)posrow * D : nullptr;
+#pragma unroll
+            for (int k = 0; k < NK; ++k) {
+                const int c = lane + 64 * k;
+                if (c >= D) break;
+                const float t = dx_extra ? v[k] + e[k] : v[k];
+                racc[k] += t;
+                if (trow) unsafeAtomicAdd(trow + c, v[k]);
+                if (prow) unsafeAtomicAdd(prow + c, t);
+            }
+        }
+    }
+    flush();
+    __syncthreads();
+    float* out = scratch + (size_t)blockIdx.x * rows * D;
+    for (int i = lane; i < rows * D; i += 64) out[i] = acc[i];
+}
+
 __global__ void dense_decoder_mask_kernel(const int32_t* cs, const int16_t* mod, uint8_t* out, int B, int M, int causal, int use_cs, int use_sep) {
     const size_t i = (size_t)blockIdx.x * 256 + threadIdx.x;
     if (i >= (size_t)B * M * M) return;
@@ -390,6 +493,57 @@
     return 0;
 }
 
+static int embed_ws_per(const fm_embed_bwd_desc* d) {
+    const long long total = (long long)d->batch * d->Nt;
+    return (int)std::max<long long>(16, (total + EMB_WS_MAX_WG - 1) / EMB_WS_MAX_WG);
+}
+static int embed_ws_groups(const fm_embed_bwd_desc* d) {
+    const long long total = (long long)d->batch * d->Nt;
+    const int per = embed_ws_per(d);
+    return (int)((total + per - 1) / per);
+}
+
+extern "C" int fm_embed_bwd_ws_scratch(const fm_embed_bwd_desc* d) {
+    FM_CHECK_ARG(d && d->n_mods > 0 && d->n_mods <= FM_MAX_MODS && d->dim > 0 && d->dim <= 2048 && d->batch > 0 && d->Nt > 0, "fm_embed_bwd_ws_scratch: bad shape");
+    return (int)((size_t)embed_ws_groups(d) * (d->n_mods + 1) * d->dim * sizeof(float));
+}
+
+extern "C" int fm_embed_bwd_ws(const fm_embed_bwd_desc* d, const void* dx_extra, int lddx_extra, void* scratch, int64_t scratch_bytes, void* stream) {
+    FM_CHECK_ARG(d && d->dx && d->slot_mod && d->slot_src && d->slot_pos && scratch, "fm_embed_bwd_ws: null pointer");
+    FM_CHECK_ARG(d->n_mods > 0 && d->n_mods <= FM_MAX_MODS && d->dim > 0 && d->dim % 4 == 0 && d->dim <= 2048 && d->lddx % 4 == 0 && d->batch > 0 && d->Nt > 0,
+                 "fm_embed_bwd_ws: bad shape (dim <= 2048)");
+    FM_CHECK_ARG(!dx_extra || (lddx_extra >= d->dim && lddx_extra % 4 == 0), "fm_embed_bwd_ws: lddx_extra=%d must be a multiple of 4 and >= dim", lddx_extra);
+    const int rows = d->n_mods + 1;
+    const size_t lds = (size_t)rows * d->dim * sizeof(float);
+    FM_CHECK_ARG(lds <= 150 * 1024, "fm_embed_bwd_ws: %zu bytes of LDS needed", lds);
+    const int G = embed_ws_groups(d);
+    const size_t need = (size_t)G * rows * d->dim * sizeof(float);
+    FM_CHECK_ARG(scratch_bytes >= (int64_t)need && (((uintptr_t)scratch) & 3) == 0, "fm_embed_bwd_ws: %zu bytes of scratch needed (fm_embed_bwd_ws_scratch)", need);
+#define EMBED_WS(NK)                                                                                                                       \
+    {                                                                                                                                      \
+        auto k = embed_bwd_ws_kernel<NK>;                                                                                                  \
+        static bool once = (hipFuncSetAttribute((const void*)k, hipFuncAttributeMaxDynamicSharedMemorySize, 150 * 1024) == hipSuccess);  \
+        (void)once;                                                                                                                        \
+        hipLaunchKernelGGL(k, dim3(G), dim3(64), lds, (hipStream_t)stream, *d, (const float*)dx_extra, lddx_extra, (float*)scratch, embed_ws_per(d)); \
+    }
+    if (d->dim <= 256) EMBED_WS(4) else if (d->dim <= 768) EMBED_WS(12) else EMBED_WS(32)
+#undef EMBED_WS
+    FM_CHECK_LAUNCH("fm_embed_bwd_ws");
+    fm_fold_parts_job jobs[FM_MAX_MODS + 1];
+    int n = 0;
+    for (int m = 0; m <= d->n_mods; ++m) {
+        void* dst = m < d->n_mods ? d->mods[m].d_mod_emb : d->d_mask_token;
+        if (!dst) continue;
+        jobs[n].part = (const float*)scratch + (size_t)m * d->dim;
+        jobs[n].dst = dst;
+        jobs[n].n_parts = G; jobs[n].D = d->dim; jobs[n].ld = rows * d->dim; jobs[n].reserved = 0;
+        ++n;
+    }
+    for (int i = 0; i < n; i += FM_FOLD_PARTS_MAX_JOBS)
+        if (int rc = fm_fold_partials(jobs + i, std::min(n - i, FM_FOLD_PARTS_MAX_JOBS), stream)) return rc;
+    return 0;
+}
+
 extern "C" int fm_dense_decoder_mask(const int32_t* cs, const int16_t* mod, void* out, int B, int M, int causal, int use_cs, int use_sep, void* stream) {
     FM_CHECK_ARG(out && (causal || !use_cs || cs) && (!use_sep || mod), "fm_dense_decoder_mask: null pointer");
     const size_t n = (size_t)B * M * M;
diff --git a/ml-4m_amd/fourm/hip/_lib.py b/ml-4m_amd/fourm/hip/_lib.py
--- a/ml-4m_amd/fourm/hip/_lib.py
+++ b/ml-4m_amd/fourm/hip/_lib.py
@@ -93,6 +93,13 @@
 
 class FoldGradJob(C.Structure):
     _fields_ = [("dWp", vp), ("W", vp), ("gamma", vp), ("gW", vp), ("ggamma", vp), ("rows", i32), ("cols", i32), ("ld_dwp", i32), ("reserved", i32)]
+
+
+FOLD_PARTS_MAX_JOBS = 16
+
+
+class FoldPartsJob(C.Structure):
+    _fields_ = [("part", vp), ("dst", vp), ("n_parts", i32), ("D", i32), ("ld", i32), ("reserved", i32)]
 
 
 class GemmF32Args(C.Structure):
@@ -162,12 +169,18 @@
 layernorm_fwd_res = _sig("fm_layernorm_fwd_res", vp, i32, vp, i32, vp, i32, vp, vp, vp, i32, i32, vp, vp, vp, i32, i32, f32, vp)
 layernorm_bwd = _sig("fm_layernorm_bwd", vp, i32, vp, vp, i32, vp, vp, vp, vp, vp, i32, vp, i32, vp, vp, i32, i32, vp)
 layernorm_bwd_h = _sig("fm_layernorm_bwd_h", vp, i32, vp, i32, vp, i32, vp, vp, vp, vp, vp, i32, vp, i32, vp, i32, i32, vp)
+layernorm_bwd_workgroups = _sig("fm_layernorm_bwd_workgroups", i32)
+layernorm_bwd_parts = _sig("fm_layernorm_bwd_parts", vp, i32, vp, vp, i32, vp, vp, vp, vp, vp, i32, vp, i32, vp, vp, i32, i32, vp)
+layernorm_bwd_h_parts = _sig("fm_layernorm_bwd_h_parts", vp, i32, vp, i32, vp, i32, vp, vp, vp, vp, vp, i32, vp, i32, vp, i32, i32, vp)
+fold_partials = _sig("fm_fold_partials", vp, i32, vp)
 attn_fwd = _sig("fm_attn_fwd", P(AttnArgs), vp)
 attn_bwd = _sig("fm_attn_bwd", P(AttnArgs), vp)
 attn_decode = _sig("fm_attn_decode", P(AttnDecodeArgs), vp)
 ATTN_DECODE_MAX_NK = 8192
 select_embed = _sig("fm_select_embed", P(SelectDesc), vp)
 embed_bwd = _sig("fm_embed_bwd", P(EmbedBwdDesc), vp)
+embed_bwd_ws_scratch = _sig("fm_embed_bwd_ws_scratch", P(EmbedBwdDesc))
+embed_bwd_ws = _sig("fm_embed_bwd_ws", P(EmbedBwdDesc), vp, i32, vp, i64, vp)
 dense_decoder_mask = _sig("fm_dense_decoder_mask", vp, vp, vp, i32, i32, i32, i32, i32, vp)
 segment_rows = _sig("fm_segment_rows", vp, i32, i32, vp, vp, vp, vp, vp, i32, vp)
 gather_rows = _sig("fm_gather_rows", vp, i32, vp, vp, i32, i32, i32, vp)
@@ -310,7 +323,8 @@
 EXPORTS = ["fm_pil_axis_table_f64", "fm_pil_crop_resize16", "fm_depth_standardize", "fm_pil_axis_table", "fm_pil_crop_resize", "fm_resize_axis_table", "fm_resize_bilinear_fwd", "fm_resize_bilinear_bwd", "fm_resize_nearest","fm_metric_sums_scratch", "fm_metric_sums", "fm_ssim_scale_scratch", "fm_ssim_scale", "fm_avgpool2x2_pair", "fm_token_histogram",
            "fm_reconst_loss_scratch", "fm_reconst_loss", "fm_scale_f32", "fm_mask_out_samples", "fm_ema_update", "fm_diffusion_pair", "fm_token_usage", "fm_lpips_stem", "fm_lpips_stem_bwd", "fm_maxpool2x2_nhwc", "fm_lpips_distance", "fm_lpips_tap_bwd", "fm_feat_distance", "fm_quick_gelu_bwd", "fm_quick_gelu_bwd_f32", "fm_clip_embed_ln_bwd", "fm_tap_add", "fm_clip_embed_ln", "fm_attn_decode", "fm_vit_patch_rows", "fm_vit_emb_rows", "fm_vit_colsum", "fm_lora_apply", "fm_lora_grad", "fm_vq_assign_wide", "fm_memcodes_assign", "fm_convnext_block", "fm_split3_bf16", "fm_unet_im2col", "fm_groupnorm_nhwc", "fm_add_bf16", "fm_silu_f32_to_bf16", "fm_timestep_embedding", "fm_unet_attention", "fm_diffusion_x0", "fm_quantile_abs",
            "fm_diffusion_step", "fm_unpack_image_u8", "fm_unpack_ids_u16", "fm_unpack_mask_bits", "fm_decoder_attention_from_target", "fm_guidance_combine", "fm_image_mask", "fm_token_budgets", "fm_span_mask", "fm_vq_code_stats", "fm_vq_ema_update", "fm_vq_code_bias", "fm_vq_assign_bias", "fm_vq_code_stats_raw", "fm_vq_ema_update_euclid", "fm_vq_unpatchify", "fm_vq_latent_grad", "fm_tanh_bwd_f32", "fm_embed_rows_f32", "fm_vq_patchify_ex", "fm_vq_cls_emb_bwd", "fm_vq_latent_grad_normalized", "fm_abi_version", "fm_last_error", "fm_gemm_nt", "fm_set_gemm_nt_config", "fm_get_gemm_nt_config", "fm_set_reserved_cus", "fm_get_reserved_cus", "fm_bf16_to_f32_scaled", "fm_add_bf16_f32", "fm_scale_rows_bf16", "fm_gemm_tn", "fm_gemm_tn_multi", "fm_set_gemm_tn_config", "fm_get_gemm_tn_config", "fm_set_tn_transpose_read",
-           "fm_get_tn_transpose_read", "fm_layernorm_fwd", "fm_layernorm_fwd_res", "fm_layernorm_bwd", "fm_layernorm_bwd_h", "fm_headnorm_fwd", "fm_headnorm_bwd", "fm_attn_fwd", "fm_attn_bwd",
+           "fm_get_tn_transpose_read", "fm_layernorm_fwd", "fm_layernorm_fwd_res", "fm_layernorm_bwd", "fm_layernorm_bwd_h", "fm_layernorm_bwd_workgroups", "fm_layernorm_bwd_parts", "fm_layernorm_bwd_h_parts", "fm_fold_partials",
+           "fm_embed_bwd_ws_scratch", "fm_embed_bwd_ws", "fm_headnorm_fwd", "fm_headnorm_bwd", "fm_attn_fwd", "fm_attn_bwd",
            "fm_set_attn_transpose_read", "fm_get_attn_transpose_read", "fm_select_embed", "fm_embed_bwd",
            "fm_dense_decoder_mask", "fm_segment_rows", "fm_gather_rows", "fm_cross_entropy", "fm_swiglu_bwd",
            "fm_gelu_bwd", "fm_cast_pad", "fm_transpose_cast_pad", "fm_shadow_refresh", "fm_fold_colscale_grad", "fm_colsum", "fm_f32_to_bf16", "fm_adamw", "fm_adamw_shadow",
diff --git a/ml-4m_amd/fourm/hip/engine.py b/ml-4m_amd/fourm/hip/engine.py
--- a/ml-4m_amd/fourm/hip/engine.py
+++ b/ml-4m_amd/fourm/hip/engine.py
@@ -18,6 +18,7 @@
 HOIST_CTX = os.environ.get("FOURM_HOIST_CTX", "1") == "1"
 LN_BWD_FROM_H = os.environ.get("FOURM_LN_BWD_FROM_H", "1") == "1"
 DP_RESERVE_ALWAYS = os.environ.get("FOURM_DP_RESERVE_ALWAYS", "0") == "1"
+STAGED_MIN_NUMEL = 65536
 
 
 def bump_weight_epoch():
@@ -243,11 +244,13 @@
         stages = {}
         for n, p in self._named:
             o, k = self._slices[id(p)]
-            stage = owner.get(id(p), "enc_emb") if k >= 65536 else "tail"
+            stage = owner.get(id(p), "enc_emb") if k >= STAGED_MIN_NUMEL else "tail"
             stages.setdefault(stage, []).append((o, ru(k, 16)))
         return stages
 
     def _stage(self, name):
+        if self.reducer is not None and getattr(self, "_ln_fold_staged", False):
+            self._fold_ln()
         if self.reducer is not None:
             self.reducer.stage_done(name)
 
@@ -821,8 +824,35 @@
     def _ln_bwd(self, norm, dy, x, sv, key, g, g_bf, R, dres, dy_row_map=None):
         dw = self._g(norm.weight)
         db = self._g(norm.bias) if isinstance(norm.bias, nn.Parameter) else None
-        ops.layernorm_bwd(dy, x, norm.weight, sv[key + ".mu"], sv[key + ".rs"], g, dres=dres, dx_bf16=g_bf, dw=dw, db=db,
+        fold = getattr(self, "_ln_fold", None)
+        if fold is None or dy.dtype == torch.float32 or (dw is None and db is None):
+            ops.layernorm_bwd(dy, x, norm.weight, sv[key + ".mu"], sv[key + ".rs"], g, dres=dres, dx_bf16=g_bf, dw=dw, db=db,
+                              dy_row_map=dy_row_map, R=R, h=sv.get(key + ".h"))
+            return
+        n, k = ops.layernorm_bwd_workgroups(R), len(fold)
+        pw = self.ws.get(f"bwd.ln_part_w{k}", (n, self.D), torch.float32) if dw is not None else None
+        pb = self.ws.get(f"bwd.ln_part_b{k}", (n, self.D), torch.float32) if db is not None else None
+        ops.layernorm_bwd(dy, x, norm.weight, sv[key + ".mu"], sv[key + ".rs"], g, dres=dres, dx_bf16=g_bf, part_dw=pw, part_db=pb,
                           dy_row_map=dy_row_map, R=R, h=sv.get(key + ".h"))
+        fold.append([(p, n, d) for p, d in ((pw, dw), (pb, db)) if p is not None])
+        if any(d.numel() >= STAGED_MIN_NUMEL for d in (dw, db) if d is not None):
+            self._ln_fold_staged = True
+        if sum(len(j) for j in fold) + 2 > L.FOLD_PARTS_MAX_JOBS:
+            self._fold_ln()
+
+    def _fold_ln(self):
+        fold = getattr(self, "_ln_fold", None)
+        if not fold:
+            return
+        jobs = [j for norm in fold for j in norm]
+        fold.clear()
+        self._ln_fold_staged = False
+        key = tuple((p.data_ptr(), n, d.data_ptr()) for p, n, d in jobs)
+        cache = self.__dict__.setdefault("_ln_fold_tables", {})
+        tables = cache.get(key)
+        if tables is None:
+            tables = cache[key] = ops.fold_partials_table(jobs)
+        ops.fold_partials(tables)
 
     def _mlp_bwd(self, mlp, sv, g_bf, R, Rp):
         bf, D, Hp, Hd = self.adt, self.D, self.Hp, self.Hd
@@ -974,24 +1004,26 @@
         if not is_dec and m.num_register_tokens and m.register_tokens.requires_grad:
             d.d_reg_tokens = self.grad_view(m.register_tokens).data_ptr()
         d.n_mods, d.batch, d.dim, d.Nt, d.is_decoder = len(sel["names"]), sel["B"], self.D, sel["Nt"], 1 if is_dec else 0
+        nbytes = L.embed_bwd_ws_scratch(ops.C.byref(d))
+        if nbytes <= 0:
+            L.check(-1)
+        scratch = self.ws.get("bwd.embed_parts", (nbytes // 4,), torch.float32)
         with ops._prof("embed_bwd"):
-            L.check(L.embed_bwd(ops.C.byref(d), ops._stream()))
-        if dx_extra is not None:
-            d2 = L.EmbedBwdDesc()
-            ops.C.memmove(ops.C.byref(d2), ops.C.byref(d), ops.C.sizeof(d))
-            for i in range(d.n_mods):
-                d2.mods[i].d_table = None
-                d2.mods[i].d_proj_bias = None
-            d2.d_reg_tokens = None
-            d2.dx, d2.lddx = dx_extra.data_ptr(), dx_extra.stride(0)
-            with ops._prof("embed_bwd"):
-                L.check(L.embed_bwd(ops.C.byref(d2), ops._stream()))
+            L.check(L.embed_bwd_ws(ops.C.byref(d), ops._p(dx_extra), dx_extra.stride(0) if dx_extra is not None else 0,
+                                   ops._p(scratch), nbytes, ops._stream()))
 
     def train_backward(self, grad_scale: torch.Tensor):
         c = self._ctx
         if c is None:
             raise RuntimeError("train_backward without a preceding training forward")
         self._ctx, self._dw_jobs = None, None
+        self._ln_fold, self._ln_fold_staged = [], False
+        try:
+            self._train_backward(c, grad_scale)
+        finally:
+            self._ln_fold = None
+
+    def _train_backward(self, c, grad_scale):
         if self.reducer is not None:
             self.reducer.begin()
             if getattr(self.reducer, "reserved_cus", 0):
@@ -1076,6 +1108,7 @@
             elif e.kind == L.KIND_SEQ_EMB and e.emb_proj.weight.requires_grad:
                 ops.gemm_tn(ge_bf, enc["seqemb_rows"], self.grad_view(e.emb_proj.weight), N=D, K=e.emb_proj.weight.shape[1], R=Rc)
         self._embed_bwd(enc, ge, dctx, False)
+        self._fold_ln()
         if self.reducer is not None:
             self.reducer.finish()
             if getattr(self.reducer, "reserved_cus", 0) and not DP_RESERVE_ALWAYS:
diff --git a/ml-4m_amd/fourm/hip/ops.py b/ml-4m_amd/fourm/hip/ops.py
--- a/ml-4m_amd/fourm/hip/ops.py
+++ b/ml-4m_amd/fourm/hip/ops.py
@@ -277,8 +277,27 @@
     return y
 
 
-def layernorm_bwd(dy, x, w, mean, rstd, dx, *, dres=None, dx_bf16=None, dw=None, db=None, dy_row_map=None, R=None, h=None):
+def layernorm_bwd_workgroups(R: int) -> int:
+    return L.layernorm_bwd_workgroups(R)
+
+
+def layernorm_bwd(dy, x, w, mean, rstd, dx, *, dres=None, dx_bf16=None, dw=None, db=None, dy_row_map=None, R=None, h=None,
+                  part_dw=None, part_db=None):
     R = x.shape[0] if R is None else R
+    if part_dw is not None or part_db is not None:
+        D, n = w.numel(), L.layernorm_bwd_workgroups(R)
+        assert dy.dtype != torch.float32 and dw is None and db is None, "partial rows: bf16 path, instead of dw / db"
+        for t in (part_dw, part_db):
+            assert t is None or (t.dtype == torch.float32 and t.is_contiguous() and t.numel() >= n * D), "partial buffer too small"
+        if h is not None and part_db is None and dy_row_map is None:
+            with _prof("layernorm_bwd", 0.0, R * D * (2 + 2 + 4 + 4 + (2 if dx_bf16 is not None else 0))):
+                L.check(L.layernorm_bwd_h_parts(_p(dy), _ld(dy), _p(h), _ld(h), _p(x), _ld(x), _p(w), _p(mean), _p(rstd), _p(dres), _p(dx), _ld(dx),
+                                                _p(dx_bf16), _ld(dx_bf16) if dx_bf16 is not None else 0, _p(part_dw), R, D, _stream()))
+            return dx
+        with _prof("layernorm_bwd", 0.0, R * D * (2 + 4 + 4 + 4 + (2 if dx_bf16 is not None else 0))):
+            L.check(L.layernorm_bwd_parts(_p(dy), _ld(dy), _p(dy_row_map), _p(x), _ld(x), _p(w), _p(mean), _p(rstd), _p(dres), _p(dx), _ld(dx),
+                                          _p(dx_bf16), _ld(dx_bf16) if dx_bf16 is not None else 0, _p(part_dw), _p(part_db), R, D, _stream()))
+        return dx
     if h is not None and dy.dtype != torch.float32 and db is None and dy_row_map is None:
         with _prof("layernorm_bwd", 0.0, R * w.numel() * (2 + 2 + 4 + 4 + (2 if dx_bf16 is not None else 0))):
             L.check(L.layernorm_bwd_h(_p(dy), _ld(dy), _p(h), _ld(h), _p(x), _ld(x), _p(w), _p(mean), _p(rstd), _p(dres), _p(dx), _ld(dx),
@@ -296,6 +315,26 @@
     L.check(L.layernorm_bwd(_p(dy), _ld(dy), _p(dy_row_map), _p(x), _ld(x), _p(w), _p(mean), _p(rstd), _p(dres), _p(dx), _ld(dx),
                             _p(dx_bf16), _ld(dx_bf16) if dx_bf16 is not None else 0, _p(dw), _p(db), R, w.numel(), _stream()))
     return dx
+
+
+def fold_partials_table(jobs):
+    tables = []
+    for lo in range(0, len(jobs), L.FOLD_PARTS_MAX_JOBS):
+        chunk = jobs[lo:lo + L.FOLD_PARTS_MAX_JOBS]
+        arr = (L.FoldPartsJob * len(chunk))()
+        for j, (part, n_parts, dst) in zip(arr, chunk):
+            D = dst.numel()
+            assert part.dtype == torch.float32 and dst.dtype == torch.float32 and part.is_contiguous() and dst.is_contiguous()
+            assert part.numel() >= n_parts * D and n_parts > 0
+            j.part, j.dst, j.n_parts, j.D, j.ld = part.data_ptr(), dst.data_ptr(), n_parts, D, D
+        tables.append(arr)
+    return tables
+
+
+def fold_partials(tables, family="layernorm_bwd"):
+    for arr in tables:
+        with _prof(family):
+            L.check(L.fold_partials(arr, len(arr), _stream()))
 
 
 @_timed("headnorm")
```
